# Kitware/pyLiDAR-SLAM

Measured on NVIDIA H100. Metric: icp_odometry_frames_per_sec, higher is better.
Workload: dtype f32

## Files before the change

### pylidar_slam_b200/csrc/context.cu

```cuda
#include <utility>

#include "internal.cuh"
#include "kdmap_device.cuh"

namespace pls {

long long g_kernel_launches = 0;

void DBuf::reserve(size_t bytes, cudaStream_t s, bool keep) {
    if (bytes <= cap) return;
    size_t want = bytes + bytes / 2 + 256;
    void* np = nullptr;
    PLS_CUDA(cudaStreamSynchronize(s));
    PLS_CUDA(cudaMalloc(&np, want));
    if (p) {
        if (keep) PLS_CUDA(cudaMemcpy(np, p, cap, cudaMemcpyDeviceToDevice));
        PLS_CUDA(cudaFree(p));
    }
    p = np;
    cap = want;
}

void DBuf::reserve_exact(size_t bytes, cudaStream_t s, bool keep) {
    if (bytes <= cap) return;
    void* np = nullptr;
    PLS_CUDA(cudaStreamSynchronize(s));
    PLS_CUDA(cudaMalloc(&np, bytes));
    if (p) {
        if (keep) PLS_CUDA(cudaMemcpy(np, p, cap, cudaMemcpyDeviceToDevice));
        PLS_CUDA(cudaFree(p));
    }
    p = np;
    cap = bytes;
}

void DBuf::release() {
    if (p) cudaFree(p);
    p = nullptr;
    cap = 0;
}

void HBuf::reserve(size_t bytes) {
    if (bytes <= cap) return;
    if (p) PLS_CUDA(cudaFreeHost(p));
    p = nullptr;
    cap = 0;
    PLS_CUDA(cudaHostAlloc(&p, bytes, cudaHostAllocMapped | cudaHostAllocPortable));
    cap = bytes;
}

void* HBuf::device_ptr() const {
    if (!p) return nullptr;
    void* d = nullptr;
    PLS_CUDA(cudaHostGetDevicePointer(&d, p, 0));
    return d;
}

void HBuf::release() {
    if (p) cudaFreeHost(p);
    p = nullptr;
    cap = 0;
}

void map_stream_begin(pls_context* ctx) {
    ctx->stream = ctx->stream_map;
    std::swap(ctx->sort, ctx->sort_map);
}

void map_stream_end(pls_context* ctx) {
    cudaEventRecord(ctx->ev_map_done, ctx->stream_map);
    ctx->map_pending = true;
    std::swap(ctx->sort, ctx->sort_map);
    ctx->stream = ctx->stream_main;
}

void map_stream_wait(pls_context* ctx) {
    if (ctx->map_pending) {
        cudaStreamWaitEvent(ctx->stream_main, ctx->ev_map_done, 0);
        ctx->map_pending = false;
    }
}

void sync_all(pls_context* ctx) {
    PLS_CUDA(cudaStreamSynchronize(ctx->stream_map));
    PLS_CUDA(cudaStreamSynchronize(ctx->stream_main));
    ctx->map_pending = false;
}

namespace {
struct PtrCacheEntry {
    const void* p;
    bool dev;
};
thread_local PtrCacheEntry t_ptr_cache[64] = {};
}

bool is_device_ptr(const void* p) {
    if (!p) return false;
    PtrCacheEntry& e = t_ptr_cache[(reinterpret_cast<uintptr_t>(p) >> 6) & 63u];
    if (e.p == p) return e.dev;
    const bool d = is_device_ptr_uncached(p);
    e.p = p;
    e.dev = d;
    return d;
}

bool is_device_ptr_uncached(const void* p) {
    if (!p) return false;
    cudaPointerAttributes a;
    cudaError_t e = cudaPointerGetAttributes(&a, p);
    if (e != cudaSuccess) {
        cudaGetLastError();
        return false;
    }
    return a.type == cudaMemoryTypeDevice || a.type == cudaMemoryTypeManaged;
}

const void* to_device(pls_context* ctx, const void* p, size_t bytes, DBuf& stage) {
    if (!p || bytes == 0) return p;
    if (is_device_ptr(p)) return p;
    stage.reserve(bytes, ctx->stream);
    PLS_CUDA(cudaMemcpyAsync(stage.p, p, bytes, cudaMemcpyHostToDevice, ctx->stream));
    return stage.p;
}

OutArg out_arg(pls_context* ctx, void* p, size_t bytes, DBuf& stage) {
    OutArg o;
    o.bytes = bytes;
    if (!p) return o;
    if (is_device_ptr(p)) {
        o.dev = p;
        return o;
    }
    stage.reserve(bytes, ctx->stream);
    o.host = p;
    o.dev = stage.p;
    return o;
}

void finish_out(pls_context* ctx, const OutArg& o, size_t bytes_used) {
    if (!o.host) return;
    size_t b = bytes_used == (size_t)-1 ? o.bytes : bytes_used;
    if (b) PLS_CUDA(cudaMemcpyAsync(o.host, o.dev, b, cudaMemcpyDeviceToHost, ctx->stream));
}

ProfileScope::ProfileScope(pls_context* c, int w, double bytes, bool count) : ctx(c), which(w) {
    ProfileSlot& s = ctx->prof[which];
    if (!s.enabled) return;
    if (s.used >= 4096) {
        cudaStreamSynchronize(ctx->stream_map);
        cudaStreamSynchronize(ctx->stream_main);
        profile_collect(ctx, which);
    }
    if (s.used + 2 > s.pool.size()) {
        for (int i = 0; i < 64; ++i) {
            cudaEvent_t e;
            if (cudaEventCreate(&e) != cudaSuccess) return;
            s.pool.push_back(e);
        }
    }
    e0 = s.pool[s.used++];
    e1 = s.pool[s.used++];
    if (count) {
        s.bytes += bytes;
        s.launches += 1;
    }
    cudaEventRecord(e0, ctx->stream);
}

ProfileScope::~ProfileScope() {
    if (e1) cudaEventRecord(e1, ctx->stream);
}

void profile_collect(pls_context* ctx, int which) {
    ProfileSlot& s = ctx->prof[which];
    for (size_t i = 0; i + 1 < s.used; i += 2) {
        float ms = 0.f;
        if (cudaEventElapsedTime(&ms, s.pool[i], s.pool[i + 1]) == cudaSuccess) s.ms += ms;
    }
    s.used = 0;
}

}

using namespace pls;

extern "C" {

const char* pls_version(void) { return "plslam_b200 0.1 (sm_90a)"; }

int pls_host_fingerprint(const void* host_ptr, int64_t num_bytes, uint64_t* out) {
    if (!host_ptr || !out || num_bytes < 0) return PLS_E_INVALID;
    const int64_t words = num_bytes / 8;
    uint64_t h = 0x9E3779B97F4A7C15ull ^ (uint64_t)num_bytes;
    const uint64_t* w = reinterpret_cast<const uint64_t*>(host_ptr);
    const int64_t step = words > 256 ? words / 256 : 1;
    for (int64_t i = 0; i < words; i += step) {
        uint64_t v;
        memcpy(&v, w + i, 8);
        h = (h ^ v) * 0x100000001B3ull;
        h ^= h >> 29;
    }
    if (words > 0) {
        uint64_t v;
        memcpy(&v, w + words - 1, 8);
        h = (h ^ v) * 0x100000001B3ull;
    }
    *out = h;
    return PLS_OK;
}

int pls_launch_count(int64_t* out) {
    if (!out) return PLS_E_INVALID;
    *out = (int64_t)pls::g_kernel_launches;
    return PLS_OK;
}

int pls_config_default(pls_config* c) {
    if (!c) return PLS_E_INVALID;
    memset(c, 0, sizeof(*c));
    c->height = 64;
    c->width = 2048;
    c->up_fov_deg = 3.0f;
    c->down_fov_deg = -24.0f;
    c->local_map_type = PLS_MAP_KDTREE;
    c->local_map_size = 20;
    c->num_neighbors_normals = 10;
    c->normals_kernel_size = 5;
    c->scheme = PLS_SCHEME_DEFAULT;
    c->sigma = 0.5f;
    c->gn_max_iters = 1;
    c->gn_norm_stop = 1e-3f;
    c->max_num_alignments = 100;
    c->threshold_delta_pose = 1e-4f;
    c->threshold_trans = 0.1f;
    c->threshold_rot = 0.3f;
    c->device = 0;
    c->stream = nullptr;
    return PLS_OK;
}

int pls_create(const pls_config* cfg, pls_context** out) {
    if (!cfg || !out) return PLS_E_INVALID;
    *out = nullptr;
    int ndev = 0;
    if (cudaGetDeviceCount(&ndev) != cudaSuccess || ndev <= 0) {
        cudaGetLastError();
        return PLS_E_CUDA;
    }
    if (cfg->device < 0 || cfg->device >= ndev) return PLS_E_INVALID;
    if (cfg->height <= 0 || cfg->width <= 0 || cfg->local_map_size <= 0) return PLS_E_INVALID;
    if (cfg->max_num_alignments < 1 || cfg->max_num_alignments > kMaxAlign) return PLS_E_INVALID;
    if (cfg->num_neighbors_normals < 3 || cfg->num_neighbors_normals + 1 > KD_KMAX_WIDE) return PLS_E_INVALID;
    if (cfg->normals_kernel_size < 1 || cfg->normals_kernel_size > 9 || (cfg->normals_kernel_size % 2) == 0)
        return PLS_E_INVALID;
    pls_context* ctx = new pls_context();
    ctx->cfg = *cfg;
    try {
        PLS_CUDA(cudaSetDevice(cfg->device));
        if (cfg->stream) {
            ctx->stream = (cudaStream_t)cfg->stream;
        } else {
            static const bool prio = !(getenv("PLS_STREAM_PRIORITY") && atoi(getenv("PLS_STREAM_PRIORITY")) == 0);
            int least = 0, greatest = 0;
            PLS_CUDA(cudaDeviceGetStreamPriorityRange(&least, &greatest));
            PLS_CUDA(cudaStreamCreateWithPriority(&ctx->stream, cudaStreamNonBlocking, prio ? greatest : 0));
            ctx->own_stream = true;
        }
        ctx->stream_main = ctx->stream;
        {
            static const bool prio = !(getenv("PLS_STREAM_PRIORITY") && atoi(getenv("PLS_STREAM_PRIORITY")) == 0);
            int least = 0, greatest = 0;
            PLS_CUDA(cudaDeviceGetStreamPriorityRange(&least, &greatest));
            PLS_CUDA(cudaStreamCreateWithPriority(&ctx->stream_map, cudaStreamNonBlocking, prio ? least : 0));
        }
        PLS_CUDA(cudaEventCreateWithFlags(&ctx->ev_map_done, cudaEventDisableTiming));
        ctx->pinned.reserve(kScalarOffset + 256);
        ctx->scalars.reserve(sizeof(FrameResult) + 4096, ctx->stream);
        PLS_CUDA(cudaMemsetAsync(ctx->scalars.p, 0, ctx->scalars.cap, ctx->stream));
        odometry_reset(ctx);
    } catch (const pls::Error& e) {
        fprintf(stderr, "pls_create: %s\n", e.msg.c_str());
        delete ctx;
        return e.code;
    }
    *out = ctx;
    return PLS_OK;
}

int pls_destroy(pls_context* ctx) {
    if (!ctx) return PLS_E_INVALID;
    cudaSetDevice(ctx->cfg.device);
    ctx->upd_pending = false;
    cudaStreamSynchronize(ctx->stream_map);
    cudaStreamSynchronize(ctx->stream_main);
    comm_free(ctx);
    if (ctx->p2p_pending_xchg) cudaFree(ctx->p2p_pending_xchg);
    for (auto& b : ctx->stage_in) b.release();
    for (auto& b : ctx->stage_out) b.release();
    for (auto& b : ctx->tmp) b.release();
    for (auto& b : ctx->next_buf) b.release();
    ctx->pinned.release();
    ctx->scalars.release();
    ctx->sort.keys_alt.release(); ctx->sort.vals_alt.release(); ctx->sort.hist.release();
    ctx->sort.status.release(); ctx->sort.plan.release();
    ctx->sort_map.keys_alt.release(); ctx->sort_map.vals_alt.release(); ctx->sort_map.hist.release();
    ctx->sort_map.status.release(); ctx->sort_map.plan.release();
    ctx->scan.status.release();
    ctx->sel[0].status.release(); ctx->sel[1].status.release(); ctx->input_zbuf.release();
    for (auto& b : ctx->kd.store) b.release();
    ctx->kd.morton.release(); ctx->kd.order.release(); ctx->kd.sorted.release(); ctx->kd.normals.release();
    ctx->kd.bbox.release(); ctx->kd.grid_hdr.release(); ctx->kd.cells.release(); ctx->kd.stats.release();
    ctx->kd_worklist.release(); ctx->kd_nn_state.release();
    ctx->pm.vmaps.release(); ctx->pm.nmaps.release(); ctx->pm.poses.release();
    ctx->pm.model_v.release(); ctx->pm.model_n.release(); ctx->pm.zbuf.release();
    for (auto& b : ctx->frame_vmap_buf) b.release();
    for (auto& b : ctx->frame_pts_buf) b.release();
    ctx->queries.release(); ctx->nn_prev.release();
    ctx->partials.release(); ctx->batch_buf.release(); ctx->hyp_buf.release(); ctx->gs_keys.release(); ctx->gs_vals.release(); ctx->gs_out_xyz.release();
    ctx->gs_out_idx.release();
    for (auto& s : ctx->prof)
        for (auto e : s.pool) cudaEventDestroy(e);
    if (ctx->ev_map_done) cudaEventDestroy(ctx->ev_map_done);
    if (ctx->ev_inputs) cudaEventDestroy(ctx->ev_inputs);
    if (ctx->ev_batch) cudaEventDestroy(ctx->ev_batch);
    ctx->gs_host_xyz.release(); ctx->gs_host_idx.release();
    if (ctx->stream_map) cudaStreamDestroy(ctx->stream_map);
    if (ctx->own_stream) cudaStreamDestroy(ctx->stream_main);
    delete ctx;
    return PLS_OK;
}

const char* pls_last_error(pls_context* ctx) { return ctx ? ctx->err.c_str() : "null context"; }

int pls_synchronize(pls_context* ctx) {
    PLS_API_BEGIN(ctx)
    sync_all(ctx);
    PLS_API_END(ctx)
}

int pls_wait_stream(pls_context* ctx, void* other_stream) {
    PLS_API_BEGIN(ctx)
    cudaStream_t other = (cudaStream_t)other_stream;
    if (other != ctx->stream_main) {
        if (!ctx->ev_inputs) PLS_CUDA(cudaEventCreateWithFlags(&ctx->ev_inputs, cudaEventDisableTiming));
        PLS_CUDA(cudaEventRecord(ctx->ev_inputs, other));
        PLS_CUDA(cudaStreamWaitEvent(ctx->stream_main, ctx->ev_inputs, 0));
    }
    PLS_API_END(ctx)
}

int pls_profile_enable(pls_context* ctx, int which, int enable) {
    PLS_API_BEGIN(ctx)
    PLS_REQUIRE(which >= 0 && which < kProfileSlots, "pls_profile_enable: bad slot");
    ctx->prof[which].enabled = enable != 0;
    PLS_API_END(ctx)
}

int pls_profile_read(pls_context* ctx, int which, double* ms_total, int64_t* launches, double* bytes, int reset) {
    PLS_API_BEGIN(ctx)
    PLS_REQUIRE(which >= 0 && which < kProfileSlots, "pls_profile_read: bad slot");
    sync_all(ctx);
    profile_collect(ctx, which);
    ProfileSlot& s = ctx->prof[which];
    if (ms_total) *ms_total = s.ms;
    if (launches) *launches = s.launches;
    if (bytes) *bytes = s.bytes;
    if (reset) {
        s.ms = 0;
        s.launches = 0;
        s.bytes = 0;
    }
    PLS_API_END(ctx)
}

}
```

### pylidar_slam_b200/csrc/internal.cuh

```cuda
#pragma once
#include <cuda_runtime.h>
#include <stddef.h>
#include <stdint.h>
#include <stdio.h>
#include <string.h>

#include <deque>
#include <string>
#include <vector>

#include "../../include/plslam_b200.h"

namespace pls {

constexpr int kNumSMs = 132;
constexpr int NACC = 30;
constexpr int kMaxAlign = 128;
constexpr int kProfileSlots = 16;
constexpr size_t kScalarOffset = 2048;

struct Error {
    int code;
    std::string msg;
};

extern long long g_kernel_launches;

#define PLS_CUDA(expr)                                                                            \
    do {                                                                                          \
        cudaError_t _e = (expr);                                                                  \
        if (_e != cudaSuccess) {                                                                  \
            throw pls::Error{PLS_E_CUDA, std::string(#expr) + ": " + cudaGetErrorString(_e) +     \
                                             " (" + __FILE__ + ":" + std::to_string(__LINE__) + ")"}; \
        }                                                                                         \
    } while (0)

#define PLS_CHECK_LAUNCH()            \
    do {                              \
        ++pls::g_kernel_launches;     \
        PLS_CUDA(cudaGetLastError()); \
    } while (0)

#ifdef __CUDACC__
__device__ __forceinline__ void pls_grid_dependency_wait() { asm volatile("griddepcontrol.wait;" ::: "memory"); }
#endif
template <typename... KArgs, typename... Args>
void launch_dependent(void (*kernel)(KArgs...), dim3 grid, dim3 block, cudaStream_t st, Args&&... args) {
    cudaLaunchConfig_t cfg = {};
    cfg.gridDim = grid;
    cfg.blockDim = block;
    cfg.dynamicSmemBytes = 0;
    cfg.stream = st;
    cudaLaunchAttribute attr[1];
    attr[0].id = cudaLaunchAttributeProgrammaticStreamSerialization;
    attr[0].val.programmaticStreamSerializationAllowed = 1;
    cfg.attrs = attr;
    cfg.numAttrs = 1;
    PLS_CUDA(cudaLaunchKernelEx(&cfg, kernel, static_cast<KArgs>(args)...));
    PLS_CHECK_LAUNCH();
}

#define PLS_REQUIRE(cond, text)                                   \
    do {                                                          \
        if (!(cond)) throw pls::Error{PLS_E_INVALID, (text)};     \
    } while (0)

struct DBuf {
    void* p = nullptr;
    size_t cap = 0;
    template <typename T>
    T* as() const { return reinterpret_cast<T*>(p); }
    void reserve(size_t bytes, cudaStream_t s, bool keep = false);
    void reserve_exact(size_t bytes, cudaStream_t s, bool keep = false);
    void release();
};

struct HBuf {
    void* p = nullptr;
    size_t cap = 0;
    template <typename T>
    T* as() const { return reinterpret_cast<T*>(p); }
    void reserve(size_t bytes);
    void release();
    void* device_ptr() const;
};

struct ProfileSlot {
    bool enabled = false;
    std::vector<cudaEvent_t> pool;
    size_t used = 0;
    double ms = 0.0;
    int64_t launches = 0;
    double bytes = 0.0;
};

struct SortScratch {
    DBuf keys_alt, vals_alt;
    DBuf hist;
    DBuf status;
    DBuf plan;
};

struct ScanScratch {
    DBuf status;
};

struct SelectScratch {
    DBuf status;
    uint32_t epoch = 0;
};

struct KdMap {
    DBuf store[2];
    int cur = 0;
    int64_t count = 0;
    std::deque<int64_t> frame_counts;
    DBuf morton, order;
    DBuf sorted;
    DBuf normals;
    DBuf bbox;
    bool bbox_clean = false;
    DBuf grid_hdr;
    DBuf cells;
    DBuf stats;
    size_t table_offset[16] = {};
    uint32_t table_mask[16] = {};
    uint32_t gen = 0;
    int64_t indexed = 0;
    bool valid = false;
    int64_t cap_points = 0;
    int64_t max_frame = 0;
    bool searched = false;
    bool searched_icp = false;
    bool searched_sharded = false;
    bool searched_normals = false;
    uint32_t searched_gen = 0;
    int64_t searched_n = 0;
};

struct ProjMap {
    int K = 0;
    int head = 0;
    DBuf vmaps, nmaps;
    DBuf poses;
    std::vector<float> host_poses;
    DBuf model_v, model_n;
    DBuf zbuf;
    bool valid = false;
    bool zbuf_clean = false;
    int64_t built_lo = 0, built_hi = 0;
};

struct FrameResult {
    float T[16];
    float params[6];
    float losses[kMaxAlign];
    int iters;
    int status;
    int done;
    int pad;
    double last_sums[NACC];
    long long counts[8];
    float first_pt[4];
};

struct Comm;

static_assert(sizeof(FrameResult) <= kScalarOffset, "FrameResult must fit before the scalar slots");

}

struct pls_context {
    pls_config cfg;
    cudaStream_t stream = nullptr;
    cudaStream_t stream_main = nullptr;
    cudaStream_t stream_map = nullptr;
    cudaEvent_t ev_map_done = nullptr;
    cudaEvent_t ev_inputs = nullptr;
    bool map_pending = false;
    bool own_stream = false;
    std::string err;

    pls::DBuf stage_in[4], stage_out[6];
    pls::HBuf pinned;
    pls::DBuf scalars;

    pls::SortScratch sort;
    pls::SortScratch sort_map;
    pls::ScanScratch scan;
    pls::SelectScratch sel[2];
    pls::DBuf input_zbuf;
    bool input_zbuf_clean = false;

    pls::DBuf tmp[8];
    pls::DBuf next_buf[8];

    pls::KdMap kd;
    pls::ProjMap pm;
    int frame_index = 0;
    int last_icp_iters = 0;
    bool icp_result = false;
    bool last_sharded = false;
    int sample_pointcloud = 0;
    float delta_since_update[16];
    pls::DBuf frame_vmap_buf[2];
    pls::DBuf frame_pts_buf[2];
    int frame_slot = 0;
    bool upd_pending = false, upd_insert = false;
    float upd_T[16];
    int upd_slot = 0;
    long long upd_count = 0;
    pls::DBuf queries;
    const float4* query_ptr = nullptr;
    pls::DBuf nn_prev;
    pls::DBuf kd_worklist;
    pls::DBuf kd_nn_state;
    pls::DBuf partials;
    pls::DBuf batch_buf;
    pls::DBuf hyp_buf;
    cudaEvent_t ev_batch = nullptr;
    pls::DBuf gs_keys, gs_vals, gs_out_xyz, gs_out_idx;
    uint32_t gs_seq = 0;
    pls::HBuf gs_host_xyz, gs_host_idx;
    int64_t last_query_count = 0;

    pls::Comm* comm = nullptr;
    void* p2p_pending_xchg = nullptr;
    pls::ProfileSlot prof[pls::kProfileSlots];
};

namespace pls {
void flush_map_update(pls_context* ctx);
}

#define PLS_API_BEGIN(ctx)                               \
    if (!(ctx)) return PLS_E_INVALID;                    \
    try {                                                \
        cudaSetDevice((ctx)->cfg.device);                \
        pls::flush_map_update(ctx);

#define PLS_API_BEGIN_FRAME(ctx)                         \
    if (!(ctx)) return PLS_E_INVALID;                    \
    try {                                                \
        cudaSetDevice((ctx)->cfg.device);

#define PLS_API_END(ctx)                                 \
    }                                                    \
    catch (const pls::Error& e) {                        \
        (ctx)->err = e.msg;                              \
        return e.code;                                   \
    }                                                    \
    catch (const std::exception& e) {                    \
        (ctx)->err = e.what();                           \
        return PLS_E_INVALID;                            \
    }                                                    \
    return PLS_OK;

namespace pls {

enum { SC_GS_COUNT = 0, SC_QUERY_COUNT = 1, SC_NAN_COUNT = 2, SC_INSERT_COUNT = 3, SC_PROJ_NC = 4,
       SC_SPARE0 = 5, SC_SPARE1 = 6,
       SC_GS_OVERFLOW = 7,
       SC_KD_COUNTERS = 8,
       SC_KD_LISTS = 16,
       SC_NUM = 32 };

bool is_device_ptr(const void* p);
bool is_device_ptr_uncached(const void* p);
const void* to_device(pls_context* ctx, const void* p, size_t bytes, DBuf& stage);
struct OutArg {
    void* host = nullptr;
    void* dev = nullptr;
    size_t bytes = 0;
};
OutArg out_arg(pls_context* ctx, void* p, size_t bytes, DBuf& stage);
void finish_out(pls_context* ctx, const OutArg& o, size_t bytes_used = (size_t)-1);

inline uint32_t* scalar_u32(pls_context* ctx, int i) {
    return reinterpret_cast<uint32_t*>(reinterpret_cast<char*>(ctx->scalars.p) + kScalarOffset) + i;
}
inline FrameResult* frame_result_dev(pls_context* ctx) { return reinterpret_cast<FrameResult*>(ctx->scalars.p); }
inline FrameResult* frame_result_host(pls_context* ctx) { return reinterpret_cast<FrameResult*>(ctx->pinned.p); }

void map_stream_begin(pls_context* ctx);
void map_stream_end(pls_context* ctx);
void map_stream_wait(pls_context* ctx);
void sync_all(pls_context* ctx);

struct ProfileScope {
    pls_context* ctx;
    int which;
    cudaEvent_t e0 = nullptr, e1 = nullptr;
    ProfileScope(pls_context* c, int w, double bytes, bool count = true);
    ~ProfileScope();
};
void profile_collect(pls_context* ctx, int which);
inline void profile_credit(pls_context* ctx, int which, int64_t launches, double bytes) {
    if (!ctx->prof[which].enabled) return;
    ctx->prof[which].launches += launches;
    ctx->prof[which].bytes += bytes;
}

void radix_sort_pairs(pls_context* ctx, uint64_t* keys, uint32_t* vals, int64_t n, int num_passes,
                      uint64_t** keys_out, uint32_t** vals_out, int64_t cap_n = 0);

void exclusive_scan_flags(pls_context* ctx, const uint8_t* flags, int64_t n, uint32_t* pos_out,
                          uint32_t* total_dev);

#ifdef __CUDACC__
__device__ __forceinline__ float warp_sum(float v) {
#pragma unroll
    for (int o = 16; o > 0; o >>= 1) v += __shfl_xor_sync(0xffffffffu, v, o);
    return v;
}
__device__ __forceinline__ double warp_sum(double v) {
#pragma unroll
    for (int o = 16; o > 0; o >>= 1) v += __shfl_xor_sync(0xffffffffu, v, o);
    return v;
}
__device__ __forceinline__ int float_to_ordered(float f) {
    int i = __float_as_int(f);
    return i >= 0 ? i : i ^ 0x7fffffff;
}
__device__ __forceinline__ float ordered_to_float(int i) {
    return __int_as_float(i >= 0 ? i : i ^ 0x7fffffff);
}
#endif

void launch_projection(pls_context* ctx, const float* xyz, const float* channels, int batch, int64_t n,
                       int C, int H, int W, float up, float down, float* out, unsigned long long* zbuf, float fill = 0.f);
void launch_projection_f64(pls_context* ctx, const double* xyz, int64_t n, int H, int W, float up, float down, float* out,
                           unsigned long long* zbuf);
void launch_zbuf_points(pls_context* ctx, const float* xyz, int64_t n, const uint32_t* n_dev, int H, int W, float up, float down,
                        unsigned long long* zbuf);
void launch_normal_map(pls_context* ctx, const float* vmap, int batch, int H, int W, int ksize, float* out);
struct GnParams {
    int scheme;
    double sigma;
};
void kdmap_reset(pls_context* ctx);
void kdmap_update(pls_context* ctx, const float* rel_pose_host, const float* pts_dev, int64_t n,
                  const float* vmap_dev, int H, int W, int64_t known_count);
void kdmap_update_packed(pls_context* ctx, const float* rel_pose_host, const float4* fresh_dev, int64_t num_new,
                         bool has_new);
constexpr int KD_BATCH_GRID = 6;
void kdmap_batch_begin(pls_context* lead, pls_context* const* ctxs, const int64_t* query_bounds, int num, cudaStream_t st,
                       int* grid);
void kdmap_batch_iterations(pls_context* lead, int num, cudaStream_t st, const int* grid, int first, int last);
void kdmap_batch_done(pls_context* lead, int num, cudaStream_t st, int* out);
struct KdScan {
    const float4* queries;
    const uint32_t* nq_dev;
    int64_t bound;
};
void kdmap_hypotheses_begin(pls_context* ctx, const KdScan* scans, int num, cudaStream_t st, int* grid, FrameResult** frs,
                            uint32_t** words);
void kdmap_hypothesis_adopt(pls_context* ctx, const KdScan& scan, int h, cudaStream_t st);
struct KdScanRows {
    const float* rows;
    int64_t n;
    float4* out;
    uint32_t* count;
};
void pack_valid_scans(pls_context* ctx, const std::vector<KdScanRows>& scans);
int kdmap_icp_iteration(pls_context* ctx, int64_t query_bound, const uint32_t* bound_dev, int rank, int num_ranks, int it,
                        float fuse_threshold, bool* solved);
void pack_valid_rows(pls_context* ctx, const float* pts_dev, int64_t n, float4* out, uint32_t* count_dev);
void pack_valid_rows_f64(pls_context* ctx, const double* pts_dev, int64_t n, float4* out, uint32_t* count_dev);
void pack_valid_pixels(pls_context* ctx, const float* vmap_dev, int64_t hw, float min_norm, float4* out,
                       uint32_t* count_dev);
struct GridSample {
    const void* xyz;
    bool f64;
    int64_t n;
    double voxel;
    void* out_xyz;
    long long* out_idx;
    void* host_xyz;
    long long* host_idx;
};
void grid_sample_enqueue(pls_context* ctx, const GridSample& g, bool count_to_host = true);
uint32_t grid_sample_finish(pls_context* ctx, const GridSample& g);
uint32_t grid_sample_host_count(pls_context* ctx, bool* overflowed);
void projmap_reset(pls_context* ctx);
void projmap_batch_begin(pls_context* lead, pls_context* const* ctxs, const int64_t* query_bounds, int num, cudaStream_t st,
                         int* grid);
void projmap_batch_iterations(pls_context* lead, pls_context* const* ctxs, const int64_t* query_bounds, int num, cudaStream_t st,
                              const int* grid, int first, int last);
void projmap_batch_done(pls_context* lead, int num, cudaStream_t st, int* out);
void projmap_hypotheses_begin(pls_context* ctx, int num, cudaStream_t st, FrameResult** frs, uint32_t** words);
void projmap_hypotheses_iterations(pls_context* ctx, int64_t query_bound, int num, cudaStream_t st, int first, int last);
void projmap_hypothesis_adopt(pls_context* ctx, int h, cudaStream_t st);
bool icp_shards(pls_context* ctx, int64_t work);
int comm_rank(pls_context* ctx);
int comm_size(pls_context* ctx);
void projmap_update(pls_context* ctx, const float* rel_pose_host, const float* vmap_dev);
void odometry_reset(pls_context* ctx);
void comm_allreduce_sums(pls_context* ctx, double* sums_dev);
void comm_free(pls_context* ctx);

}
```

### pylidar_slam_b200/csrc/kdmap.cu

```cuda
#include <stdlib.h>

#include <vector>

#include "gn_device.cuh"
#include "internal.cuh"
#include "icp_device.cuh"
#include "kdmap_device.cuh"
#include "pose_device.cuh"

namespace pls {

namespace {

inline int grid_for(int64_t n, int threads, int cap_blocks) {
    int64_t b = (n + threads - 1) / threads;
    return (int)(b < 1 ? 1 : (b > cap_blocks ? cap_blocks : b));
}

__global__ void kd_bbox_init_kernel(int* bbox) {
    if (threadIdx.x < 3) bbox[threadIdx.x] = 0x7fffffff;
    else if (threadIdx.x < 6) bbox[threadIdx.x] = (int)0x80000000;
}

struct Rigid {
    float R[9];
    float t[3];
};

__global__ void __launch_bounds__(256)
kd_move_append_kernel(const float4* __restrict__ src, int64_t skip, int64_t kept, Rigid X,
                      const float4* __restrict__ fresh, const uint32_t* __restrict__ num_new_dev, int64_t num_new_cap,
                      float4* __restrict__ dst, int* __restrict__ bbox) {
    const int64_t num_new = num_new_dev ? (int64_t)*num_new_dev : num_new_cap;
    const int64_t total = kept + num_new;
    float mn[3] = {FLT_MAX, FLT_MAX, FLT_MAX}, mx[3] = {-FLT_MAX, -FLT_MAX, -FLT_MAX};
    for (int64_t k = (int64_t)blockIdx.x * blockDim.x + threadIdx.x; k < total; k += (int64_t)gridDim.x * blockDim.x) {
        float4 p;
        if (k < kept) {
            float4 s = src[k + skip];
            p.x = X.R[0] * s.x + X.R[1] * s.y + X.R[2] * s.z + X.t[0];
            p.y = X.R[3] * s.x + X.R[4] * s.y + X.R[5] * s.z + X.t[1];
            p.z = X.R[6] * s.x + X.R[7] * s.y + X.R[8] * s.z + X.t[2];
            p.w = 0.f;
        } else {
            p = fresh[k - kept];
        }
        dst[k] = p;
        mn[0] = fminf(mn[0], p.x); mn[1] = fminf(mn[1], p.y); mn[2] = fminf(mn[2], p.z);
        mx[0] = fmaxf(mx[0], p.x); mx[1] = fmaxf(mx[1], p.y); mx[2] = fmaxf(mx[2], p.z);
    }
#pragma unroll
    for (int a = 0; a < 3; ++a) {
#pragma unroll
        for (int o = 16; o > 0; o >>= 1) {
            mn[a] = fminf(mn[a], __shfl_xor_sync(0xffffffffu, mn[a], o));
            mx[a] = fmaxf(mx[a], __shfl_xor_sync(0xffffffffu, mx[a], o));
        }
    }
    __shared__ float smn[8][3], smx[8][3];
    const int warp = threadIdx.x >> 5, lane = threadIdx.x & 31;
    if (lane == 0) {
#pragma unroll
        for (int a = 0; a < 3; ++a) { smn[warp][a] = mn[a]; smx[warp][a] = mx[a]; }
    }
    __syncthreads();
    if (threadIdx.x < 3) {
        const int a = threadIdx.x;
        float lo = smn[0][a], hi = smx[0][a];
        for (int w = 1; w < 8; ++w) { lo = fminf(lo, smn[w][a]); hi = fmaxf(hi, smx[w][a]); }
        if (lo != FLT_MAX) atomicMin(&bbox[a], float_to_ordered(lo));
        if (hi != -FLT_MAX) atomicMax(&bbox[3 + a], float_to_ordered(hi));
    }
}

template <typename T>
__global__ void kd_valid_rows_kernel(const T* __restrict__ pts, int64_t n, uint8_t* __restrict__ flags) {
    for (int64_t i = (int64_t)blockIdx.x * blockDim.x + threadIdx.x; i < n; i += (int64_t)gridDim.x * blockDim.x) {
        T x = pts[3 * i], y = pts[3 * i + 1], z = pts[3 * i + 2];
        flags[i] = (x == x && y == y && z == z) ? 1 : 0;
    }
}
template <typename T>
__global__ void kd_pack_rows_kernel(const T* __restrict__ pts, int64_t n, const uint8_t* __restrict__ flags,
                                    const uint32_t* __restrict__ pos, float4* __restrict__ out) {
    for (int64_t i = (int64_t)blockIdx.x * blockDim.x + threadIdx.x; i < n; i += (int64_t)gridDim.x * blockDim.x)
        if (flags[i]) out[pos[i]] = make_float4((float)pts[3 * i], (float)pts[3 * i + 1], (float)pts[3 * i + 2], 0.f);
}
constexpr int KD_PACK_THREADS = 1024, KD_PACK_ROWS = 4;
__global__ void __launch_bounds__(KD_PACK_THREADS) kd_pack_scans_kernel(const KdScanRows* __restrict__ scans) {
    __shared__ uint32_t s_warp[KD_PACK_ROWS][32];
    __shared__ uint32_t s_sub[KD_PACK_ROWS];
    const KdScanRows sc = scans[blockIdx.x];
    const int lane = threadIdx.x & 31, warp = threadIdx.x >> 5;
    const uint32_t below = (1u << lane) - 1u;
    uint32_t base = 0;
    for (int64_t t0 = 0; t0 < sc.n; t0 += (int64_t)KD_PACK_THREADS * KD_PACK_ROWS) {
        float4 v[KD_PACK_ROWS];
        bool ok[KD_PACK_ROWS];
        uint32_t rank[KD_PACK_ROWS];
#pragma unroll
        for (int j = 0; j < KD_PACK_ROWS; ++j) {
            const int64_t i = t0 + (int64_t)j * KD_PACK_THREADS + threadIdx.x;
            ok[j] = false;
            if (i < sc.n) {
                const float x = sc.rows[3 * i], y = sc.rows[3 * i + 1], z = sc.rows[3 * i + 2];
                ok[j] = x == x && y == y && z == z;
                v[j] = make_float4(x, y, z, 0.f);
            }
            const unsigned b = __ballot_sync(0xffffffffu, ok[j]);
            rank[j] = __popc(b & below);
            if (lane == 0) s_warp[j][warp] = __popc(b);
        }
        __syncthreads();
        if (warp < KD_PACK_ROWS) {
            const uint32_t c = s_warp[warp][lane];
            uint32_t inc = c;
#pragma unroll
            for (int o = 1; o < 32; o <<= 1) {
                const uint32_t u = __shfl_up_sync(0xffffffffu, inc, o);
                if (lane >= o) inc += u;
            }
            s_warp[warp][lane] = inc - c;
            if (lane == 31) s_sub[warp] = inc;
        }
        __syncthreads();
#pragma unroll
        for (int j = 0; j < KD_PACK_ROWS; ++j) {
            if (ok[j]) sc.out[base + s_warp[j][warp] + rank[j]] = v[j];
            base += s_sub[j];
        }
        __syncthreads();
    }
    if (threadIdx.x == 0) *sc.count = base;
}

template <typename T>
__global__ void kd_nonfinite_rows_kernel(const T* __restrict__ pts, int64_t n, uint32_t* __restrict__ count) {
    uint32_t bad = 0;
    for (int64_t i = (int64_t)blockIdx.x * blockDim.x + threadIdx.x; i < n; i += (int64_t)gridDim.x * blockDim.x)
        bad += !(isfinite((float)pts[3 * i]) && isfinite((float)pts[3 * i + 1]) && isfinite((float)pts[3 * i + 2]));
    bad = __reduce_add_sync(0xffffffffu, bad);
    if ((threadIdx.x & 31) == 0 && bad) atomicAdd(count, bad);
}
__global__ void kd_valid_pixels_kernel(const float* __restrict__ vmap, int64_t hw, float min_norm,
                                       uint8_t* __restrict__ flags) {
    for (int64_t i = (int64_t)blockIdx.x * blockDim.x + threadIdx.x; i < hw; i += (int64_t)gridDim.x * blockDim.x) {
        float x = vmap[i], y = vmap[hw + i], z = vmap[2 * hw + i];
        flags[i] = (sqrtf(x * x + y * y + z * z) > min_norm) ? 1 : 0;
    }
}
__global__ void kd_pack_pixels_kernel(const float* __restrict__ vmap, int64_t hw, const uint8_t* __restrict__ flags,
                                      const uint32_t* __restrict__ pos, float4* __restrict__ out) {
    for (int64_t i = (int64_t)blockIdx.x * blockDim.x + threadIdx.x; i < hw; i += (int64_t)gridDim.x * blockDim.x)
        if (flags[i]) out[pos[i]] = make_float4(vmap[i], vmap[hw + i], vmap[2 * hw + i], 0.f);
}

__global__ void kd_grid_header_kernel(int* __restrict__ bbox, KdGridHeader* __restrict__ hdr, float cell_target) {
    if (threadIdx.x != 0) return;
    const float mnx = ordered_to_float(bbox[0]), mny = ordered_to_float(bbox[1]), mnz = ordered_to_float(bbox[2]);
    const float ex = ordered_to_float(bbox[3]) - mnx, ey = ordered_to_float(bbox[4]) - mny,
                ez = ordered_to_float(bbox[5]) - mnz;
    const float ext = fmaxf(fmaxf(ex, ey), fmaxf(ez, 1e-6f));
    const int b0 = KD_MIN_B0;
    const float scale = fminf((float)(1 << b0) / cell_target, (float)KD_COORD_MAX / ext);
    hdr->mn[0] = mnx; hdr->mn[1] = mny; hdr->mn[2] = mnz;
    hdr->scale = scale;
    hdr->b0 = b0;
    hdr->cell0 = (float)(1 << b0) / scale;
    hdr->top = KD_COORD_BITS - b0;
    for (int l = 0; l < KD_MAX_LEVELS; ++l) hdr->overflow[l] = 0;
    bbox[0] = bbox[1] = bbox[2] = 0x7fffffff;
    bbox[3] = bbox[4] = bbox[5] = (int)0x80000000;
}

__global__ void kd_cell_key_kernel(const float4* __restrict__ pts, int64_t n, const KdGridHeader* __restrict__ hdr,
                                   uint64_t* __restrict__ keys, uint32_t* __restrict__ vals) {
    pls_grid_dependency_wait();
    const float mnx = hdr->mn[0], mny = hdr->mn[1], mnz = hdr->mn[2];
    const float scale = hdr->scale;
    const int b0 = hdr->b0;
    for (int64_t i = (int64_t)blockIdx.x * blockDim.x + threadIdx.x; i < n; i += (int64_t)gridDim.x * blockDim.x) {
        const float4 p = pts[i];
        const uint32_t qx = (uint32_t)fminf(fmaxf((p.x - mnx) * scale, 0.f), (float)KD_COORD_MAX);
        const uint32_t qy = (uint32_t)fminf(fmaxf((p.y - mny) * scale, 0.f), (float)KD_COORD_MAX);
        const uint32_t qz = (uint32_t)fminf(fmaxf((p.z - mnz) * scale, 0.f), (float)KD_COORD_MAX);
        keys[i] = (uint64_t)kd_cell_id(qx >> b0, qy >> b0, qz >> b0);
        vals[i] = (uint32_t)i;
    }
}

struct CellTables {
    uint4* table[KD_MAX_LEVELS];
    uint32_t mask[KD_MAX_LEVELS];
};

__device__ __forceinline__ int cell_claim(uint4* table, uint32_t mask, uint32_t id, uint32_t gen) {
    const unsigned long long want = (unsigned long long)id | ((unsigned long long)gen << 32);
    uint32_t h = kd_hash(id) & mask;
    for (int probe = 0; probe < 64; ++probe) {
        unsigned long long* word = reinterpret_cast<unsigned long long*>(&table[h]);
        unsigned long long old = *reinterpret_cast<volatile unsigned long long*>(word);
        while (true) {
            if (old == want) return (int)h;
            if ((uint32_t)(old >> 32) == gen) break;
            const unsigned long long prev = atomicCAS(word, old, want);
            if (prev == old) return (int)h;
            old = prev;
        }
        h = (h + 1) & mask;
    }
    return -1;
}

__global__ void __launch_bounds__(256)
kd_finalize_kernel(const float4* __restrict__ pts, const uint64_t* __restrict__ keys, const uint32_t* __restrict__ order,
                   int64_t n, CellTables T, KdGridHeader* hdr, uint32_t gen, float4* __restrict__ sorted) {
    pls_grid_dependency_wait();
    const int top = hdr->top;
    for (int64_t i = (int64_t)blockIdx.x * blockDim.x + threadIdx.x; i < n; i += (int64_t)gridDim.x * blockDim.x) {
        const uint32_t src = order[i];
        float4 p = pts[src];
        p.w = __uint_as_float(src);
        sorted[i] = p;
        const uint32_t k = (uint32_t)keys[i];
        int nh = top + 1, nt = top + 1;
        if (i > 0) {
            const uint32_t d = k ^ (uint32_t)keys[i - 1];
            nh = d ? min((31 - __clz((int)d)) / 3 + 1, top + 1) : 0;
        }
        if (i + 1 < n) {
            const uint32_t d = k ^ (uint32_t)keys[i + 1];
            nt = d ? min((31 - __clz((int)d)) / 3 + 1, top + 1) : 0;
        }
        const int nl = max(nh, nt);
        for (int l = 0; l < nl; ++l) {
            const int slot = cell_claim(T.table[l], T.mask[l], k >> (3 * l), gen);
            if (slot < 0) {
                hdr->overflow[l] = 1;
            } else {
                if (l < nh) T.table[l][slot].z = (uint32_t)i;
                if (l < nt) T.table[l][slot].w = (uint32_t)i;
            }
        }
    }
}

__global__ void kd_export_kernel(const float4* __restrict__ pts, int64_t n, float* __restrict__ out) {
    for (int64_t i = (int64_t)blockIdx.x * blockDim.x + threadIdx.x; i < n; i += (int64_t)gridDim.x * blockDim.x) {
        float4 p = pts[i];
        out[3 * i] = p.x; out[3 * i + 1] = p.y; out[3 * i + 2] = p.z;
    }
}

constexpr int KD_THREADS = 256;
constexpr int KD_WARPS = KD_THREADS / 32;

enum { KDC_NN_CAND = 0, KDC_KNN_CAND = 1, KDC_NORMALS = 2 };
enum { KDL_PENDING = 0, KDL_HARD_NN = 2, KDL_WORDS = 4 };

#ifdef PLS_KD_SPLIT
constexpr int KD_SPLIT_ITERS = 8;
constexpr int KD_SPLIT_BLOCKS = 8 * kNumSMs;
constexpr int KD_SPLIT_WORDS = (KD_SPLIT_ITERS + 1) * KD_SPLIT_BLOCKS * 2 * KD_SPLIT_STAMPS;
__device__ unsigned long long g_kd_split[KD_SPLIT_WORDS];
__device__ unsigned long long g_kd_split_normals_end;

__device__ __forceinline__ unsigned long long* kd_split_record(const FrameResult* fr) {
    const int slot = fr->done ? KD_SPLIT_ITERS : fr->iters;
    if ((!fr->done && slot >= KD_SPLIT_ITERS) || blockIdx.x >= KD_SPLIT_BLOCKS) return nullptr;
    return g_kd_split + ((size_t)slot * KD_SPLIT_BLOCKS + blockIdx.x) * 2 * KD_SPLIT_STAMPS;
}
#define KD_SPLIT_BEGIN()                             \
    unsigned long long* split = kd_split_record(fr); \
    __shared__ unsigned long long s_split[2];        \
    if (threadIdx.x == 0) {                          \
        PLS_SPLIT(0);                                \
        s_split[0] = s_split[1] = 0;                 \
        unsigned sm;                                 \
        asm volatile("mov.u32 %0, %%smid;" : "=r"(sm)); \
        if (split) split[11] = sm + 1;               \
    }
#define KD_SPLIT_MAX(k, dep) atomicMax(&s_split[k], split_now(dep))
#define KD_SPLIT_BLOCK_MAX()         \
    if (threadIdx.x == 0 && split) { \
        split[2] = s_split[0];       \
        split[3] = s_split[1];       \
    }
#define KD_SPLIT_ARG , unsigned long long* split, unsigned long long* s_split
#define KD_SPLIT_PASS , split, s_split
#else
#define KD_SPLIT_BEGIN()
#define KD_SPLIT_MAX(k, dep) \
    do {                     \
    } while (0)
#define KD_SPLIT_BLOCK_MAX()
#define KD_SPLIT_ARG
#define KD_SPLIT_PASS
#endif

__device__ __forceinline__ unsigned kd_logical_blocks(int64_t bound, const uint32_t* __restrict__ bound_dev) {
    if (!bound_dev) return gridDim.x;
    const int64_t n = min(bound, (int64_t)*bound_dev);
    const int64_t b = (n + KD_THREADS - 1) / KD_THREADS;
    return (unsigned)(b < 1 ? 1 : (b > 8 * kNumSMs ? 8 * kNumSMs : b));
}

__device__ __forceinline__ void block_flush_list(const int* s_list, int n, int* __restrict__ list, uint32_t* count, int* s_base) {
    if (n == 0) return;
    if (threadIdx.x == 0) *s_base = (int)atomicAdd(count, (uint32_t)n);
    __syncthreads();
    for (int i = threadIdx.x; i < n; i += blockDim.x) list[*s_base + i] = s_list[i];
}

__device__ __forceinline__ bool claim_normal(const KdIndex& ix, int pos) {
    const uint32_t claimed = kd_normal_claimed(ix.gen), valid = kd_normal_valid(ix.gen);
    uint32_t* w = reinterpret_cast<uint32_t*>(&ix.normals[pos].w);
    const uint32_t cur = __ldcg(w);
    return cur != valid && cur != claimed && atomicCAS(w, cur, claimed) == cur;
}

__device__ __forceinline__ void transform_query(const float* T, const float4& p0, float* p) {
    p[0] = p0.x * T[0] + p0.y * T[1] + p0.z * T[2] + T[3];
    p[1] = p0.x * T[4] + p0.y * T[5] + p0.z * T[6] + T[7];
    p[2] = p0.x * T[8] + p0.y * T[9] + p0.z * T[10] + T[11];
}

__device__ __forceinline__ bool match_proven(const KdIndex& ix, const float* p, int pos, const float4& state) {
    if (pos < 0) return false;
    const float4 s = state;
    const float d = sqrtf(dist2_point(p[0], p[1], p[2], __ldg(ix.sorted + pos)));
    const float eps = sqrtf(dist2_point(p[0], p[1], p[2], s));
    return (d + eps) * 1.00001f + 1e-6f < sqrtf(s.w);
}

template <int R = 1>
__device__ __forceinline__ void warp_normal_moments(const KdIndex& ix, const KdGridLocal& g, const float4& c, int k, int lane,
                                                    int* cand, unsigned long long* stage, float* cov) {
    if constexpr (R == 1) {
        int ni;
        const int found = warp_knn(ix, g, c.x, c.y, c.z, k + 1, lane, ni, cand, stage);
        warp_second_moments(ix, c, k, found, ni, lane, cov);
    } else {
        unsigned long long kept[R];
        const int found = warp_knn_wide<R>(ix, g, c.x, c.y, c.z, k + 1, lane, kept, cand, stage);
        warp_second_moments_wide<R>(ix, c, k, found, kept, lane, cov);
    }
}

__device__ __forceinline__ void store_normal(const KdIndex& ix, int pos, const float* cov, uint32_t valid) {
    float nn[3];
    smallest_eigenvector(cov, nn);
    __stcg(ix.normals + pos, make_float4(nn[0], nn[1], nn[2], __uint_as_float(valid)));
}

__device__ __forceinline__ void accumulate_match(double* acc, const KdIndex& ix, const float* p, int pos, int scheme,
                                                 float sigma KD_SPLIT_ARG) {
    const float4 qq = __ldg(ix.sorted + pos);
    const float4 nv = __ldcg(ix.normals + pos);
    float q[3] = {qq.x, qq.y, qq.z};
    float nn[3] = {nv.x, nv.y, nv.z};
    float J[6];
    const float r = p2plane_residual_jacobian_identity(p, q, nn, J);
    KD_SPLIT_MAX(0, r);
    const float w = ls_weight<float>(scheme, sigma, r, p, q);
    accumulate_normal_equations<float>(acc, J, w, r * w, r);
}

template <int THREADS>
__device__ __forceinline__ void block_partial_and_finish(double* acc, FrameResult* fr, double* __restrict__ partials,
                                                         float fuse_threshold, unsigned block, unsigned grid KD_SPLIT_ARG) {
    KD_SPLIT_MAX(1, acc[0] + acc[29]);
    __syncwarp();
    block_reduce_store<THREADS, KD_WARPS>(acc, partials + (size_t)block * NACC);
    KD_SPLIT_BLOCK_MAX()
    if (fuse_threshold >= 0.f) icp_finish_in_last_block<THREADS>(fr, partials, (int)grid, fuse_threshold PLS_SPLIT_PASS);
}

__device__ __forceinline__ void kd_nn_verify_body(const KdIndex& ix, const float4* __restrict__ queries,
                                                  const uint32_t* __restrict__ nq_dev, int64_t q_begin, int64_t q_stride,
                                                  const float* __restrict__ T, const int* __restrict__ done,
                                                  const int* __restrict__ match, const float4* __restrict__ nn_state,
                                                  int* __restrict__ hard, uint32_t* lists, int parity, unsigned block) {
    if (done && *done) return;
    __shared__ float sT[12];
    __shared__ int s_hard[KD_THREADS];
    __shared__ int s_nh, s_base;
    if (threadIdx.x < 12) sT[threadIdx.x] = T[threadIdx.x];
    if (threadIdx.x == 0) {
        s_nh = 0;
        if (block == 0)
            for (int l = 0; l < KDL_WORDS; l += 2) lists[l + (parity ^ 1)] = 0;
    }
    __syncthreads();
    const int64_t nq = (int64_t)*nq_dev;
    const int64_t qi = q_begin + ((int64_t)block * KD_THREADS + threadIdx.x) * q_stride;
    if (qi < nq) {
        float p[3];
        transform_query(sT, queries[qi], p);
        if (!match_proven(ix, p, match[qi], nn_state[qi])) s_hard[atomicAdd(&s_nh, 1)] = (int)qi;
    }
    __syncthreads();
    block_flush_list(s_hard, s_nh, hard, lists + KDL_HARD_NN + parity, &s_base);
}

__global__ void __launch_bounds__(KD_THREADS)
kd_nn_verify_kernel(KdIndex ix, const float4* __restrict__ queries, const uint32_t* __restrict__ nq_dev, int64_t q_begin,
                    int64_t q_stride, const float* __restrict__ T, const int* __restrict__ done, const int* __restrict__ match,
                    const float4* __restrict__ nn_state, int* __restrict__ hard, uint32_t* lists, int parity) {
    kd_nn_verify_body(ix, queries, nq_dev, q_begin, q_stride, T, done, match, nn_state, hard, lists, parity, blockIdx.x);
}


__device__ __forceinline__ void kd_nn_warp_body(const KdIndex& ix, const float4* __restrict__ queries,
                                                const uint32_t* __restrict__ nq_dev, int64_t q_begin, int64_t q_stride,
                                                const int* __restrict__ hard, uint32_t* lists, int parity,
                                                const float* __restrict__ T, const int* __restrict__ done,
                                                int* __restrict__ match, float4* __restrict__ nn_state, int want_normals,
                                                int* __restrict__ pending, unsigned long long* __restrict__ counters,
                                                unsigned block, unsigned grid) {
    if (done && *done) return;
    int n;
    if (hard) {
        n = (int)lists[KDL_HARD_NN + parity];
    } else {
        const int64_t nq = (int64_t)*nq_dev;
        n = nq > q_begin ? (int)((nq - q_begin + q_stride - 1) / q_stride) : 0;
        if (block == 0 && threadIdx.x == 0)
            for (int l = 0; l < KDL_WORDS; l += 2) lists[l + (parity ^ 1)] = 0;
    }
    const int lane = threadIdx.x & 31;
    const int warp_global = block * KD_WARPS + (threadIdx.x >> 5);
    const int total_warps = grid * KD_WARPS;
    if (warp_global >= n) return;
    float t[12];
#pragma unroll
    for (int a = 0; a < 12; ++a) t[a] = T[a];
    const KdGridLocal g = kd_load_grid(ix);
    uint32_t* pending_count = lists + KDL_PENDING + parity;
    int my_pos = -1, held = 0, cand = 0;
    auto flush_claims = [&]() {
        const bool mine = want_normals && my_pos >= 0 && claim_normal(ix, my_pos);
        const unsigned m = __ballot_sync(FULL, mine);
        if (m) {
            int base = 0;
            if (lane == 0) base = (int)atomicAdd(pending_count, (uint32_t)__popc(m));
            base = __shfl_sync(FULL, base, 0);
            if (mine) pending[base + __popc(m & ((1u << lane) - 1u))] = my_pos;
        }
        my_pos = -1;
        held = 0;
    };
    int s = warp_global;
    int64_t qi = hard ? (int64_t)hard[s] : q_begin + (int64_t)s * q_stride;
    float4 p0 = queries[qi];
    int hint = hard ? match[qi] : -1;
    while (true) {
        const int sn = s + total_warps;
        int64_t qn = qi;
        float4 pn = p0;
        int hn = -1;
        if (sn < n) {
            qn = hard ? (int64_t)hard[sn] : q_begin + (int64_t)sn * q_stride;
            pn = queries[qn];
            if (hard) hn = match[qn];
        }
        float p[3];
        transform_query(t, p0, p);
        float second;
        const int pos = warp_nearest(ix, g, p[0], p[1], p[2], hint, lane, &cand, &second);
        if (lane == 0) {
            match[qi] = pos;
            if (nn_state) nn_state[qi] = make_float4(p[0], p[1], p[2], second);
        }
        if (lane == held) my_pos = pos;
        if (++held == 32) flush_claims();
        if (sn >= n) break;
        s = sn;
        qi = qn;
        p0 = pn;
        hint = hn;
    }
    flush_claims();
    if (counters && lane == 0 && cand) atomicAdd(counters + KDC_NN_CAND, (unsigned long long)cand);
}

__global__ void __launch_bounds__(KD_THREADS)
kd_nn_warp_kernel(KdIndex ix, const float4* __restrict__ queries, const uint32_t* __restrict__ nq_dev, int64_t q_begin,
                  int64_t q_stride, const int* __restrict__ hard, uint32_t* lists, int parity, const float* __restrict__ T,
                  const int* __restrict__ done, int* __restrict__ match, float4* __restrict__ nn_state, int want_normals,
                  int* __restrict__ pending, unsigned long long* __restrict__ counters) {
    pls_grid_dependency_wait();
    kd_nn_warp_body(ix, queries, nq_dev, q_begin, q_stride, hard, lists, parity, T, done, match, nn_state, want_normals,
                    pending, counters, blockIdx.x, gridDim.x);
}

template <int R = 1>
__device__ __forceinline__ void kd_normals_warp_body(const KdIndex& ix, int k_normals, const int* __restrict__ worklist,
                                                     const uint32_t* __restrict__ wl_count, const int* __restrict__ done,
                                                     unsigned long long* __restrict__ counters, unsigned block, unsigned grid) {
    if (done && *done) return;
    __shared__ unsigned long long s_stage[KD_WARPS][KNN_STAGE];
    const int n = (int)*wl_count;
    const int lane = threadIdx.x & 31;
    const int warp_global = block * KD_WARPS + (threadIdx.x >> 5);
    const int total_warps = grid * KD_WARPS;
    if (warp_global >= n) return;
    unsigned long long* stage = s_stage[threadIdx.x >> 5];
    const KdGridLocal g = kd_load_grid(ix);
    const uint32_t valid = kd_normal_valid(ix.gen);
    float mycov[6];
    int mypos = -1, held = 0, cand = 0, done_here = 0;
    int e = warp_global;
    int pos = worklist[e];
    float4 c = __ldg(ix.sorted + pos);
    while (true) {
        const int en = e + total_warps;
        int posn = 0;
        float4 cn = c;
        if (en < n) {
            posn = worklist[en];
// ... 104 lines not shown
    for (int64_t round = (int64_t)block * KD_THREADS;; round += (int64_t)grid * KD_THREADS) {
        if (q_begin + round * q_stride >= nq) break;
        if (threadIdx.x == 0) s_nh = 0;
        __syncthreads();
        const int64_t qi = q_begin + (round + threadIdx.x) * q_stride;
        if (owner && qi < nq) {
            float p[3];
            transform_query(sT, queries[qi], p);
            if (!match_proven(ix, p, match[qi], nn_state[qi])) s_hard[atomicAdd(&s_nh, 1)] = threadIdx.x;
        }
        __syncthreads();
        const int nh = s_nh;
#ifdef PLS_KD_SPLIT
        if (threadIdx.x == 0 && split) split[9] += (unsigned long long)nh;
#endif
        if (warp < nh) {
            const KdGridLocal g = kd_load_grid(ix);
            for (int e = warp; e < nh; e += KD_REFINE_WARPS) {
                const int64_t q = q_begin + (round + s_hard[e]) * q_stride;
                float p[3];
                transform_query(sT, queries[q], p);
                float second;
                const int pos = warp_nearest(ix, g, p[0], p[1], p[2], match[q], lane, &cand_nn, &second);
                if (lane == 0) {
                    match[q] = pos;
                    nn_state[q] = make_float4(p[0], p[1], p[2], second);
                }
                if (pos < 0) continue;
                const uint32_t state = __shfl_sync(FULL, __ldcg(reinterpret_cast<const uint32_t*>(&ix.normals[pos].w)), 0);
                if (state == valid) continue;
                float cov[6];
                warp_normal_moments(ix, g, __ldg(ix.sorted + pos), k_normals, lane, &cand_knn, s_stage[warp], cov);
                if (lane == 0) store_normal(ix, pos, cov, valid);
                ++normals_here;
            }
        }
        __syncthreads();
    }
    if (counters && lane == 0) {
        if (cand_nn) atomicAdd(counters + KDC_NN_CAND, (unsigned long long)cand_nn);
        if (cand_knn) atomicAdd(counters + KDC_KNN_CAND, (unsigned long long)cand_knn);
        if (normals_here) atomicAdd(counters + KDC_NORMALS, (unsigned long long)normals_here);
    }
#ifdef PLS_KD_SPLIT
    if (lane == 0 && split && normals_here) atomicAdd(split + 10, (unsigned long long)normals_here);
#endif
    if (threadIdx.x == 0) PLS_SPLIT(1);
    double acc[NACC];
#pragma unroll
    for (int a = 0; a < NACC; ++a) acc[a] = 0.0;
    for (int64_t s = (int64_t)block * KD_THREADS + threadIdx.x; owner; s += (int64_t)grid * KD_THREADS) {
        const int64_t qi = q_begin + s * q_stride;
        if (qi >= nq) break;
        const int pos = match[qi];
        if (pos < 0) continue;
        float p[3];
        transform_query(sT, queries[qi], p);
        accumulate_match(acc, ix, p, pos, scheme, sigma KD_SPLIT_PASS);
    }
    block_partial_and_finish<KD_REFINE_THREADS>(acc, fr, partials, fuse_threshold, block, grid KD_SPLIT_PASS);
}

__global__ void __launch_bounds__(KD_REFINE_THREADS)
kd_icp_refine_kernel(KdIndex ix, const float4* __restrict__ queries, const uint32_t* __restrict__ nq_dev, int64_t q_begin,
                     int64_t q_stride, FrameResult* fr, int scheme, float sigma, int k_normals, int* __restrict__ match,
                     float4* __restrict__ nn_state, double* __restrict__ partials, float fuse_threshold,
                     unsigned long long* __restrict__ counters, int64_t bound, const uint32_t* __restrict__ bound_dev) {
    pls_grid_dependency_wait();
    const unsigned grid = kd_logical_blocks(bound, bound_dev);
    if (blockIdx.x >= grid) return;
    KD_SPLIT_BEGIN()
    kd_icp_refine_body(ix, queries, nq_dev, q_begin, q_stride, fr, scheme, sigma, k_normals, match, nn_state, partials,
                       fuse_threshold, counters, blockIdx.x, grid KD_SPLIT_PASS);
}

struct KdSeq {
    KdIndex ix;
    const float4* queries;
    const uint32_t* nq_dev;
    FrameResult* fr;
    int* match;
    float4* nn_state;
    int* pending;
    int* hard;
    uint32_t* lists;
    double* partials;
    unsigned long long* counters;
    int scheme;
    float sigma;
    int k_normals;
    float fuse_threshold;
    int max_iters;
    int blocks;
    int refine_blocks;
    int verify_blocks;
    int nn_blocks, kn_blocks;
};
static_assert(sizeof(KdSeq) % sizeof(int) == 0, "KdSeq is copied in 4-byte words");

__device__ __forceinline__ void load_seq(const KdSeq* __restrict__ seqs, KdSeq& s) {
    const int* src = reinterpret_cast<const int*>(seqs + blockIdx.y);
    int* dst = reinterpret_cast<int*>(&s);
    for (int i = threadIdx.x; i < (int)(sizeof(KdSeq) / sizeof(int)); i += blockDim.x) dst[i] = __ldg(src + i);
    __syncthreads();
}

#ifdef PLS_KD_SPLIT
#define KD_SPLIT_NONE()                     \
    unsigned long long* split = nullptr;    \
    __shared__ unsigned long long s_split[2];
#else
#define KD_SPLIT_NONE()
#endif

__device__ __forceinline__ bool four_launch_step(const KdSeq& s, int it) {
    return it == 0 || (s.refine_blocks == 0 && it < s.max_iters);
}

__global__ void __launch_bounds__(KD_THREADS) kd_nn_verify_batch_kernel(const KdSeq* __restrict__ seqs, int it) {
    __shared__ KdSeq s;
    load_seq(seqs, s);
    if ((int)blockIdx.x >= s.verify_blocks || !four_launch_step(s, it)) return;
    kd_nn_verify_body(s.ix, s.queries, s.nq_dev, 0, 1, s.fr->T, &s.fr->done, s.match, s.nn_state, s.hard, s.lists, it & 1,
                      blockIdx.x);
}

__global__ void __launch_bounds__(KD_THREADS) kd_nn_warp_batch_kernel(const KdSeq* __restrict__ seqs, int it) {
    __shared__ KdSeq s;
    load_seq(seqs, s);
    if ((int)blockIdx.x >= s.nn_blocks || !four_launch_step(s, it)) return;
    kd_nn_warp_body(s.ix, s.queries, s.nq_dev, 0, 1, it == 0 ? nullptr : s.hard, s.lists, it & 1, s.fr->T, &s.fr->done,
                    s.match, s.nn_state, 1, s.pending, s.counters, blockIdx.x, s.nn_blocks);
}

__global__ void __launch_bounds__(KD_THREADS) kd_normals_warp_batch_kernel(const KdSeq* __restrict__ seqs, int it) {
    __shared__ KdSeq s;
    load_seq(seqs, s);
    if ((int)blockIdx.x >= s.kn_blocks || !four_launch_step(s, it) || kd_wide_k(s.k_normals)) return;
    kd_normals_warp_body(s.ix, s.k_normals, s.pending, s.lists + KDL_PENDING + (it & 1), &s.fr->done, s.counters,
                         blockIdx.x, s.kn_blocks);
}

template <int R>
__global__ void __launch_bounds__(KD_THREADS) kd_normals_wide_batch_kernel(const KdSeq* __restrict__ seqs, int it) {
    __shared__ KdSeq s;
    load_seq(seqs, s);
    if ((int)blockIdx.x >= s.kn_blocks || !four_launch_step(s, it) || !kd_wide_k(s.k_normals)) return;
    kd_normals_warp_body<R>(s.ix, s.k_normals, s.pending, s.lists + KDL_PENDING + (it & 1), &s.fr->done, s.counters,
                            blockIdx.x, s.kn_blocks);
}

__global__ void __launch_bounds__(KD_THREADS) kd_residual_batch_kernel(const KdSeq* __restrict__ seqs, int it) {
    __shared__ KdSeq s;
    load_seq(seqs, s);
    if ((int)blockIdx.x >= s.blocks || !four_launch_step(s, it)) return;
    KD_SPLIT_NONE()
    kd_residual_body(s.ix, s.queries, s.nq_dev, 0, 1, s.fr, s.scheme, s.sigma, s.match, s.partials, s.fuse_threshold,
                     blockIdx.x, s.blocks KD_SPLIT_PASS);
}

__global__ void __launch_bounds__(KD_REFINE_THREADS) kd_icp_refine_batch_kernel(const KdSeq* __restrict__ seqs, int it) {
    __shared__ KdSeq s;
    load_seq(seqs, s);
    if ((int)blockIdx.x >= s.refine_blocks || it >= s.max_iters) return;
    KD_SPLIT_NONE()
    kd_icp_refine_body(s.ix, s.queries, s.nq_dev, 0, 1, s.fr, s.scheme, s.sigma, s.k_normals, s.match, s.nn_state,
                       s.partials, s.fuse_threshold, s.counters, blockIdx.x, s.refine_blocks KD_SPLIT_PASS);
}

__global__ void kd_batch_done_kernel(const KdSeq* __restrict__ seqs, int num, int* __restrict__ out) {
    for (int i = threadIdx.x; i < num; i += blockDim.x) out[i] = seqs[i].fr->done;
}

__global__ void kd_rows_to_float4_kernel(const float* __restrict__ rows, int64_t n, float4* __restrict__ out) {
    for (int64_t i = (int64_t)blockIdx.x * blockDim.x + threadIdx.x; i < n; i += (int64_t)gridDim.x * blockDim.x)
        out[i] = make_float4(rows[3 * i], rows[3 * i + 1], rows[3 * i + 2], 0.f);
}

__global__ void kd_search_export_kernel(KdIndex ix, const int* __restrict__ match, int64_t n, float* __restrict__ out_nb,
                                        float* __restrict__ out_nrm, long long* __restrict__ out_idx) {
    const float nan = __int_as_float(0x7fc00000);
    for (int64_t i = (int64_t)blockIdx.x * blockDim.x + threadIdx.x; i < n; i += (int64_t)gridDim.x * blockDim.x) {
        const int pos = match[i];
        float4 q = make_float4(nan, nan, nan, 0.f), nv = make_float4(nan, nan, nan, 0.f);
        long long idx = -1;
        if (pos >= 0) {
            q = __ldg(ix.sorted + pos);
            idx = (long long)__float_as_uint(q.w);
            if (out_nrm) nv = __ldcg(ix.normals + pos);
        }
        out_nb[3 * i] = q.x; out_nb[3 * i + 1] = q.y; out_nb[3 * i + 2] = q.z;
        if (out_idx) out_idx[i] = idx;
        if (out_nrm) { out_nrm[3 * i] = nv.x; out_nrm[3 * i + 1] = nv.y; out_nrm[3 * i + 2] = nv.z; }
    }
}

__global__ void __launch_bounds__(KD_THREADS)
kd_knn_export_kernel(KdIndex ix, const float* __restrict__ rows, int64_t n, int K, long long* __restrict__ out_idx,
                     float* __restrict__ out_d2, int* __restrict__ out_pos) {
    __shared__ unsigned long long s_stage[KD_WARPS][KNN_STAGE];
    const int lane = threadIdx.x & 31, warp = threadIdx.x >> 5;
    const KdGridLocal g = kd_load_grid(ix);
    const float nan = __int_as_float(0x7fc00000);
    for (int64_t q = (int64_t)blockIdx.x * KD_WARPS + warp; q < n; q += (int64_t)gridDim.x * KD_WARPS) {
        const float x = rows[3 * q], y = rows[3 * q + 1], z = rows[3 * q + 2];
        int pos;
        warp_knn(ix, g, x, y, z, K, lane, pos, nullptr, s_stage[warp]);
        if (lane < K) {
            long long idx = -1;
            float d2 = nan;
            if (pos >= 0) {
                const float4 s = __ldg(ix.sorted + pos);
                idx = (long long)__float_as_uint(s.w);
                d2 = dist2_point(x, y, z, s);
            }
            out_idx[q * K + lane] = idx;
            out_d2[q * K + lane] = d2;
            if (out_pos) out_pos[q * K + lane] = pos;
        }
    }
}

template <int R>
__global__ void __maxnreg__(128)
kd_knn_wide_export_kernel(KdIndex ix, const float* __restrict__ rows, int64_t n, int K, long long* __restrict__ out_idx,
                          float* __restrict__ out_d2, int* __restrict__ out_pos) {
    __shared__ unsigned long long s_stage[KD_WARPS][KNN_STAGE];
    const int lane = threadIdx.x & 31, warp = threadIdx.x >> 5;
    const KdGridLocal g = kd_load_grid(ix);
    const float nan = __int_as_float(0x7fc00000);
    for (int64_t q = (int64_t)blockIdx.x * KD_WARPS + warp; q < n; q += (int64_t)gridDim.x * KD_WARPS) {
        const float x = rows[3 * q], y = rows[3 * q + 1], z = rows[3 * q + 2];
        unsigned long long kept[R];
        warp_knn_wide<R>(ix, g, x, y, z, K, lane, kept, nullptr, s_stage[warp]);
#pragma unroll
        for (int r = 0; r < R; ++r) {
            const int j = r * 32 + lane;
            if (j >= K) break;
            const int pos = kept[r] != KNN_NONE ? (int)(unsigned)kept[r] : -1;
            long long idx = -1;
            float d2 = nan;
            if (pos >= 0) {
                const float4 s = __ldg(ix.sorted + pos);
                idx = (long long)__float_as_uint(s.w);
                d2 = dist2_point(x, y, z, s);
            }
            out_idx[q * K + j] = idx;
            out_d2[q * K + j] = d2;
            if (out_pos) out_pos[q * K + j] = pos;
        }
    }
}

size_t cell_table_bytes(int64_t M, uint32_t* masks, size_t* offsets) {
    size_t off = 0;
    for (int l = 0; l < KD_MAX_LEVELS; ++l) {
        uint64_t want = (uint64_t)(1.5 * (double)M) >> l;
        uint32_t sz = 64;
        while (sz < want) sz <<= 1;
        if (masks) masks[l] = sz - 1;
        if (offsets) offsets[l] = off;
        off += (size_t)sz * sizeof(uint4);
    }
    return off;
}

void kd_reserve_capacity(pls_context* ctx, int64_t need) {
    KdMap& kd = ctx->kd;
    if (need <= kd.cap_points) return;
    cudaStream_t st = ctx->stream;
    int64_t steady = (int64_t)(1.3 * (double)kd.max_frame * (double)(ctx->cfg.local_map_size + 1));
    if (steady > need + (8ll << 20)) steady = need + (8ll << 20);
    int64_t cap = need + need / 4 + 64;
    if (cap < steady) cap = steady;
    const size_t C = (size_t)cap;
    kd.store[kd.cur].reserve_exact(C * sizeof(float4), st, true);
    kd.store[kd.cur ^ 1].reserve_exact(C * sizeof(float4), st);
    kd.morton.reserve_exact(C * sizeof(uint64_t), st);
    kd.order.reserve_exact(C * sizeof(uint32_t), st);
    kd.sorted.reserve_exact(C * sizeof(float4), st);
    kd.normals.reserve_exact(C * sizeof(float4), st);
    const size_t table_bytes = cell_table_bytes(cap, nullptr, nullptr);
    kd.cells.reserve_exact(table_bytes, st);
    PLS_CUDA(cudaMemsetAsync(kd.normals.p, 0, C * sizeof(float4), st));
    PLS_CUDA(cudaMemsetAsync(kd.cells.p, 0, table_bytes, st));
    kd.cap_points = cap;
}

KdIndex make_index(pls_context* ctx) {
    KdIndex ix;
    ix.sorted = ctx->kd.sorted.as<float4>();
    ix.normals = ctx->kd.normals.as<float4>();
    ix.M = (int)ctx->kd.indexed;
    ix.gen = ctx->kd.gen;
    ix.grid = ctx->kd.grid_hdr.as<KdGridHeader>();
    for (int l = 0; l < KD_MAX_LEVELS; ++l) {
        ix.table[l] = reinterpret_cast<const uint4*>(reinterpret_cast<const char*>(ctx->kd.cells.p) + ctx->kd.table_offset[l]);
        ix.mask[l] = ctx->kd.table_mask[l];
    }
    ix.stats = ctx->kd.stats.p ? ctx->kd.stats.as<unsigned long long>() : nullptr;
    return ix;
}

void build_index(pls_context* ctx) {
    KdMap& kd = ctx->kd;
    cudaStream_t st = ctx->stream;
    const int64_t M = kd.count;
    kd.indexed = M;
    kd.valid = M > 0;
    if (M <= 0) return;
    ProfileScope ps(ctx, 3, (double)M * 32.0);
    PLS_REQUIRE(M < (1ll << 30), "kd map: too many points");
    kd_reserve_capacity(ctx, M);
    kd.gen += 1;
    if (kd.gen >= 0x7ffffff0u) {
        PLS_CUDA(cudaMemsetAsync(kd.normals.p, 0, kd.normals.cap, st));
        PLS_CUDA(cudaMemsetAsync(kd.cells.p, 0, kd.cells.cap, st));
        kd.gen = 1;
    }
    const float4* pts = kd.store[kd.cur].as<float4>();
    kd.grid_hdr.reserve(sizeof(KdGridHeader), st);
    static const float cell_target = getenv("PLS_KD_CELL") ? (float)atof(getenv("PLS_KD_CELL")) : KD_CELL_TARGET;
    kd_grid_header_kernel<<<1, 32, 0, st>>>(kd.bbox.as<int>(), kd.grid_hdr.as<KdGridHeader>(), cell_target);
    PLS_CHECK_LAUNCH();
    kd.bbox_clean = true;
    launch_dependent(kd_cell_key_kernel, grid_for(M, 256, 8 * kNumSMs), 256, st, pts, M, kd.grid_hdr.as<KdGridHeader>(),
                     kd.morton.as<uint64_t>(), kd.order.as<uint32_t>());
    uint64_t* sk;
    uint32_t* sv;
    radix_sort_pairs(ctx, kd.morton.as<uint64_t>(), kd.order.as<uint32_t>(), M, 4, &sk, &sv, kd.cap_points);
    cell_table_bytes(kd.cap_points, kd.table_mask, kd.table_offset);
    CellTables T;
    for (int l = 0; l < KD_MAX_LEVELS; ++l) {
        T.table[l] = reinterpret_cast<uint4*>(reinterpret_cast<char*>(kd.cells.p) + kd.table_offset[l]);
        T.mask[l] = kd.table_mask[l];
    }
    launch_dependent(kd_finalize_kernel, grid_for(M, 256, 8 * kNumSMs), 256, st, pts, sk, sv, M, T, kd.grid_hdr.as<KdGridHeader>(),
                     kd.gen, kd.sorted.as<float4>());
}

}

void kdmap_reset(pls_context* ctx) {
    if (getenv("PLS_KD_STATS") && !ctx->kd.stats.p) {
        ctx->kd.stats.reserve(16 * sizeof(unsigned long long), ctx->stream);
        cudaMemsetAsync(ctx->kd.stats.p, 0, 16 * sizeof(unsigned long long), ctx->stream);
    }
    ctx->kd.count = 0;
    ctx->kd.cur = 0;
    ctx->kd.frame_counts.clear();
    ctx->kd.indexed = 0;
    ctx->kd.valid = false;
    ctx->kd.bbox_clean = false;
    ctx->kd.max_frame = 0;
    ctx->kd.searched = false;
}

template <typename T>
static void pack_valid_rows_impl(pls_context* ctx, const T* pts_dev, int64_t n, float4* out, uint32_t* count_dev) {
    cudaStream_t st = ctx->stream;
    if (n <= 0) {
        PLS_CUDA(cudaMemsetAsync(count_dev, 0, sizeof(uint32_t), st));
        return;
    }
    ctx->tmp[1].reserve((size_t)n, st);
    ctx->tmp[2].reserve((size_t)n * sizeof(uint32_t), st);
    const int g = grid_for(n, 256, 8 * kNumSMs);
    kd_valid_rows_kernel<T><<<g, 256, 0, st>>>(pts_dev, n, ctx->tmp[1].as<uint8_t>());
    PLS_CHECK_LAUNCH();
    exclusive_scan_flags(ctx, ctx->tmp[1].as<uint8_t>(), n, ctx->tmp[2].as<uint32_t>(), count_dev);
    kd_pack_rows_kernel<T><<<g, 256, 0, st>>>(pts_dev, n, ctx->tmp[1].as<uint8_t>(), ctx->tmp[2].as<uint32_t>(), out);
    PLS_CHECK_LAUNCH();
}

void pack_valid_rows(pls_context* ctx, const float* pts_dev, int64_t n, float4* out, uint32_t* count_dev) {
    pack_valid_rows_impl<float>(ctx, pts_dev, n, out, count_dev);
}
void pack_valid_rows_f64(pls_context* ctx, const double* pts_dev, int64_t n, float4* out, uint32_t* count_dev) {
    pack_valid_rows_impl<double>(ctx, pts_dev, n, out, count_dev);
}

void pack_valid_scans(pls_context* ctx, const std::vector<KdScanRows>& scans) {
    cudaStream_t st = ctx->stream;
    const size_t bytes = scans.size() * sizeof(KdScanRows);
    ctx->stage_in[2].reserve(bytes, st);
    PLS_CUDA(cudaMemcpyAsync(ctx->stage_in[2].p, scans.data(), bytes, cudaMemcpyHostToDevice, st));
    kd_pack_scans_kernel<<<(unsigned)scans.size(), KD_PACK_THREADS, 0, st>>>(ctx->stage_in[2].as<KdScanRows>());
    PLS_CHECK_LAUNCH();
}

void pack_valid_pixels(pls_context* ctx, const float* vmap_dev, int64_t hw, float min_norm, float4* out,
                       uint32_t* count_dev) {
    cudaStream_t st = ctx->stream;
    ctx->tmp[1].reserve((size_t)hw, st);
    ctx->tmp[2].reserve((size_t)hw * sizeof(uint32_t), st);
    const int g = grid_for(hw, 256, 8 * kNumSMs);
    kd_valid_pixels_kernel<<<g, 256, 0, st>>>(vmap_dev, hw, min_norm, ctx->tmp[1].as<uint8_t>());
    PLS_CHECK_LAUNCH();
    exclusive_scan_flags(ctx, ctx->tmp[1].as<uint8_t>(), hw, ctx->tmp[2].as<uint32_t>(), count_dev);
    kd_pack_pixels_kernel<<<g, 256, 0, st>>>(vmap_dev, hw, ctx->tmp[1].as<uint8_t>(), ctx->tmp[2].as<uint32_t>(), out);
    PLS_CHECK_LAUNCH();
}

void kdmap_update_packed(pls_context* ctx, const float* rel_pose_host, const float4* fresh_dev, int64_t num_new,
                         bool has_new) {
    KdMap& kd = ctx->kd;
    cudaStream_t st = ctx->stream;
    Rigid X;
    int64_t skip = 0;
    const bool first = kd.frame_counts.empty() && kd.count == 0;
    if (first) {
        for (int i = 0; i < 9; ++i) X.R[i] = (i % 4 == 0) ? 1.f : 0.f;
        X.t[0] = X.t[1] = X.t[2] = 0.f;
        kd.frame_counts.push_back(num_new);
    } else {
        float inv[16];
        rigid_inverse(rel_pose_host, inv);
        X.R[0] = inv[0]; X.R[1] = inv[1]; X.R[2] = inv[2];
        X.R[3] = inv[4]; X.R[4] = inv[5]; X.R[5] = inv[6];
        X.R[6] = inv[8]; X.R[7] = inv[9]; X.R[8] = inv[10];
        X.t[0] = inv[3]; X.t[1] = inv[7]; X.t[2] = inv[11];
        if (has_new) {
            kd.frame_counts.push_back(num_new);
            if ((int)kd.frame_counts.size() > ctx->cfg.local_map_size) {
                skip = kd.frame_counts.front();
                kd.frame_counts.pop_front();
            }
        }
    }
    if (!has_new) num_new = 0;
    const int64_t kept = kd.count - skip;
    const int64_t total = kept + num_new;
    if (num_new > kd.max_frame) kd.max_frame = num_new;
    kd_reserve_capacity(ctx, total > 0 ? total : 1);
    const int dst = kd.cur ^ 1;
    kd.bbox.reserve(8 * sizeof(int), st);
    if (!kd.bbox_clean) {
        kd_bbox_init_kernel<<<1, 32, 0, st>>>(kd.bbox.as<int>());
        PLS_CHECK_LAUNCH();
    }
    kd.bbox_clean = false;
    if (total > 0) {
        kd_move_append_kernel<<<grid_for(total, 256, 8 * kNumSMs), 256, 0, st>>>(
            kd.store[kd.cur].as<float4>(), skip, kept, X, fresh_dev, nullptr, num_new, kd.store[dst].as<float4>(),
            kd.bbox.as<int>());
        PLS_CHECK_LAUNCH();
    }
    kd.cur = dst;
    kd.count = total;
    build_index(ctx);
}

void kdmap_update(pls_context* ctx, const float* rel_pose_host, const float* pts_dev, int64_t n,
                  const float* vmap_dev, int H, int W, int64_t known_count) {
    cudaStream_t st = ctx->stream;
    const bool has_new = (pts_dev != nullptr) || (vmap_dev != nullptr);
    const int64_t cap_new = pts_dev ? n : (vmap_dev ? (int64_t)H * W : 0);
    int64_t num_new = 0;
    if (has_new && cap_new > 0) {
        ctx->tmp[4].reserve((size_t)cap_new * sizeof(float4), st);
        uint32_t* cnt = scalar_u32(ctx, SC_INSERT_COUNT);
        if (pts_dev) {
            pack_valid_rows(ctx, pts_dev, cap_new, ctx->tmp[4].as<float4>(), cnt);
        } else {
            pack_valid_pixels(ctx, vmap_dev, cap_new, 0.01f, ctx->tmp[4].as<float4>(), cnt);
        }
        if (known_count >= 0) {
            num_new = known_count;
        } else {
            uint32_t c = 0;
            PLS_CUDA(cudaMemcpyAsync(&c, cnt, sizeof(uint32_t), cudaMemcpyDeviceToHost, st));
            PLS_CUDA(cudaStreamSynchronize(st));
            num_new = c;
        }
    }
    kdmap_update_packed(ctx, rel_pose_host, ctx->tmp[4].as<float4>(), num_new, has_new);
}

static int resident_blocks(const void* kernel) {
    int per_sm = 0;
    if (cudaOccupancyMaxActiveBlocksPerMultiprocessor(&per_sm, kernel, KD_THREADS, 0) != cudaSuccess || per_sm < 1) {
        cudaGetLastError();
        per_sm = 2;
    }
    return per_sm * kNumSMs;
}

static unsigned long long* kd_counters(pls_context* ctx) {
    return reinterpret_cast<unsigned long long*>(scalar_u32(ctx, SC_KD_COUNTERS));
}

static void record_search(KdMap& kd, bool icp, bool sharded, bool normals, int64_t n) {
    kd.searched = true;
    kd.searched_icp = icp;
    kd.searched_sharded = sharded;
    kd.searched_normals = normals;
    kd.searched_gen = kd.gen;
    kd.searched_n = n;
}

struct KdPlan {
    int64_t mine;
    size_t slots;
    int blocks;
    int wblocks;
};

static KdPlan plan_kd_iteration(pls_context* ctx, int64_t query_bound, int num_ranks) {
    cudaStream_t st = ctx->stream;
    KdPlan p;
    p.mine = (query_bound + num_ranks - 1) / num_ranks;
    p.slots = (size_t)p.mine + 64;
    p.blocks = grid_for(p.mine, KD_THREADS, 8 * kNumSMs);
    p.wblocks = (int)((p.mine + KD_WARPS - 1) / KD_WARPS);
    ctx->nn_prev.reserve((size_t)query_bound * sizeof(int), st);
    ctx->partials.reserve((size_t)p.blocks * NACC * sizeof(double), st);
    ctx->kd_worklist.reserve(2 * p.slots * sizeof(int), st);
    ctx->kd_nn_state.reserve(p.slots * (size_t)num_ranks * sizeof(float4), st);
    return p;
}

template <int R>
static void launch_normals_wide(pls_context* ctx, int wblocks, const KdIndex& ix, const int* pending, const uint32_t* count,
                                const int* done, unsigned long long* counters) {
    static const int resident = resident_blocks((const void*)kd_normals_wide_kernel<R>);
    launch_dependent(kd_normals_wide_kernel<R>, wblocks < resident ? wblocks : resident, KD_THREADS, ctx->stream, ix,
                     ctx->cfg.num_neighbors_normals, pending, count, done, counters);
}

static void launch_search(pls_context* ctx, const KdPlan& plan, const KdIndex& ix, const float4* queries, const uint32_t* nq_dev,
                          int rank, int num_ranks, const float* T, const int* done, int* match, bool first, bool normals,
                          int parity) {
    cudaStream_t st = ctx->stream;
    int* pending = ctx->kd_worklist.as<int>();
    int* hard_nn = pending + plan.slots;
    float4* nn_state = ctx->kd_nn_state.as<float4>();
    uint32_t* lists = scalar_u32(ctx, SC_KD_LISTS);
    unsigned long long* counters = kd_counters(ctx);
    const int tblocks = (int)((plan.mine + KD_THREADS - 1) / KD_THREADS);
    static const int resident_nn = resident_blocks((const void*)kd_nn_warp_kernel);
    static const int resident_kn = resident_blocks((const void*)kd_normals_warp_kernel);
    const int wblocks = plan.wblocks;
    if (!first) {
        ProfileScope p6(ctx, 6, 0.0);
        kd_nn_verify_kernel<<<tblocks, KD_THREADS, 0, st>>>(ix, queries, nq_dev, (int64_t)rank, (int64_t)num_ranks, T, done, match,
                                                            nn_state, hard_nn, lists, parity);
        PLS_CHECK_LAUNCH();
    }
    {
        ProfileScope p7(ctx, 7, 0.0);
        launch_dependent(kd_nn_warp_kernel, wblocks < resident_nn ? wblocks : resident_nn, KD_THREADS, st, ix, queries, nq_dev,
                         (int64_t)rank, (int64_t)num_ranks, first ? nullptr : hard_nn, lists, parity, T, done, match, nn_state,
                         normals ? 1 : 0, pending, counters);
    }
    if (!normals) return;
    ProfileScope p9(ctx, 9, 0.0);
    const int k = ctx->cfg.num_neighbors_normals;
    if (!kd_wide_k(k)) {
        launch_dependent(kd_normals_warp_kernel, wblocks < resident_kn ? wblocks : resident_kn, KD_THREADS, st, ix, k, pending,
                         lists + KDL_PENDING + parity, done, counters);
        return;
    }
    switch (kd_wide_regs(k + 1)) {
        case 2: launch_normals_wide<2>(ctx, wblocks, ix, pending, lists + KDL_PENDING + parity, done, counters); break;
        case 4: launch_normals_wide<4>(ctx, wblocks, ix, pending, lists + KDL_PENDING + parity, done, counters); break;
        default: launch_normals_wide<8>(ctx, wblocks, ix, pending, lists + KDL_PENDING + parity, done, counters); break;
    }
}

constexpr int64_t KD_COLD_MAP_POINTS = 2000000;

static bool kd_later_four_launch(int64_t indexed, int k) { return indexed >= KD_COLD_MAP_POINTS || kd_wide_k(k); }

int kdmap_icp_iteration(pls_context* ctx, int64_t query_bound, const uint32_t* bound_dev, int rank, int num_ranks, int it,
                        float fuse_threshold, bool* solved) {
    PLS_REQUIRE(ctx->kd.valid, "kd map: search before any update");
    PLS_REQUIRE(!bound_dev || num_ranks == 1, "kd ICP: a device-side query bound needs an unsharded frame");
    cudaStream_t st = ctx->stream;
    FrameResult* fr = frame_result_dev(ctx);
    const uint32_t* nq_dev = reinterpret_cast<const uint32_t*>(&fr->counts[1]);
    ProfileScope ps(ctx, 0, 0.0, false);
    const KdIndex ix = make_index(ctx);
    const KdPlan plan = plan_kd_iteration(ctx, query_bound, num_ranks);
    const int blocks = plan.blocks;
    record_search(ctx->kd, true, num_ranks > 1, true, 0);
    if (it == 0 || kd_later_four_launch(ctx->kd.indexed, ctx->cfg.num_neighbors_normals)) {
        launch_search(ctx, plan, ix, ctx->query_ptr, nq_dev, rank, num_ranks, fr->T, &fr->done, ctx->nn_prev.as<int>(), it == 0,
                      true, it & 1);
        ProfileScope p10(ctx, 10, 0.0);
        launch_dependent(kd_residual_kernel, blocks, KD_THREADS, st, ix, ctx->query_ptr, nq_dev, (int64_t)rank, (int64_t)num_ranks,
                         fr, ctx->cfg.scheme, ctx->cfg.sigma, ctx->nn_prev.as<int>(), ctx->partials.as<double>(), fuse_threshold,
                         plan.mine, bound_dev);
    } else {
        ProfileScope p11(ctx, 11, 0.0);
        launch_dependent(kd_icp_refine_kernel, blocks, KD_REFINE_THREADS, st, ix, ctx->query_ptr, nq_dev, (int64_t)rank,
                         (int64_t)num_ranks, fr, ctx->cfg.scheme, ctx->cfg.sigma, ctx->cfg.num_neighbors_normals,
                         ctx->nn_prev.as<int>(), ctx->kd_nn_state.as<float4>(), ctx->partials.as<double>(), fuse_threshold,
                         kd_counters(ctx), plan.mine, bound_dev);
    }
    *solved = fuse_threshold >= 0.f;
    return blocks;
}

static KdSeq make_seq(pls_context* ctx, const KdPlan& plan, const float4* queries, FrameResult* fr, const uint32_t* nq_dev,
                      int* match, float4* nn_state, int* worklist, uint32_t* words, double* partials, int share_nn,
                      int share_kn) {
    KdSeq s;
    s.ix = make_index(ctx);
    s.queries = queries;
    s.nq_dev = nq_dev;
    s.fr = fr;
    s.match = match;
    s.nn_state = nn_state;
    s.pending = worklist;
    s.hard = worklist + plan.slots;
    s.lists = words + (SC_KD_LISTS - SC_KD_COUNTERS);
    s.partials = partials;
    s.counters = reinterpret_cast<unsigned long long*>(words);
    s.scheme = ctx->cfg.scheme;
    s.sigma = ctx->cfg.sigma;
    s.k_normals = ctx->cfg.num_neighbors_normals;
    s.fuse_threshold = ctx->cfg.threshold_delta_pose;
    s.max_iters = ctx->cfg.max_num_alignments;
    s.blocks = plan.blocks;
    s.refine_blocks = kd_later_four_launch(ctx->kd.indexed, ctx->cfg.num_neighbors_normals) ? 0 : plan.blocks;
    s.verify_blocks = (int)((plan.mine + KD_THREADS - 1) / KD_THREADS);
    s.nn_blocks = plan.wblocks < share_nn ? plan.wblocks : share_nn;
    s.kn_blocks = plan.wblocks < share_kn ? plan.wblocks : share_kn;
    return s;
}

static void upload_seqs(pls_context* lead, const std::vector<KdSeq>& seqs, cudaStream_t st, int* grid) {
    grid[0] = grid[1] = grid[2] = 1;
    grid[3] = grid[4] = grid[5] = 0;
    for (const KdSeq& s : seqs) {
        grid[0] = grid[0] > s.blocks ? grid[0] : s.blocks;
        grid[1] = grid[1] > s.nn_blocks ? grid[1] : s.nn_blocks;
        grid[2] = grid[2] > s.kn_blocks ? grid[2] : s.kn_blocks;
        if (s.refine_blocks == 0) grid[3] = grid[3] > s.verify_blocks ? grid[3] : s.verify_blocks;
        else grid[4] = 1;
        if (kd_wide_k(s.k_normals)) {
            const int r = kd_wide_regs(s.k_normals + 1);
            grid[5] = grid[5] > r ? grid[5] : r;
        }
    }
    const size_t bytes = seqs.size() * sizeof(KdSeq);
    lead->batch_buf.reserve(bytes + PLS_MAX_SEQUENCES * sizeof(int), st);
    PLS_CUDA(cudaMemcpyAsync(lead->batch_buf.p, seqs.data(), bytes, cudaMemcpyHostToDevice, st));
}

void kdmap_batch_begin(pls_context* lead, pls_context* const* ctxs, const int64_t* query_bounds, int num, cudaStream_t st,
                       int* grid) {
    static const int resident_nn = resident_blocks((const void*)kd_nn_warp_batch_kernel);
    static const int resident_kn = resident_blocks((const void*)kd_normals_warp_batch_kernel);
    const int share_nn = (resident_nn + num - 1) / num, share_kn = (resident_kn + num - 1) / num;
    std::vector<KdSeq> seqs;
    for (int i = 0; i < num; ++i) {
        pls_context* ctx = ctxs[i];
        PLS_REQUIRE(ctx->kd.valid, "kd map: search before any update");
        const KdPlan plan = plan_kd_iteration(ctx, query_bounds[i], 1);
        ctx->last_sharded = false;
        record_search(ctx->kd, true, false, true, 0);
        FrameResult* fr = frame_result_dev(ctx);
        seqs.push_back(make_seq(ctx, plan, ctx->query_ptr, fr, reinterpret_cast<const uint32_t*>(&fr->counts[1]), ctx->nn_prev.as<int>(),
                                ctx->kd_nn_state.as<float4>(), ctx->kd_worklist.as<int>(), scalar_u32(ctx, SC_KD_COUNTERS),
                                ctx->partials.as<double>(), share_nn, share_kn));
    }
    upload_seqs(lead, seqs, st, grid);
}

void kdmap_batch_iterations(pls_context* lead, int num, cudaStream_t st, const int* grid, int first, int last) {
    const KdSeq* seqs = lead->batch_buf.as<KdSeq>();
    for (int it = first; it < last; ++it) {
        if (it > 0 && grid[4]) {
            kd_icp_refine_batch_kernel<<<dim3(grid[0], num), KD_REFINE_THREADS, 0, st>>>(seqs, it);
            PLS_CHECK_LAUNCH();
        }
        if (it > 0 && !grid[3]) continue;
        if (it > 0) {
            kd_nn_verify_batch_kernel<<<dim3(grid[3], num), KD_THREADS, 0, st>>>(seqs, it);
            PLS_CHECK_LAUNCH();
        }
        kd_nn_warp_batch_kernel<<<dim3(grid[1], num), KD_THREADS, 0, st>>>(seqs, it);
        PLS_CHECK_LAUNCH();
        kd_normals_warp_batch_kernel<<<dim3(grid[2], num), KD_THREADS, 0, st>>>(seqs, it);
        PLS_CHECK_LAUNCH();
        if (grid[5]) {
            const dim3 g(grid[2], num);
            if (grid[5] == 2) kd_normals_wide_batch_kernel<2><<<g, KD_THREADS, 0, st>>>(seqs, it);
            else if (grid[5] == 4) kd_normals_wide_batch_kernel<4><<<g, KD_THREADS, 0, st>>>(seqs, it);
            else kd_normals_wide_batch_kernel<8><<<g, KD_THREADS, 0, st>>>(seqs, it);
            PLS_CHECK_LAUNCH();
        }
        kd_residual_batch_kernel<<<dim3(grid[0], num), KD_THREADS, 0, st>>>(seqs, it);
        PLS_CHECK_LAUNCH();
    }
}

void kdmap_hypotheses_begin(pls_context* ctx, const KdScan* scans, int num, cudaStream_t st, int* grid, FrameResult** frs,
                            uint32_t** words) {
    PLS_REQUIRE(ctx->kd.valid, "kd map: search before any update");
    static const int resident_nn = resident_blocks((const void*)kd_nn_warp_batch_kernel);
    static const int resident_kn = resident_blocks((const void*)kd_normals_warp_batch_kernel);
    ctx->last_sharded = false;
    record_search(ctx->kd, true, false, true, 0);
    auto up = [](size_t b) { return (b + 255) & ~(size_t)255; };
    const size_t fr_bytes = up((size_t)num * sizeof(FrameResult)), word_bytes = up((size_t)num * 16 * sizeof(uint32_t));
    std::vector<KdPlan> plans;
    std::vector<size_t> offs;
    size_t total = fr_bytes + word_bytes;
    for (int h = 0; h < num; ++h) {
        plans.push_back(plan_kd_iteration(ctx, scans[h].bound, 1));
        const KdPlan& p = plans.back();
        offs.push_back(total);
        total += up((size_t)scans[h].bound * sizeof(int)) + up(p.slots * sizeof(float4)) + up(2 * p.slots * sizeof(int)) +
                 up((size_t)p.blocks * NACC * sizeof(double));
    }
    ctx->hyp_buf.reserve(total, st);
    char* base = ctx->hyp_buf.as<char>();
    *frs = reinterpret_cast<FrameResult*>(base);
    *words = reinterpret_cast<uint32_t*>(base + fr_bytes);
    const int share_nn = (resident_nn + num - 1) / num, share_kn = (resident_kn + num - 1) / num;
    std::vector<KdSeq> seqs;
    for (int h = 0; h < num; ++h) {
        const KdPlan& p = plans[(size_t)h];
        char* match = base + offs[(size_t)h];
        char* state = match + up((size_t)scans[h].bound * sizeof(int));
        char* list = state + up(p.slots * sizeof(float4));
        char* part = list + up(2 * p.slots * sizeof(int));
        seqs.push_back(make_seq(ctx, p, scans[h].queries, *frs + h, scans[h].nq_dev, reinterpret_cast<int*>(match),
                                reinterpret_cast<float4*>(state), reinterpret_cast<int*>(list), *words + 16 * h,
                                reinterpret_cast<double*>(part), share_nn, share_kn));
    }
    upload_seqs(ctx, seqs, st, grid);
}

void kdmap_hypothesis_adopt(pls_context* ctx, const KdScan& scan, int h, cudaStream_t st) {
    KdSeq s;
    PLS_CUDA(cudaMemcpyAsync(&s, ctx->batch_buf.as<KdSeq>() + h, sizeof(KdSeq), cudaMemcpyDeviceToHost, st));
    PLS_CUDA(cudaStreamSynchronize(st));
    PLS_CUDA(cudaMemcpyAsync(ctx->nn_prev.p, s.match, (size_t)scan.bound * sizeof(int), cudaMemcpyDeviceToDevice, st));
    PLS_CUDA(cudaMemcpyAsync(ctx->kd_nn_state.p, s.nn_state, (size_t)scan.bound * sizeof(float4), cudaMemcpyDeviceToDevice,
                             st));
    FrameResult* fr = frame_result_dev(ctx);
    PLS_CUDA(cudaMemcpyAsync(fr, s.fr, offsetof(FrameResult, counts), cudaMemcpyDeviceToDevice, st));
    uint32_t* nq = reinterpret_cast<uint32_t*>(&fr->counts[1]);
    if (scan.nq_dev != nq) PLS_CUDA(cudaMemcpyAsync(nq, scan.nq_dev, sizeof(uint32_t), cudaMemcpyDeviceToDevice, st));
    ctx->query_ptr = scan.queries;
}

void kdmap_batch_done(pls_context* lead, int num, cudaStream_t st, int* out) {
    int* dev = reinterpret_cast<int*>(lead->batch_buf.as<char>() + (size_t)num * sizeof(KdSeq));
    kd_batch_done_kernel<<<1, 64, 0, st>>>(lead->batch_buf.as<KdSeq>(), num, dev);
    PLS_CHECK_LAUNCH();
    PLS_CUDA(cudaMemcpyAsync(out, dev, (size_t)num * sizeof(int), cudaMemcpyDeviceToHost, st));
    PLS_CUDA(cudaStreamSynchronize(st));
}

}

using namespace pls;

extern "C" {

int pls_kdmap_update_points(pls_context* ctx, const float* rel_pose, const float* points, int64_t n) {
    PLS_API_BEGIN(ctx)
    map_stream_wait(ctx);
    PLS_REQUIRE(rel_pose, "pls_kdmap_update_points: rel_pose required");
    PLS_REQUIRE(ctx->cfg.local_map_type == PLS_MAP_KDTREE, "context holds a projective map");
    float rel[16];
    if (is_device_ptr(rel_pose)) PLS_CUDA(cudaMemcpy(rel, rel_pose, sizeof(rel), cudaMemcpyDeviceToHost));
    else memcpy(rel, rel_pose, sizeof(rel));
    const float* d = (points && n > 0) ? (const float*)to_device(ctx, points, (size_t)n * 3 * sizeof(float), ctx->stage_in[0]) : nullptr;
    kdmap_update(ctx, rel, d, d ? n : 0, nullptr, 0, 0, -1);
    PLS_CUDA(cudaStreamSynchronize(ctx->stream));
    PLS_API_END(ctx)
}

int pls_kdmap_set_points(pls_context* ctx, const void* xyz, int is_f64, int64_t n) {
    PLS_API_BEGIN(ctx)
    PLS_REQUIRE(ctx->cfg.local_map_type == PLS_MAP_KDTREE, "context holds a projective map");
    PLS_REQUIRE(n >= 0 && (xyz || n == 0), "pls_kdmap_set_points: points must be [n,3] with n >= 0");
    PLS_REQUIRE(n < (1ll << 30), "kd map: too many points");
    sync_all(ctx);
    cudaStream_t st = ctx->stream;
    const size_t elem = is_f64 ? sizeof(double) : sizeof(float);
    const void* d = n > 0 ? to_device(ctx, xyz, (size_t)n * 3 * elem, ctx->stage_in[0]) : nullptr;
    if (n > 0) {
        uint32_t* bad = scalar_u32(ctx, SC_SPARE0);
        PLS_CUDA(cudaMemsetAsync(bad, 0, sizeof(uint32_t), st));
        const int g = grid_for(n, 256, 8 * kNumSMs);
        if (is_f64) kd_nonfinite_rows_kernel<double><<<g, 256, 0, st>>>((const double*)d, n, bad);
        else kd_nonfinite_rows_kernel<float><<<g, 256, 0, st>>>((const float*)d, n, bad);
        PLS_CHECK_LAUNCH();
        uint32_t nbad = 0;
        PLS_CUDA(cudaMemcpyAsync(&nbad, bad, sizeof(nbad), cudaMemcpyDeviceToHost, st));
        PLS_CUDA(cudaStreamSynchronize(st));
        PLS_REQUIRE(nbad == 0, "pls_kdmap_set_points: the cloud has rows with a NaN or infinite coordinate, which the "
                               "kd map cannot search");
    }
    kdmap_reset(ctx);
    if (n > 0) {
        ctx->tmp[4].reserve((size_t)n * sizeof(float4), st);
        if (is_f64) pack_valid_rows_f64(ctx, (const double*)d, n, ctx->tmp[4].as<float4>(), scalar_u32(ctx, SC_INSERT_COUNT));
        else pack_valid_rows(ctx, (const float*)d, n, ctx->tmp[4].as<float4>(), scalar_u32(ctx, SC_INSERT_COUNT));
    }
    kdmap_update_packed(ctx, nullptr, ctx->tmp[4].as<float4>(), n, true);
    ctx->kd.frame_counts.clear();
    ctx->kd.max_frame = 0;
    PLS_CUDA(cudaStreamSynchronize(st));
    PLS_API_END(ctx)
}

int pls_kdmap_frames(pls_context* ctx, int64_t* out_counts, int* out_num) {
    PLS_API_BEGIN(ctx)
    PLS_REQUIRE(out_num, "pls_kdmap_frames: null output");
    const std::deque<int64_t>& fc = ctx->kd.frame_counts;
    *out_num = (int)fc.size();
    if (out_counts)
        for (size_t i = 0; i < fc.size(); ++i) out_counts[i] = fc[i];
    PLS_API_END(ctx)
}

int pls_kdmap_update_vertex_map(pls_context* ctx, const float* rel_pose, const float* vertex_map, int height, int width) {
    PLS_API_BEGIN(ctx)
    map_stream_wait(ctx);
    PLS_REQUIRE(rel_pose && vertex_map && height > 0 && width > 0, "pls_kdmap_update_vertex_map: bad arguments");
    PLS_REQUIRE(ctx->cfg.local_map_type == PLS_MAP_KDTREE, "context holds a projective map");
    float rel[16];
    if (is_device_ptr(rel_pose)) PLS_CUDA(cudaMemcpy(rel, rel_pose, sizeof(rel), cudaMemcpyDeviceToHost));
    else memcpy(rel, rel_pose, sizeof(rel));
    const float* d = (const float*)to_device(ctx, vertex_map, (size_t)3 * height * width * sizeof(float), ctx->stage_in[0]);
    kdmap_update(ctx, rel, nullptr, 0, d, height, width, -1);
    PLS_CUDA(cudaStreamSynchronize(ctx->stream));
    PLS_API_END(ctx)
}

int pls_kdmap_stats(pls_context* ctx, unsigned long long* out16) {
    PLS_API_BEGIN(ctx)
    PLS_REQUIRE(out16, "pls_kdmap_stats: null output");
    memset(out16, 0, 16 * sizeof(unsigned long long));
    if (ctx->kd.stats.p) {
        PLS_CUDA(cudaMemcpyAsync(out16, ctx->kd.stats.p, 16 * sizeof(unsigned long long), cudaMemcpyDeviceToHost, ctx->stream));
        PLS_CUDA(cudaStreamSynchronize(ctx->stream));
    }
    PLS_API_END(ctx)
}

int pls_kdmap_size(pls_context* ctx, int64_t* num_points) {
    PLS_API_BEGIN(ctx)
    PLS_REQUIRE(num_points, "pls_kdmap_size: null output");
    *num_points = ctx->kd.count;
    PLS_API_END(ctx)
}

int pls_kdmap_points(pls_context* ctx, float* out) {
    PLS_API_BEGIN(ctx)
    map_stream_wait(ctx);
    PLS_REQUIRE(out, "pls_kdmap_points: null output");
    const int64_t M = ctx->kd.count;
    if (M > 0) {
        OutArg o = out_arg(ctx, out, (size_t)M * 3 * sizeof(float), ctx->stage_out[0]);
        kd_export_kernel<<<grid_for(M, 256, 8 * kNumSMs), 256, 0, ctx->stream>>>(ctx->kd.store[ctx->kd.cur].as<float4>(), M,
                                                                                 (float*)o.dev);
        PLS_CHECK_LAUNCH();
        finish_out(ctx, o);
        PLS_CUDA(cudaStreamSynchronize(ctx->stream));
    }
    PLS_API_END(ctx)
}

int pls_kdmap_nn_search(pls_context* ctx, const float* queries, int64_t n, float* out_neighbors, float* out_normals,
                        int64_t* out_idx) {
    PLS_API_BEGIN(ctx)
    map_stream_wait(ctx);
    PLS_REQUIRE(queries && out_neighbors && n > 0, "pls_kdmap_nn_search: bad arguments");
    if (!ctx->kd.valid) throw pls::Error{PLS_E_STATE, "pls_kdmap_nn_search: the map is empty"};
    const float* d = (const float*)to_device(ctx, queries, (size_t)n * 3 * sizeof(float), ctx->stage_in[0]);
    OutArg onb = out_arg(ctx, out_neighbors, (size_t)n * 3 * sizeof(float), ctx->stage_out[0]);
    OutArg onr = out_arg(ctx, out_normals, (size_t)n * 3 * sizeof(float), ctx->stage_out[1]);
    OutArg oix = out_arg(ctx, out_idx, (size_t)n * sizeof(int64_t), ctx->stage_out[2]);
    cudaStream_t st = ctx->stream;
    ctx->queries.reserve((size_t)n * sizeof(float4), st);
    ctx->tmp[6].reserve(16 * sizeof(float) + 16, st);
    static const float eye12[12] = {1, 0, 0, 0, 0, 1, 0, 0, 0, 0, 1, 0};
    PLS_CUDA(cudaMemcpyAsync(ctx->tmp[6].p, eye12, sizeof(eye12), cudaMemcpyHostToDevice, st));
    uint32_t* nq = scalar_u32(ctx, SC_QUERY_COUNT);
    const uint32_t nq_host[3] = {(uint32_t)n, 0u, 0u};
    PLS_CUDA(cudaMemcpyAsync(nq, nq_host, sizeof(uint32_t), cudaMemcpyHostToDevice, st));
    PLS_CUDA(cudaMemsetAsync(scalar_u32(ctx, SC_KD_LISTS), 0, 8 * sizeof(uint32_t), st));
    kd_rows_to_float4_kernel<<<grid_for(n, 256, 8 * kNumSMs), 256, 0, st>>>(d, n, ctx->queries.as<float4>());
    PLS_CHECK_LAUNCH();
    const KdIndex ix = make_index(ctx);
    const KdPlan plan = plan_kd_iteration(ctx, n, 1);
    launch_search(ctx, plan, ix, ctx->queries.as<float4>(), nq, 0, 1, ctx->tmp[6].as<float>(), nullptr, ctx->nn_prev.as<int>(),
                  true, out_normals != nullptr, 0);
    record_search(ctx->kd, false, false, out_normals != nullptr, n);
    kd_search_export_kernel<<<grid_for(n, 256, 8 * kNumSMs), 256, 0, st>>>(ix, ctx->nn_prev.as<int>(), n, (float*)onb.dev,
                                                                            (float*)onr.dev, (long long*)oix.dev);
    PLS_CHECK_LAUNCH();
    finish_out(ctx, onb);
    finish_out(ctx, onr);
    finish_out(ctx, oix);
    PLS_CUDA(cudaStreamSynchronize(ctx->stream));
    PLS_API_END(ctx)
}

int pls_kdmap_knn(pls_context* ctx, const float* queries, int64_t n, int k, int64_t* out_idx, float* out_d2,
                  int32_t* out_pos) {
    PLS_API_BEGIN(ctx)
    map_stream_wait(ctx);
    PLS_REQUIRE(queries && out_idx && out_d2 && n > 0, "pls_kdmap_knn: bad arguments");
    PLS_REQUIRE(k >= 0 && k + 1 <= KD_KMAX_WIDE, "pls_kdmap_knn: k must be in [0, 255]");
    if (!ctx->kd.valid) throw pls::Error{PLS_E_STATE, "pls_kdmap_knn: the map is empty"};
    const int K = k + 1;
    const size_t entries = (size_t)n * K;
    const float* d = (const float*)to_device(ctx, queries, (size_t)n * 3 * sizeof(float), ctx->stage_in[0]);
    OutArg oix = out_arg(ctx, out_idx, entries * sizeof(int64_t), ctx->stage_out[0]);
    OutArg od2 = out_arg(ctx, out_d2, entries * sizeof(float), ctx->stage_out[1]);
    OutArg ops = out_arg(ctx, out_pos, entries * sizeof(int32_t), ctx->stage_out[2]);
    const int blocks = grid_for(n, KD_THREADS / 32, 8 * kNumSMs);
    const KdIndex ix = make_index(ctx);
    long long* pi = (long long*)oix.dev;
    float* pd = (float*)od2.dev;
    int* pp = (int*)ops.dev;
    cudaStream_t st = ctx->stream;
    if (K <= KD_KMAX) kd_knn_export_kernel<<<blocks, KD_THREADS, 0, st>>>(ix, d, n, K, pi, pd, pp);
    else if (kd_wide_regs(K) == 2) kd_knn_wide_export_kernel<2><<<blocks, KD_THREADS, 0, st>>>(ix, d, n, K, pi, pd, pp);
    else if (kd_wide_regs(K) == 4) kd_knn_wide_export_kernel<4><<<blocks, KD_THREADS, 0, st>>>(ix, d, n, K, pi, pd, pp);
    else kd_knn_wide_export_kernel<8><<<blocks, KD_THREADS, 0, st>>>(ix, d, n, K, pi, pd, pp);
    PLS_CHECK_LAUNCH();
    finish_out(ctx, oix);
    finish_out(ctx, od2);
    finish_out(ctx, ops);
    PLS_CUDA(cudaStreamSynchronize(ctx->stream));
    PLS_API_END(ctx)
}

int pls_kdmap_last_correspondences(pls_context* ctx, int64_t n, int64_t* out_idx, float* out_neighbors, float* out_normals,
                                   float* out_search_state, double* out_sums) {
    PLS_API_BEGIN_FRAME(ctx)
    const KdMap& kd = ctx->kd;
    if (!kd.searched) throw pls::Error{PLS_E_STATE, "pls_kdmap_last_correspondences: no kd search has run"};
    if (!kd.valid || kd.searched_gen != kd.gen)
        throw pls::Error{PLS_E_STATE, "pls_kdmap_last_correspondences: the map was rebuilt since the last search"};
    if (kd.searched_sharded)
        throw pls::Error{PLS_E_STATE, "pls_kdmap_last_correspondences: the last ICP split its queries over the ranks"};
    cudaStream_t st = ctx->stream;
    int64_t count = kd.searched_n;
    if (kd.searched_icp) {
        long long c = 0;
        PLS_CUDA(cudaMemcpyAsync(&c, &frame_result_dev(ctx)->counts[1], sizeof(c), cudaMemcpyDeviceToHost, st));
        PLS_CUDA(cudaStreamSynchronize(st));
        count = (int64_t)c;
    }
    PLS_REQUIRE(n == count, "pls_kdmap_last_correspondences: n must be the query count of the last search");
    if (n > 0 && (out_idx || out_neighbors || out_normals)) {
        OutArg onb = out_arg(ctx, out_neighbors, (size_t)n * 3 * sizeof(float), ctx->stage_out[0]);
        OutArg onr = out_arg(ctx, out_normals, (size_t)n * 3 * sizeof(float), ctx->stage_out[1]);
        OutArg oix = out_arg(ctx, out_idx, (size_t)n * sizeof(int64_t), ctx->stage_out[2]);
        float* nb = (float*)onb.dev;
        if (!nb) {
            ctx->stage_out[3].reserve((size_t)n * 3 * sizeof(float), st);
            nb = ctx->stage_out[3].as<float>();
        }
        kd_search_export_kernel<<<grid_for(n, 256, 8 * kNumSMs), 256, 0, st>>>(
            make_index(ctx), ctx->nn_prev.as<int>(), n, nb, kd.searched_normals ? (float*)onr.dev : nullptr,
            (long long*)oix.dev);
        PLS_CHECK_LAUNCH();
        if (onr.dev && !kd.searched_normals)
            PLS_CUDA(cudaMemsetAsync(onr.dev, 0xff, onr.bytes, st));
        finish_out(ctx, onb);
        finish_out(ctx, onr);
        finish_out(ctx, oix);
    }
    if (n > 0 && out_search_state)
        PLS_CUDA(cudaMemcpyAsync(out_search_state, ctx->kd_nn_state.p, (size_t)n * sizeof(float4), cudaMemcpyDefault, st));
    if (out_sums) {
        if (kd.searched_icp) {
            PLS_CUDA(cudaMemcpyAsync(out_sums, frame_result_dev(ctx)->last_sums, NACC * sizeof(double), cudaMemcpyDefault, st));
        } else {
            PLS_CUDA(cudaStreamSynchronize(st));
            if (is_device_ptr(out_sums)) PLS_CUDA(cudaMemsetAsync(out_sums, 0xff, NACC * sizeof(double), st));
            else memset(out_sums, 0xff, NACC * sizeof(double));
        }
    }
    PLS_CUDA(cudaStreamSynchronize(st));
    PLS_API_END(ctx)
}

#ifdef PLS_KD_SPLIT
PLS_API int pls_debug_kd_split(pls_context* ctx, unsigned long long* out, int64_t words) {
    PLS_API_BEGIN(ctx)
    PLS_REQUIRE(out && words == (int64_t)KD_SPLIT_WORDS + 1, "pls_debug_kd_split: bad arguments");
    sync_all(ctx);
    PLS_CUDA(cudaMemcpyFromSymbol(out, g_kd_split, KD_SPLIT_WORDS * sizeof(unsigned long long)));
    PLS_CUDA(cudaMemcpyFromSymbol(out + KD_SPLIT_WORDS, g_kd_split_normals_end, sizeof(unsigned long long)));
    static const unsigned long long zero = 0;
    void* p = nullptr;
    PLS_CUDA(cudaGetSymbolAddress(&p, g_kd_split));
    PLS_CUDA(cudaMemset(p, 0, KD_SPLIT_WORDS * sizeof(unsigned long long)));
    PLS_CUDA(cudaMemcpyToSymbol(g_kd_split_normals_end, &zero, sizeof(zero)));
    PLS_API_END(ctx)
}
#endif

}
```

### pylidar_slam_b200/csrc/odometry.cu

```cuda
#include <stdlib.h>

#include <chrono>
#include <utility>
#include <vector>

#include "internal.cuh"
#include "icp_device.cuh"
#include "pose_device.cuh"
#include "projection_device.cuh"
#include "select_device.cuh"

namespace pls {

int projmap_icp_iteration(pls_context* ctx, int64_t query_bound, int rank, int num_ranks);
int comm_rank(pls_context* ctx);
int comm_size(pls_context* ctx);
bool comm_is_p2p(pls_context* ctx);
void* comm_p2p_peers(pls_context* ctx);
unsigned long long* comm_p2p_seq(pls_context* ctx);
double* comm_allreduce_buffer(pls_context* ctx);

namespace {

int64_t g_shard_min_override = -1;
int64_t shard_min_default() {
    static const int64_t v = getenv("PLS_SHARD_MIN") ? atoll(getenv("PLS_SHARD_MIN")) : 24576;
    return v;
}

struct Pose16 {
    float m[16];
};

__device__ __forceinline__ void frame_begin_body(FrameResult* fr, const float* T0_dev , const Pose16& T0,
                                                 uint32_t* worklist_counts , int queries_are_rows) {
    int t = threadIdx.x;
    if (t < 16) worklist_counts[t] = 0;
    if (t < 16) fr->T[t] = T0_dev ? T0_dev[t] : T0.m[t];
    uint32_t* cw = reinterpret_cast<uint32_t*>(fr->counts);
    static_assert(sizeof(fr->counts) == 16 * sizeof(uint32_t), "counts: 8 words of 64 bits");
    if (t < 16 && t != 2 && t != 4) cw[t] = 0u;
    if (t == 2 && queries_are_rows) cw[2] = cw[4];
    if (t < 6) fr->params[t] = 0.f;
    if (t < kMaxAlign) fr->losses[t] = __int_as_float(0x7fc00000);
    if (t == 0) {
        fr->iters = 0;
        fr->status = 0;
        fr->done = 0;
        fr->pad = 0;
    }
    if (t < NACC) fr->last_sums[t] = 0.0;
}

__global__ void frame_begin_kernel(FrameResult* fr, const float* T0_dev , Pose16 T0, int max_iters,
                                   uint32_t* worklist_counts , int queries_are_rows) {
    frame_begin_body(fr, T0_dev, T0, worklist_counts, queries_are_rows);
}

__global__ void hypotheses_begin_kernel(FrameResult* frs, const float* __restrict__ T0s, uint32_t* words) {
    frame_begin_body(frs + blockIdx.x, T0s + 16 * blockIdx.x, Pose16{}, words + 16 * blockIdx.x, 0);
}


__global__ void __launch_bounds__(256) reduce_partials_kernel(const FrameResult* fr, const double* __restrict__ partials,
                                                              int num_blocks, double* __restrict__ out) {
    if (fr->done) return;
    __shared__ double sums[NACC];
    sum_partials_256(partials, num_blocks, sums);
    __syncthreads();
    if (threadIdx.x < NACC) out[threadIdx.x] = sums[threadIdx.x];
}

__global__ void __launch_bounds__(256) icp_step_kernel(FrameResult* fr, const double* __restrict__ partials,
                                                       int num_blocks, const double* __restrict__ reduced, float threshold_delta) {
    icp_step_body(fr, partials, num_blocks, reduced, threshold_delta);
}

struct P2PSlot {
    double sums[NACC];
    unsigned long long seq;
    unsigned long long pad;
};
static_assert(sizeof(P2PSlot) == 256, "P2PSlot must match comm.cu's kP2PSlotBytes");
__global__ void __launch_bounds__(256)
icp_step_p2p_kernel(FrameResult* fr, const double* __restrict__ partials, int num_blocks, float threshold_delta,
                    P2PSlot* const* __restrict__ peers, int world, int rank, unsigned long long* seq_counter) {
    if (fr->done) return;
    __shared__ double sums[NACC];
    __shared__ int timed_out;
    __shared__ unsigned long long s_seq;
    if (threadIdx.x == 0) {
        timed_out = 0;
        s_seq = ++(*seq_counter);
    }
    sum_partials_256(partials, num_blocks, sums);
    __syncthreads();
    const unsigned long long seq = s_seq;
    const int parity = (int)(seq & 1ull);
    if (threadIdx.x < NACC)
        for (int r = 0; r < world; ++r) peers[r][parity * world + rank].sums[threadIdx.x] = sums[threadIdx.x];
    __threadfence_system();
    __syncthreads();
    if (threadIdx.x < world) {
        volatile unsigned long long* flag = &peers[threadIdx.x][parity * world + rank].seq;
        *flag = seq;
    }
    if (threadIdx.x < world) {
        volatile unsigned long long* mine = &peers[rank][parity * world + threadIdx.x].seq;
        const long long t0 = clock64();
        while (*mine < seq) {
            if (clock64() - t0 > 6000000000ll) {
                timed_out = 1;
                break;
            }
        }
    }
    __threadfence_system();
    __syncthreads();
    if (timed_out) {
        if (threadIdx.x == 0) {
            fr->status = PLS_E_COMM;
            fr->done = 1;
        }
        return;
    }
    if (threadIdx.x < NACC) {
        double s = 0.0;
        for (int r = 0; r < world; ++r) s += __ldcv(&peers[rank][parity * world + r].sums[threadIdx.x]);
        sums[threadIdx.x] = s;
        fr->last_sums[threadIdx.x] = s;
    }
    __syncthreads();
    if (threadIdx.x != 0) return;
    icp_solve_and_update(fr, sums, threshold_delta);
}

__global__ void scrub_vertex_map_kernel(const float* __restrict__ in, int64_t hw, float* __restrict__ out) {
    for (int64_t i = (int64_t)blockIdx.x * blockDim.x + threadIdx.x; i < hw; i += (int64_t)gridDim.x * blockDim.x) {
        float x = in[i], y = in[hw + i], z = in[2 * hw + i];
        bool bad = !(x == x) || !(y == y) || !(z == z);
        out[i] = bad ? 0.f : x;
        out[hw + i] = bad ? 0.f : y;
        out[2 * hw + i] = bad ? 0.f : z;
    }
}

__global__ void first_point_kernel(const float4* __restrict__ packed, const uint32_t* __restrict__ count,
                                   float4* __restrict__ out, uint32_t* __restrict__ out_count, FrameResult* fr) {
    if (threadIdx.x == 0) {
        uint32_t c = *count;
        if (c > 0) {
            out[0] = packed[0];
            fr->first_pt[0] = packed[0].x; fr->first_pt[1] = packed[0].y; fr->first_pt[2] = packed[0].z;
        }
        *out_count = c > 0 ? 1u : 0u;
    }
}

struct FrameInputSelect {
    const float* pts;
    ProjConst pc;
    unsigned long long* zbuf;
    float4* frame_pts;
    float4* queries;
    struct State {
        float x, y, z;
        int pix;
    };
    __device__ __forceinline__ uint32_t flags(int64_t i, State& s) const {
        s.x = pts[3 * i];
        s.y = pts[3 * i + 1];
        s.z = pts[3 * i + 2];
        s.pix = -1;
        const bool valid = s.x == s.x && s.y == s.y && s.z == s.z;
        if (!valid) return 0u;
        uint32_t f = 1u;
        if (zbuf) {
            int pix;
            float r;
            if (project_to_pixel(s.x, s.y, s.z, pc, pix, r) &&
                zbuf[pix] == (((unsigned long long)__float_as_uint(r) << 32) | (unsigned long long)(uint32_t)i)) {
                s.pix = pix;
                f |= 2u;
            }
        }
        return f;
    }
    __device__ __forceinline__ void emit(int64_t, int which, uint32_t pos, const State& s) const {
        if (which == 0) {
            frame_pts[pos] = make_float4(s.x, s.y, s.z, 0.f);
        } else {
            queries[pos] = make_float4(s.x, s.y, s.z, 0.f);
            zbuf[s.pix] = ~0ull;
        }
    }
};

}

bool icp_shards(pls_context* ctx, int64_t work) {
    const int size = comm_size(ctx);
    int64_t shard_min = g_shard_min_override >= 0 ? g_shard_min_override : shard_min_default();
    if (g_shard_min_override < 0 && ctx->cfg.local_map_type == PLS_MAP_KDTREE && ctx->kd.indexed >= 2000000) shard_min /= 3;
    return size > 1 && work / size >= shard_min;
}

namespace {

inline int grid_for(int64_t n, int threads = 256) {
    int64_t b = (n + threads - 1) / threads;
    int64_t cap = 8 * kNumSMs;
    return (int)(b < 1 ? 1 : (b > cap ? cap : b));
}

uint32_t* count_slot(pls_context* ctx, int i) { return reinterpret_cast<uint32_t*>(&frame_result_dev(ctx)->counts[i]); }

int enqueue_icp_iterations(pls_context* ctx, int64_t query_bound, const uint32_t* bound_dev, int first, int last) {
    cudaStream_t st = ctx->stream;
    FrameResult* fr = frame_result_dev(ctx);
    int rank = comm_rank(ctx), size = comm_size(ctx);
    if (size > 1) {
        PLS_REQUIRE(!bound_dev, "ICP: a device-side query bound cannot decide the sharding");
        const int64_t work = ctx->cfg.local_map_type == PLS_MAP_KDTREE ? query_bound : (int64_t)ctx->cfg.height * ctx->cfg.width;
        if (!icp_shards(ctx, work)) {
            rank = 0;
            size = 1;
        }
    }
    ctx->last_sharded = size > 1;
    int last_blocks = 0;
    for (int it = first; it < last; ++it) {
        int blocks;
        bool solved = false;
        if (ctx->cfg.local_map_type == PLS_MAP_KDTREE)
            blocks = kdmap_icp_iteration(ctx, query_bound, bound_dev, rank, size, it,
                                         size == 1 ? ctx->cfg.threshold_delta_pose : -1.f, &solved);
        else
            blocks = projmap_icp_iteration(ctx, query_bound, rank, size);
        last_blocks = blocks;
        if (solved) continue;
        if (size > 1 && comm_is_p2p(ctx)) {
            icp_step_p2p_kernel<<<1, 256, 0, st>>>(fr, ctx->partials.as<double>(), blocks, ctx->cfg.threshold_delta_pose,
                                                   (P2PSlot* const*)comm_p2p_peers(ctx), size, rank, comm_p2p_seq(ctx));
            PLS_CHECK_LAUNCH();
            continue;
        }
        const double* reduced = nullptr;
        if (size > 1) {
            double* buf = comm_allreduce_buffer(ctx);
            reduce_partials_kernel<<<1, 256, 0, st>>>(fr, ctx->partials.as<double>(), blocks, buf);
            PLS_CHECK_LAUNCH();
            comm_allreduce_sums(ctx, buf);
            reduced = buf;
            blocks = 0;
        }
        icp_step_kernel<<<1, 256, 0, st>>>(fr, ctx->partials.as<double>(), blocks, reduced, ctx->cfg.threshold_delta_pose);
        PLS_CHECK_LAUNCH();
    }
    return last_blocks;
}

struct HostTrace {
    bool on = getenv("PLS_HOST_TRACE") != nullptr;
    double acc[4] = {0, 0, 0, 0};
    int frames = 0, extra_rounds = 0;
    std::chrono::steady_clock::time_point t;
    void start() { if (on) t = std::chrono::steady_clock::now(); }
    void lap(int k) {
        if (!on) return;
        const auto now = std::chrono::steady_clock::now();
        acc[k] += std::chrono::duration<double, std::micro>(now - t).count();
        t = now;
    }
    void end_frame() {
        if (!on || ++frames < 64) return;
        fprintf(stderr, "[plslam_b200 host trace] per frame: enqueue input+ICP %.1f us, wait for the pose %.1f us, "
                        "map-update enqueue %.1f us, rest %.1f us; %d of %d frames needed a second round of ICP launches\n",
                acc[0] / frames, acc[1] / frames, acc[2] / frames, acc[3] / frames, extra_rounds, frames);
        frames = 0;
        extra_rounds = 0;
        acc[0] = acc[1] = acc[2] = acc[3] = 0;
    }
};
HostTrace g_trace;

struct BatchTrace {
    const char* path = nullptr;
    cudaEvent_t ev[3] = {nullptr, nullptr, nullptr};
    std::chrono::steady_clock::time_point t_call, t_epi;
    int sequences = 0, icp_sequences = 0, extra_rounds = 0;
    void begin(cudaStream_t st) {
        path = getenv("PLS_BATCH_TRACE");
        if (!path) return;
        t_call = std::chrono::steady_clock::now();
        for (auto& e : ev) PLS_CUDA(cudaEventCreate(&e));
        PLS_CUDA(cudaEventRecord(ev[0], st));
    }
    void inputs_done(cudaStream_t st, int num, int icp) {
        sequences = num;
        icp_sequences = icp;
        if (path) PLS_CUDA(cudaEventRecord(ev[1], st));
    }
    void icp_done(cudaStream_t st) {
        if (path) PLS_CUDA(cudaEventRecord(ev[2], st));
    }
    void epilogue_begin() {
        if (path) t_epi = std::chrono::steady_clock::now();
    }
    void end() {
        if (!path) return;
        const auto now = std::chrono::steady_clock::now();
        float input_ms = 0.f, icp_ms = 0.f;
        PLS_CUDA(cudaEventSynchronize(ev[1]));
        PLS_CUDA(cudaEventElapsedTime(&input_ms, ev[0], ev[1]));
        if (icp_sequences > 0) PLS_CUDA(cudaEventElapsedTime(&icp_ms, ev[1], ev[2]));
        FILE* f = fopen(path, "a");
        if (!f) return;
        fprintf(f, "{\"sequences\": %d, \"icp_sequences\": %d, \"input_ms\": %.6f, \"icp_ms\": %.6f, \"epilogue_ms\": %.6f, "
                   "\"call_ms\": %.6f, \"extra_rounds\": %d}\n",
                sequences, icp_sequences, input_ms, icp_ms,
                std::chrono::duration<double, std::milli>(now - t_epi).count(),
                std::chrono::duration<double, std::milli>(now - t_call).count(), extra_rounds);
        fclose(f);
    }
    ~BatchTrace() {
        for (auto e : ev)
            if (e) cudaEventDestroy(e);
    }
};

void frame_begin(pls_context* ctx, const float* T0_host, const float* T0_dev, bool queries_are_rows) {
    Pose16 T0;
    for (int i = 0; i < 16; ++i) T0.m[i] = T0_host ? T0_host[i] : ((i % 5 == 0) ? 1.f : 0.f);
    frame_begin_kernel<<<1, kMaxAlign, 0, ctx->stream>>>(frame_result_dev(ctx), T0_dev, T0, ctx->cfg.max_num_alignments,
                                                         scalar_u32(ctx, SC_KD_COUNTERS), queries_are_rows ? 1 : 0);
    PLS_CHECK_LAUNCH();
}

template <typename Enqueue, typename ReadDone>
int icp_rounds(pls_context* const* ctxs, int num, Enqueue enqueue, ReadDone read_done) {
    int upfront = 0, max_it = 0;
    for (int j = 0; j < num; ++j) {
        const int last = ctxs[j]->last_icp_iters, m = ctxs[j]->cfg.max_num_alignments;
        const int u = last > 0 && last + 1 < m ? last + 1 : m;
        upfront = u > upfront ? u : upfront;
        max_it = m > max_it ? m : max_it;
    }
    enqueue(0, upfront);
    int enq = upfront, extra = 0;
    int done[PLS_MAX_SEQUENCES];
    while (enq < max_it) {
        read_done(done);
        bool more = false;
        for (int j = 0; j < num; ++j) more = more || (!done[j] && enq < ctxs[j]->cfg.max_num_alignments);
        if (!more) break;
        const int k = (max_it - enq) < 4 ? (max_it - enq) : 4;
        enqueue(enq, enq + k);
        enq += k;
        extra += 1;
    }
    return extra;
}

int run_icp(pls_context* ctx, int64_t query_bound, const uint32_t* bound_dev) {
    cudaStream_t st = ctx->stream;
    FrameResult* fr = frame_result_dev(ctx);
    if (query_bound < 1) query_bound = 1;
    ctx->pm.zbuf_clean = false;
    int blocks = 0;
    auto enqueue = [&](int first, int last) {
        blocks = enqueue_icp_iterations(ctx, query_bound, bound_dev, first, last);
        if (first == 0) g_trace.lap(0);
    };
    auto read_done = [&](int* done) {
        int flags[3];
        PLS_CUDA(cudaMemcpyAsync(flags, &fr->iters, sizeof(flags), cudaMemcpyDeviceToHost, st));
        PLS_CUDA(cudaStreamSynchronize(st));
        done[0] = flags[2];
    };
    g_trace.extra_rounds += icp_rounds(&ctx, 1, enqueue, read_done);
    return blocks;
}

void enqueue_result_copy(pls_context* ctx, cudaStream_t st) {
    PLS_CUDA(cudaMemcpyAsync(ctx->pinned.p, ctx->scalars.p, kScalarOffset + SC_NUM * sizeof(uint32_t), cudaMemcpyDeviceToHost,
                             st));
}

void fetch_result(pls_context* ctx) {
    enqueue_result_copy(ctx, ctx->stream);
    PLS_CUDA(cudaStreamSynchronize(ctx->stream));
}

void credit_icp_profile(pls_context* ctx, const FrameResult* h, int blocks) {
    if (ctx->cfg.local_map_type == PLS_MAP_KDTREE) {
        const unsigned long long* kc = reinterpret_cast<const unsigned long long*>(
            reinterpret_cast<const char*>(h) + kScalarOffset + SC_KD_COUNTERS * sizeof(uint32_t));
        const double iters = (double)h->iters, nq = (double)h->counts[1] / (ctx->last_sharded ? (double)comm_size(ctx) : 1.0);
        const double bytes = iters * nq * (12.0 + 27.0 * 8.0 + 4.0) + 16.0 * (double)kc[0]
                             + 32.0 * (double)kc[2] + 16.0 * (double)kc[1]
                             + iters * (nq * 36.0 + (double)blocks * NACC * 8.0);
        profile_credit(ctx, 0, h->iters, bytes);
    } else {
        const double share = ctx->last_sharded ? 1.0 / (double)comm_size(ctx) : 1.0;
        const double hw = (double)ctx->cfg.height * ctx->cfg.width * share;
        profile_credit(ctx, 1, h->iters, (double)h->iters * (hw * 12.0 * (ctx->pm.K + 1) + h->last_sums[29] * share * 12.0 +
                                                              (double)blocks * NACC * 8.0));
    }
}

void raise_status(pls_context* ctx, int status) {
    if (status == PLS_E_COMM) throw pls::Error{PLS_E_COMM, "peer-to-peer all-reduce timed out waiting for a peer rank"};
    if (status == PLS_E_SINGULAR) throw pls::Error{PLS_E_SINGULAR, "Invalid Jacobian in Gauss Newton minimization"};
}

bool keyframe_decision(pls_context* ctx, const float* T) {
    float nd[16], prm[6];
    mat4_mul(ctx->delta_since_update, T, nd);
    from_pose(nd, prm);
    const float tn = sqrtf(prm[0] * prm[0] + prm[1] * prm[1] + prm[2] * prm[2]);
    const float rn = sqrtf(prm[3] * prm[3] + prm[4] * prm[4] + prm[5] * prm[5]);
    const bool insert = tn > ctx->cfg.threshold_trans || rn * 180.0f / 3.14159265358979323846f > ctx->cfg.threshold_rot;
    if (insert) {
        for (int i = 0; i < 16; ++i) ctx->delta_since_update[i] = (i % 5 == 0) ? 1.f : 0.f;
    } else {
        memcpy(ctx->delta_since_update, nd, sizeof(nd));
    }
    return insert;
}

}

void flush_map_update(pls_context* ctx) {
    if (!ctx->upd_pending) return;
    ctx->upd_pending = false;
    const bool kd = ctx->cfg.local_map_type == PLS_MAP_KDTREE;
    DBuf& frame_vmap = ctx->frame_vmap_buf[ctx->upd_slot];
    DBuf& frame_pts = ctx->frame_pts_buf[ctx->upd_slot];
    map_stream_begin(ctx);
    try {
        if (kd) {
            if (ctx->upd_insert) kdmap_update_packed(ctx, ctx->upd_T, frame_pts.as<float4>(), (int64_t)ctx->upd_count, true);
            else kdmap_update_packed(ctx, ctx->upd_T, nullptr, 0, false);
        } else {
            projmap_update(ctx, ctx->upd_T, ctx->upd_insert ? frame_vmap.as<float>() : nullptr);
        }
    } catch (...) {
        map_stream_end(ctx);
        throw;
    }
    map_stream_end(ctx);
}

namespace {

struct FrameIn {
    int64_t pts_bound = 0;
    int64_t query_bound = 0;
    const uint32_t* n_dev = nullptr;
};

struct FrameOut {
    float* pose;
    float* params;
    int* has_pose;
    double* info;
    int64_t samples;
    void put_samples() const {
        if (info && samples >= 0) info[4] = (double)samples;
    }
};

const char* frame_refusal(const pls_context* ctx, int layout, int64_t n, double voxel) {
    if (ctx->cfg.gn_max_iters != 1) return "fused ICP path supports gauss_newton_config.max_iters == 1";
    if (layout < 0) return nullptr;
    if (layout < PLS_INPUT_NDARRAY || layout > PLS_INPUT_TENSOR_F64) return "process_frame: unknown layout";
    if (voxel > 0.0 && layout != PLS_INPUT_NDARRAY && layout != PLS_INPUT_TENSOR) return "grid-sampled input is a point layout";
    if (layout != PLS_INPUT_VERTEX_MAP && n <= 0) return "process_frame: empty point cloud";
    return nullptr;
}

const void* stage_frame_input(pls_context* ctx, const void* data, int* layout, int64_t n) {
    const int hint = *layout & (PLS_PTR_DEVICE | PLS_PTR_HOST);
    *layout &= ~(PLS_PTR_DEVICE | PLS_PTR_HOST);
    const bool is64 = *layout == PLS_INPUT_NDARRAY_F64 || *layout == PLS_INPUT_TENSOR_F64;
    const size_t bytes = *layout == PLS_INPUT_VERTEX_MAP ? (size_t)3 * ctx->cfg.height * ctx->cfg.width * sizeof(float)
                                                         : (size_t)n * 3 * (is64 ? sizeof(double) : sizeof(float));
    if (hint == PLS_PTR_DEVICE) return data;
    if (hint != PLS_PTR_HOST) return to_device(ctx, data, bytes, ctx->stage_in[0]);
    ctx->stage_in[0].reserve(bytes, ctx->stream);
    PLS_CUDA(cudaMemcpyAsync(ctx->stage_in[0].p, data, bytes, cudaMemcpyHostToDevice, ctx->stream));
    return ctx->stage_in[0].p;
}

GridSample frame_grid_sample(pls_context* ctx, const void* raw, int64_t n, double voxel) {
    ctx->gs_out_xyz.reserve((size_t)n * 3 * sizeof(float), ctx->stream);
    return GridSample{raw, false, n, voxel, ctx->gs_out_xyz.p, nullptr, nullptr, nullptr};
}

bool frame_input(pls_context* ctx, const void* data_void, int layout, int64_t n, const uint32_t* n_dev,
                 const float* init_pose, FrameIn& in, const FrameOut& out) {
    cudaStream_t st = ctx->stream;
    const bool is64 = layout == PLS_INPUT_NDARRAY_F64 || layout == PLS_INPUT_TENSOR_F64;
    if (layout == PLS_INPUT_NDARRAY_F64) layout = PLS_INPUT_NDARRAY;
    if (layout == PLS_INPUT_TENSOR_F64) layout = PLS_INPUT_TENSOR;
    const float* data_dev = is64 ? nullptr : (const float*)data_void;
    const double* data64 = is64 ? (const double*)data_void : nullptr;
    const int H = ctx->cfg.height, W = ctx->cfg.width;
    const int64_t hw = (int64_t)H * W;
    const bool kd = ctx->cfg.local_map_type == PLS_MAP_KDTREE;
    FrameResult* fr = frame_result_dev(ctx);
    if (layout == PLS_INPUT_NDARRAY) ctx->sample_pointcloud = 1;
    const bool first = ctx->frame_index == 0;
    ctx->frame_slot ^= 1;
    DBuf& frame_vmap = ctx->frame_vmap_buf[ctx->frame_slot];
    DBuf& frame_pts = ctx->frame_pts_buf[ctx->frame_slot];

    frame_vmap.reserve((size_t)3 * hw * sizeof(float), st);
    int64_t pts_bound = 0;
    bool fused_input = false;
    if (layout == PLS_INPUT_VERTEX_MAP) {
        scrub_vertex_map_kernel<<<grid_for(hw), 256, 0, st>>>(data_dev, hw, frame_vmap.as<float>());
        PLS_CHECK_LAUNCH();
        ctx->tmp[5].reserve((size_t)hw * sizeof(float4), st);
        pack_valid_pixels(ctx, frame_vmap.as<float>(), hw, 0.f, ctx->tmp[5].as<float4>(), count_slot(ctx, 1));
        frame_pts.reserve(sizeof(float4) * 4, st);
        first_point_kernel<<<1, 32, 0, st>>>(ctx->tmp[5].as<float4>(), count_slot(ctx, 1), frame_pts.as<float4>(),
                                              count_slot(ctx, 2), fr);
        PLS_CHECK_LAUNCH();
        pts_bound = 1;
    } else {
        PLS_REQUIRE(n > 0, "process_frame: empty point cloud");
        frame_pts.reserve((size_t)n * sizeof(float4), st);
        pts_bound = n;
        fused_input = !is64 && kd && !first && n <= SEL_MAX_N && n < (1ll << 32);
        PLS_REQUIRE(fused_input || !n_dev, "process_frame: a device-side row count needs the fused kd input stage");
        if (fused_input) {
            const bool pixel_queries = !ctx->sample_pointcloud;
            FrameInputSelect op;
            op.pts = data_dev;
            op.pc = make_proj_const(H, W, ctx->cfg.up_fov_deg, ctx->cfg.down_fov_deg);
            op.zbuf = nullptr;
            op.frame_pts = frame_pts.as<float4>();
            op.queries = nullptr;
            if (pixel_queries) {
                if (ctx->input_zbuf.cap < (size_t)hw * sizeof(unsigned long long)) ctx->input_zbuf_clean = false;
                ctx->input_zbuf.reserve((size_t)hw * sizeof(unsigned long long), st);
                if (!ctx->input_zbuf_clean)
                    PLS_CUDA(cudaMemsetAsync(ctx->input_zbuf.p, 0xff, (size_t)hw * sizeof(unsigned long long), st));
                ctx->input_zbuf_clean = false;
                ctx->queries.reserve((size_t)(n < hw ? n : hw) * sizeof(float4), st);
                launch_zbuf_points(ctx, data_dev, n, n_dev, H, W, ctx->cfg.up_fov_deg, ctx->cfg.down_fov_deg,
                                   ctx->input_zbuf.as<unsigned long long>());
                op.zbuf = ctx->input_zbuf.as<unsigned long long>();
                op.queries = ctx->queries.as<float4>();
            }
            select_launch(ctx, op, n, n_dev, count_slot(ctx, 2), pixel_queries ? count_slot(ctx, 1) : nullptr);
            if (pixel_queries) ctx->input_zbuf_clean = true;
        } else if (is64) {
            pack_valid_rows_f64(ctx, data64, n, frame_pts.as<float4>(), count_slot(ctx, 2));
        } else {
            pack_valid_rows(ctx, data_dev, n, frame_pts.as<float4>(), count_slot(ctx, 2));
        }
        if (!fused_input && (first || !ctx->sample_pointcloud || !kd)) {
            ctx->tmp[3].reserve((size_t)hw * sizeof(unsigned long long), st);
            if (is64)
                launch_projection_f64(ctx, data64, n, H, W, ctx->cfg.up_fov_deg, ctx->cfg.down_fov_deg, frame_vmap.as<float>(),
                                      ctx->tmp[3].as<unsigned long long>());
            else
                launch_projection(ctx, data_dev, nullptr, 1, n, 3, H, W, ctx->cfg.up_fov_deg, ctx->cfg.down_fov_deg,
                                  frame_vmap.as<float>(), ctx->tmp[3].as<unsigned long long>());
        }
    }
    in.pts_bound = pts_bound;
    in.n_dev = n_dev;

    float eye[16];
    for (int i = 0; i < 16; ++i) eye[i] = (i % 5 == 0) ? 1.f : 0.f;

    if (first) {
        flush_map_update(ctx);
        map_stream_wait(ctx);
        if (kd) kdmap_update(ctx, eye, nullptr, 0, frame_vmap.as<float>(), H, W, -1);
        else projmap_update(ctx, eye, frame_vmap.as<float>());
        ctx->frame_index = 1;
        if (out.has_pose) *out.has_pose = 0;
        if (out.pose) memcpy(out.pose, eye, sizeof(eye));
        if (out.params) memset(out.params, 0, 6 * sizeof(float));
        fetch_result(ctx);
        if (out.info) {
            FrameResult* h = frame_result_host(ctx);
            for (int i = 0; i < 12; ++i) out.info[i] = 0.0;
            out.info[3] = (double)ctx->kd.count;
            out.info[5] = (double)(pts_bound - (int64_t)h->counts[2]);
        }
        out.put_samples();
        return false;
    }

    int64_t query_bound;
    const bool queries_are_rows = ctx->sample_pointcloud && layout != PLS_INPUT_VERTEX_MAP;
    if (queries_are_rows) {
        ctx->query_ptr = frame_pts.as<float4>();
        query_bound = n;
    } else if (layout == PLS_INPUT_VERTEX_MAP) {
        ctx->query_ptr = ctx->tmp[5].as<float4>();
        query_bound = hw;
    } else if (fused_input) {
        ctx->query_ptr = ctx->queries.as<float4>();
        query_bound = n < hw ? n : hw;
    } else {
        ctx->queries.reserve((size_t)hw * sizeof(float4), st);
        pack_valid_pixels(ctx, frame_vmap.as<float>(), hw, 0.f, ctx->queries.as<float4>(), count_slot(ctx, 1));
        ctx->query_ptr = ctx->queries.as<float4>();
        query_bound = n < hw ? n : hw;
    }
    in.query_bound = query_bound;

    flush_map_update(ctx);
    map_stream_wait(ctx);
    frame_begin(ctx, init_pose, nullptr, queries_are_rows);
    return true;
}

void frame_epilogue(pls_context* ctx, const FrameIn& in, const FrameOut& out, bool trace) {
    FrameResult* h = frame_result_host(ctx);
    ctx->last_icp_iters = h->iters;
    raise_status(ctx, h->status);

    const bool insert = keyframe_decision(ctx, h->T);
    ctx->upd_pending = true;
    ctx->upd_insert = insert;
    memcpy(ctx->upd_T, h->T, sizeof(ctx->upd_T));
    ctx->upd_slot = ctx->frame_slot;
    ctx->upd_count = (long long)h->counts[2];
    if (trace) g_trace.lap(2);
    ctx->frame_index += 1;
    if (out.pose) memcpy(out.pose, h->T, 16 * sizeof(float));
    if (out.params) memcpy(out.params, h->params, 6 * sizeof(float));
    if (out.has_pose) *out.has_pose = 1;
    if (out.info) {
        out.info[0] = (double)h->iters;
        out.info[1] = h->iters > 0 ? (double)h->losses[h->iters - 1] : 0.0;
        out.info[2] = (double)h->counts[1];
        out.info[3] = (double)ctx->kd.count;
        out.info[4] = (double)h->counts[0];
        out.info[5] = (double)(in.pts_bound - (int64_t)h->counts[2]);
        out.info[6] = (double)h->status;
        out.info[7] = insert ? 1.0 : 0.0;
        out.info[8] = h->first_pt[0]; out.info[9] = h->first_pt[1]; out.info[10] = h->first_pt[2];
        out.info[11] = ctx->last_sharded ? 1.0 : 0.0;
    }
    out.put_samples();
}

bool process_frame_device(pls_context* ctx, const void* data_void, int layout, int64_t n, const uint32_t* n_dev,
                          const float* init_pose, FrameOut out) {
    g_trace.start();
    FrameIn in;
    if (!frame_input(ctx, data_void, layout, n, n_dev, init_pose, in, out)) return true;
    int icp_blocks = run_icp(ctx, in.query_bound, in.n_dev);
    fetch_result(ctx);
    g_trace.lap(1);
    if (in.n_dev) {
        bool overflowed = false;
        const int64_t rows = grid_sample_host_count(ctx, &overflowed);
        if (overflowed) return false;
        in.pts_bound = rows;
        out.samples = rows;
        const int64_t q = rows < in.query_bound ? rows : in.query_bound;
        icp_blocks = grid_for(q < 1 ? 1 : q);
    }
    ctx->icp_result = true;
    credit_icp_profile(ctx, frame_result_host(ctx), icp_blocks);
    frame_epilogue(ctx, in, out, true);
    g_trace.lap(3);
    g_trace.end_frame();
    return true;
}

struct FrameEntryState {
    int frame_slot, frame_index, last_icp_iters;
    bool input_zbuf_clean;
    explicit FrameEntryState(const pls_context* ctx)
        : frame_slot(ctx->frame_slot), frame_index(ctx->frame_index), last_icp_iters(ctx->last_icp_iters),
          input_zbuf_clean(ctx->input_zbuf_clean) {}
    void restore(pls_context* ctx) const {
        ctx->frame_slot = frame_slot;
        ctx->frame_index = frame_index;
        ctx->last_icp_iters = last_icp_iters;
        ctx->input_zbuf_clean = input_zbuf_clean;
    }
};

}

void odometry_reset(pls_context* ctx) {
    kdmap_reset(ctx);
    projmap_reset(ctx);
    ctx->frame_index = 0;
    ctx->last_icp_iters = 0;
    for (int i = 0; i < 16; ++i) ctx->delta_since_update[i] = (i % 5 == 0) ? 1.f : 0.f;
}

static void register_batch(pls_context* ctx, const KdScan* scans, int64_t n, const float* T0_dev, int B, float* out_T,
                           float* out_params, float* out_losses, int* out_iters, int* out_status) {
    const bool kd = ctx->cfg.local_map_type == PLS_MAP_KDTREE;
    cudaStream_t st = ctx->stream;
    const int M = ctx->cfg.max_num_alignments;
    std::vector<FrameResult> h((size_t)PLS_MAX_SEQUENCES);
    std::vector<float> T((size_t)B * 16), params((size_t)B * 6), losses((size_t)B * M);
    std::vector<int> iters((size_t)B), status((size_t)B);
    int first_error = PLS_OK, last = 0;
    for (int c0 = 0; c0 < B; c0 += PLS_MAX_SEQUENCES) {
        const int num = B - c0 < PLS_MAX_SEQUENCES ? B - c0 : PLS_MAX_SEQUENCES;
        int grid[KD_BATCH_GRID];
        FrameResult* frs = nullptr;
        uint32_t* words = nullptr;
        if (kd) kdmap_hypotheses_begin(ctx, scans + c0, num, st, grid, &frs, &words);
        else projmap_hypotheses_begin(ctx, num, st, &frs, &words);
        hypotheses_begin_kernel<<<num, kMaxAlign, 0, st>>>(frs, T0_dev + 16 * (size_t)c0, words);
        PLS_CHECK_LAUNCH();
        std::vector<pls_context*> same((size_t)num, ctx);
        if (kd)
            icp_rounds(same.data(), num, [&](int a, int b) { kdmap_batch_iterations(ctx, num, st, grid, a, b); },
                       [&](int* done) { kdmap_batch_done(ctx, num, st, done); });
        else
            icp_rounds(same.data(), num, [&](int a, int b) { projmap_hypotheses_iterations(ctx, n, num, st, a, b); },
                       [&](int* done) { projmap_batch_done(ctx, num, st, done); });
        PLS_CUDA(cudaMemcpyAsync(h.data(), frs, (size_t)num * sizeof(FrameResult), cudaMemcpyDeviceToHost, st));
        PLS_CUDA(cudaStreamSynchronize(st));
        for (int j = 0; j < num; ++j) {
            const FrameResult& r = h[(size_t)j];
            const size_t b = (size_t)(c0 + j);
            memcpy(&T[16 * b], r.T, 16 * sizeof(float));
            memcpy(&params[6 * b], r.params, 6 * sizeof(float));
            memcpy(&losses[(size_t)M * b], r.losses, (size_t)M * sizeof(float));
            iters[b] = r.iters;
            status[b] = r.status;
            if (first_error == PLS_OK && (r.status == PLS_E_SINGULAR || r.status == PLS_E_COMM)) first_error = r.status;
        }
        last = num - 1;
    }
    if (kd) kdmap_hypothesis_adopt(ctx, scans[B - 1], last, st);
    else projmap_hypothesis_adopt(ctx, last, st);
    fetch_result(ctx);
    ctx->icp_result = true;
    auto put = [&](void* dst, const void* src, size_t bytes) {
        if (!dst) return;
        if (is_device_ptr(dst)) PLS_CUDA(cudaMemcpy(dst, src, bytes, cudaMemcpyHostToDevice));
        else memcpy(dst, src, bytes);
    };
    put(out_T, T.data(), T.size() * sizeof(float));
    put(out_params, params.data(), params.size() * sizeof(float));
    put(out_losses, losses.data(), losses.size() * sizeof(float));
    put(out_iters, iters.data(), iters.size() * sizeof(int));
    put(out_status, status.data(), status.size() * sizeof(int));
    if (!out_status) raise_status(ctx, first_error);
}

}

using namespace pls;

extern "C" {

int pls_map_init(pls_context* ctx) {
    PLS_API_BEGIN(ctx)
    sync_all(ctx);
    kdmap_reset(ctx);
    projmap_reset(ctx);
    PLS_API_END(ctx)
}

int pls_set_shard_min(int64_t work_items_per_rank) {
    g_shard_min_override = work_items_per_rank;
    return PLS_OK;
}

int pls_last_sharded(pls_context* ctx, int* out) {
    PLS_API_BEGIN(ctx)
    PLS_REQUIRE(out, "pls_last_sharded: null output");
    *out = ctx->last_sharded ? 1 : 0;
    PLS_API_END(ctx)
}

int pls_odometry_init(pls_context* ctx) {
    PLS_API_BEGIN(ctx)
    sync_all(ctx);
    odometry_reset(ctx);
    PLS_API_END(ctx)
}

int pls_register_frame(pls_context* ctx, const float* points, int64_t n, const float* T0, float* out_T,
                       float* out_params, float* out_losses, int* out_iters) {
    PLS_API_BEGIN(ctx)
    PLS_REQUIRE(points && n > 0, "pls_register_frame: points must be [n,3] with n > 0");
    PLS_REQUIRE(ctx->cfg.gn_max_iters == 1, "fused ICP path supports gauss_newton_config.max_iters == 1");
    cudaStream_t st = ctx->stream;
    map_stream_wait(ctx);
    const float* d = (const float*)to_device(ctx, points, (size_t)n * 3 * sizeof(float), ctx->stage_in[0]);
    FrameResult* fr = frame_result_dev(ctx);
    PLS_CUDA(cudaMemsetAsync(fr->counts, 0, sizeof(fr->counts), st));
    ctx->queries.reserve((size_t)n * sizeof(float4), st);
    pack_valid_rows(ctx, d, n, ctx->queries.as<float4>(), count_slot(ctx, 1));
    ctx->query_ptr = ctx->queries.as<float4>();
    const float* T0_dev = nullptr;
    if (T0) {
        ctx->tmp[6].reserve(16 * sizeof(float), st);
        PLS_CUDA(cudaMemcpyAsync(ctx->tmp[6].p, T0, 16 * sizeof(float),
                                 is_device_ptr(T0) ? cudaMemcpyDeviceToDevice : cudaMemcpyHostToDevice, st));
        T0_dev = ctx->tmp[6].as<float>();
    }
    frame_begin(ctx, nullptr, T0_dev, false);
    const int icp_blocks = run_icp(ctx, n, nullptr);
    fetch_result(ctx);
    ctx->icp_result = true;
    FrameResult* h = frame_result_host(ctx);
    credit_icp_profile(ctx, h, icp_blocks);
    auto put = [&](void* dst, const void* src, size_t bytes) {
        if (!dst) return;
        if (is_device_ptr(dst)) PLS_CUDA(cudaMemcpy(dst, src, bytes, cudaMemcpyHostToDevice));
        else memcpy(dst, src, bytes);
    };
    put(out_T, h->T, 16 * sizeof(float));
    put(out_params, h->params, 6 * sizeof(float));
    put(out_losses, h->losses, (size_t)ctx->cfg.max_num_alignments * sizeof(float));
    if (out_iters) *out_iters = h->iters;
    raise_status(ctx, h->status);
    PLS_API_END(ctx)
}

int pls_register_hypotheses(pls_context* ctx, const float* points, int64_t n, const float* T0s, int B, float* out_T,
                            float* out_params, float* out_losses, int* out_iters, int* out_status) {
    PLS_API_BEGIN(ctx)
    PLS_REQUIRE(points && n > 0, "pls_register_hypotheses: points must be [n,3] with n > 0");
    PLS_REQUIRE(T0s && B > 0, "pls_register_hypotheses: T0s must be [B,16] with B > 0");
    PLS_REQUIRE(ctx->cfg.gn_max_iters == 1, "fused ICP path supports gauss_newton_config.max_iters == 1");
    const bool kd = ctx->cfg.local_map_type == PLS_MAP_KDTREE;
    PLS_REQUIRE(!ctx->comm, "pls_register_hypotheses: a context with a multi-GPU communicator is not supported");
    if (kd) PLS_REQUIRE(ctx->kd.valid, "kd map: search before any update");
    else PLS_REQUIRE(ctx->pm.valid, "projective map: search before any update");
    cudaStream_t st = ctx->stream;
    map_stream_wait(ctx);
    const float* d = (const float*)to_device(ctx, points, (size_t)n * 3 * sizeof(float), ctx->stage_in[0]);
    const float* T0_dev = (const float*)to_device(ctx, T0s, (size_t)B * 16 * sizeof(float), ctx->stage_in[1]);
    FrameResult* fr = frame_result_dev(ctx);
    PLS_CUDA(cudaMemsetAsync(fr->counts, 0, sizeof(fr->counts), st));
    ctx->queries.reserve((size_t)n * sizeof(float4), st);
    pack_valid_rows(ctx, d, n, ctx->queries.as<float4>(), count_slot(ctx, 1));
    ctx->query_ptr = ctx->queries.as<float4>();
    const std::vector<KdScan> scans(kd ? (size_t)B : 0, KdScan{ctx->query_ptr, count_slot(ctx, 1), n});
    register_batch(ctx, scans.data(), n, T0_dev, B, out_T, out_params, out_losses, out_iters, out_status);
    PLS_API_END(ctx)
}

int pls_register_scans(pls_context* ctx, const float* const* scans, const int64_t* n, int S, const int* scan_of,
                       const float* T0s, int B, float* out_T, float* out_params, float* out_losses, int* out_iters,
                       int* out_status) {
    PLS_API_BEGIN(ctx)
    PLS_REQUIRE(ctx->cfg.local_map_type == PLS_MAP_KDTREE, "pls_register_scans: needs a kd-tree local map");
    PLS_REQUIRE(ctx->cfg.gn_max_iters == 1, "fused ICP path supports gauss_newton_config.max_iters == 1");
    PLS_REQUIRE(!ctx->comm, "pls_register_scans: a context with a multi-GPU communicator is not supported");
    PLS_REQUIRE(ctx->kd.valid, "kd map: search before any update");
    PLS_REQUIRE(scans && n && S > 0, "pls_register_scans: scans and n must hold S > 0 scans");
    PLS_REQUIRE(T0s && B > 0, "pls_register_scans: T0s must be [B,16] with B > 0");
    PLS_REQUIRE(scan_of || B == S, "pls_register_scans: without scan_of, B must equal S");
    for (int s = 0; s < S; ++s) PLS_REQUIRE(scans[s] && n[s] > 0, "pls_register_scans: every scan must be [n,3] with n > 0");
    for (int b = 0; scan_of && b < B; ++b)
        PLS_REQUIRE(scan_of[b] >= 0 && scan_of[b] < S, "pls_register_scans: scan_of entries must lie in [0, S)");
    cudaStream_t st = ctx->stream;
    map_stream_wait(ctx);
    size_t host_rows = 0;
    for (int s = 0; s < S; ++s)
        if (!is_device_ptr(scans[s])) host_rows += (size_t)n[s];
    if (host_rows) ctx->stage_in[0].reserve(host_rows * 3 * sizeof(float), st);
    size_t rows = 0;
    for (int s = 0; s < S; ++s) rows += (size_t)n[s];
    ctx->queries.reserve(rows * sizeof(float4) + (size_t)S * sizeof(uint32_t), st);
    float4* q = ctx->queries.as<float4>();
    uint32_t* counts = reinterpret_cast<uint32_t*>(q + rows);
    std::vector<KdScanRows> pack((size_t)S);
    std::vector<KdScan> packed((size_t)S);
    float* staged = ctx->stage_in[0].as<float>();
    for (int s = 0; s < S; ++s) {
        const float* d = scans[s];
        if (!is_device_ptr(d)) {
            PLS_CUDA(cudaMemcpyAsync(staged, d, (size_t)n[s] * 3 * sizeof(float), cudaMemcpyHostToDevice, st));
            d = staged;
            staged += (size_t)n[s] * 3;
        }
        pack[(size_t)s] = KdScanRows{d, n[s], q, counts + s};
        packed[(size_t)s] = KdScan{q, counts + s, n[s]};
        q += n[s];
    }
    const float* T0_dev = (const float*)to_device(ctx, T0s, (size_t)B * 16 * sizeof(float), ctx->stage_in[1]);
    FrameResult* fr = frame_result_dev(ctx);
    PLS_CUDA(cudaMemsetAsync(fr->counts, 0, sizeof(fr->counts), st));
    pack_valid_scans(ctx, pack);
    std::vector<KdScan> regs((size_t)B);
    for (int b = 0; b < B; ++b) regs[(size_t)b] = packed[(size_t)(scan_of ? scan_of[b] : b)];
    register_batch(ctx, regs.data(), 0, T0_dev, B, out_T, out_params, out_losses, out_iters, out_status);
    PLS_API_END(ctx)
}

int pls_process_frame(pls_context* ctx, const void* data, int layout, int64_t n, const float* init_pose,
                      float* out_pose, float* out_params, int* out_has_pose, double* out_info) {
    PLS_API_BEGIN(ctx)
    PLS_REQUIRE(data, "pls_process_frame: null data");
    if (const char* why = frame_refusal(ctx, layout & ~(PLS_PTR_DEVICE | PLS_PTR_HOST), n, 0.0))
        throw pls::Error{PLS_E_INVALID, why};
    const void* d = stage_frame_input(ctx, data, &layout, n);
    process_frame_device(ctx, d, layout, n, nullptr, init_pose, FrameOut{out_pose, out_params, out_has_pose, out_info, -1});
    PLS_API_END(ctx)
}

int pls_process_frame_grid_sample(pls_context* ctx, const float* raw_points, int64_t n, double voxel, int layout,
                                  const float* init_pose, float* out_pose, float* out_params, int* out_has_pose,
                                  double* out_info) {
    PLS_API_BEGIN(ctx)
    PLS_REQUIRE(raw_points && n > 0 && voxel > 0.0, "pls_process_frame_grid_sample: bad arguments");
    if (const char* why = frame_refusal(ctx, layout, n, voxel)) throw pls::Error{PLS_E_INVALID, why};
    const void* d = to_device(ctx, raw_points, (size_t)n * 3 * sizeof(float), ctx->stage_in[0]);
    const GridSample g = frame_grid_sample(ctx, d, n, voxel);
    const FrameOut out{out_pose, out_params, out_has_pose, out_info, -1};
    const bool deferred = ctx->frame_index > 0 && ctx->cfg.local_map_type == PLS_MAP_KDTREE && comm_size(ctx) == 1 &&
                          n <= SEL_MAX_N;
    if (deferred) {
        const FrameEntryState entry(ctx);
        grid_sample_enqueue(ctx, g, false);
        if (process_frame_device(ctx, ctx->gs_out_xyz.p, layout, n, scalar_u32(ctx, SC_GS_COUNT), init_pose, out)) return PLS_OK;
        entry.restore(ctx);
    } else {
        grid_sample_enqueue(ctx, g);
        PLS_CUDA(cudaStreamSynchronize(ctx->stream));
    }
    const int64_t S = grid_sample_finish(ctx, g);
    FrameOut sized = out;
    sized.samples = S;
    process_frame_device(ctx, ctx->gs_out_xyz.p, layout, S, nullptr, init_pose, sized);
    PLS_API_END(ctx)
}

int pls_last_icp_sums(pls_context* ctx, double* out_sums, int* out_iters) {
    PLS_API_BEGIN_FRAME(ctx)
    PLS_REQUIRE(out_sums, "pls_last_icp_sums: null output");
    if (!ctx->icp_result) throw pls::Error{PLS_E_STATE, "pls_last_icp_sums: no ICP frame has run on this context"};
    const FrameResult* h = frame_result_host(ctx);
    memcpy(out_sums, h->last_sums, NACC * sizeof(double));
    if (out_iters) *out_iters = h->iters;
    PLS_API_END(ctx)
}

int pls_process_frames(pls_context* const* ctxs, int num, const void* const* data, const int* layouts, const int64_t* n,
                       double voxel, const float* const* init_poses, float* out_poses, float* out_params, int* out_has_pose,
                       double* out_info, int* out_status) {
    const char* why = nullptr;
    if (!ctxs || num < 0 || num > PLS_MAX_SEQUENCES) why = "pls_process_frames: need 0 <= num <= PLS_MAX_SEQUENCES contexts";
    else if (num > 0 && (!data || !layouts || !n)) why = "pls_process_frames: data, layouts and n are required";
    for (int i = 0; !why && i < num; ++i) {
        const pls_context* c = ctxs[i];
        if (!c) { why = "pls_process_frames: null context"; break; }
        if (c->cfg.local_map_type != ctxs[0]->cfg.local_map_type)
            why = "pls_process_frames: batched sequences share one local map type: all kd-tree or all projective";
        else if (c->comm) why = "pls_process_frames: a context with a multi-GPU communicator cannot be batched";
        else if (c->cfg.device != ctxs[0]->cfg.device) why = "pls_process_frames: every context must be on one device";
        for (int j = 0; !why && j < i; ++j)
            if (ctxs[j] == c) why = "pls_process_frames: a context is listed twice";
        if (!why) why = frame_refusal(c, data[i] ? layouts[i] & ~(PLS_PTR_DEVICE | PLS_PTR_HOST) : -1, n[i], voxel);
    }
    if (why) {
        for (int i = 0; ctxs && i < num; ++i)
            if (ctxs[i]) ctxs[i]->err = why;
        return PLS_E_INVALID;
    }
    std::vector<int> active;
    for (int i = 0; i < num; ++i)
        if (data[i]) active.push_back(i);
    for (int i = 0; i < num; ++i)
        if (out_status) out_status[i] = PLS_OK;
    if (active.empty()) return PLS_OK;

    struct ProfileOff {
        std::vector<std::pair<pls_context*, int>> off;
        ~ProfileOff() {
            for (auto& o : off) o.first->prof[o.second].enabled = true;
        }
    } prof_off;
    for (int i : active)
        for (int w = 0; w < kProfileSlots; ++w)
            if (ctxs[i]->prof[w].enabled) {
                ctxs[i]->prof[w].enabled = false;
                prof_off.off.push_back({ctxs[i], w});
            }

    pls_context* lead = ctxs[active[0]];
    int cur = active[0];
    std::vector<int> status((size_t)num, PLS_OK);
    std::vector<char> finished((size_t)num, 0);
    for (int i = 0; i < num; ++i) finished[i] = data[i] == nullptr;
    BatchTrace trace;
    try {
        PLS_CUDA(cudaSetDevice(lead->cfg.device));
        const cudaStream_t st = lead->stream;
        trace.begin(st);
        auto order_before_lead = [&](pls_context* ctx) {
            if (ctx == lead) return;
            if (!ctx->ev_batch) PLS_CUDA(cudaEventCreateWithFlags(&ctx->ev_batch, cudaEventDisableTiming));
            PLS_CUDA(cudaEventRecord(ctx->ev_batch, ctx->stream));
            PLS_CUDA(cudaStreamWaitEvent(st, ctx->ev_batch, 0));
        };
        std::vector<const void*> dev((size_t)num, nullptr);
        std::vector<int64_t> rows(n, n + num);
        std::vector<int> lay(layouts, layouts + num);
        std::vector<GridSample> gs((size_t)num);
        for (int i : active) {
            cur = i;
            pls_context* ctx = ctxs[i];
            flush_map_update(ctx);
            dev[i] = stage_frame_input(ctx, data[i], &lay[i], n[i]);
            if (voxel > 0.0) {
                gs[i] = frame_grid_sample(ctx, dev[i], n[i], voxel);
                grid_sample_enqueue(ctx, gs[i]);
                order_before_lead(ctx);
            }
        }
        if (voxel > 0.0) {
            PLS_CUDA(cudaStreamSynchronize(st));
            for (int i : active) {
                cur = i;
                rows[i] = grid_sample_finish(ctxs[i], gs[i]);
                dev[i] = ctxs[i]->gs_out_xyz.p;
            }
        }
        std::vector<FrameIn> in((size_t)num);
        std::vector<pls_context*> icp;
        std::vector<int> icp_seq;
        std::vector<int64_t> bounds;
        auto outputs = [&](int i) {
            return FrameOut{out_poses ? out_poses + 16 * i : nullptr, out_params ? out_params + 6 * i : nullptr,
                            out_has_pose ? out_has_pose + i : nullptr, out_info ? out_info + 12 * i : nullptr,
                            voxel > 0.0 ? rows[i] : -1};
        };
        for (int i : active) {
            cur = i;
            pls_context* ctx = ctxs[i];
            bool runs_icp = false;
            try {
                runs_icp = frame_input(ctx, dev[i], lay[i], rows[i], nullptr, init_poses ? init_poses[i] : nullptr, in[i],
                                       outputs(i));
            } catch (const pls::Error& e) {
                if (e.code != PLS_E_INVALID) throw;
                ctx->err = e.msg;
                status[i] = e.code;
                finished[i] = 1;
                continue;
            }
            if (!runs_icp) {
                finished[i] = 1;
                continue;
            }
            ctx->pm.zbuf_clean = false;
            icp.push_back(ctx);
            icp_seq.push_back(i);
            bounds.push_back(in[i].query_bound < 1 ? 1 : in[i].query_bound);
            order_before_lead(ctx);
        }
        const int m = (int)icp.size();
        trace.inputs_done(st, (int)active.size(), m);
        if (m > 0) {
            cur = icp_seq[0];
            int grid[KD_BATCH_GRID];
            const bool kd = lead->cfg.local_map_type == PLS_MAP_KDTREE;
            if (kd) kdmap_batch_begin(lead, icp.data(), bounds.data(), m, st, grid);
            else projmap_batch_begin(lead, icp.data(), bounds.data(), m, st, grid);
            auto enqueue = [&](int first, int last) {
                if (kd) kdmap_batch_iterations(lead, m, st, grid, first, last);
                else projmap_batch_iterations(lead, icp.data(), bounds.data(), m, st, grid, first, last);
            };
            auto read_done = [&](int* done) {
                if (kd) kdmap_batch_done(lead, m, st, done);
                else projmap_batch_done(lead, m, st, done);
            };
            trace.extra_rounds += icp_rounds(icp.data(), m, enqueue, read_done);
            for (pls_context* ctx : icp) enqueue_result_copy(ctx, st);
            trace.icp_done(st);
            PLS_CUDA(cudaStreamSynchronize(st));
            for (pls_context* ctx : icp) ctx->icp_result = true;
        }
        trace.epilogue_begin();
        for (int j = 0; j < m; ++j) {
            const int i = icp_seq[j];
            cur = i;
            try {
                frame_epilogue(icp[j], in[i], outputs(i), false);
            } catch (const pls::Error& e) {
                if (e.code != PLS_E_SINGULAR) throw;
                icp[j]->err = e.msg;
                status[i] = e.code;
            }
            finished[i] = 1;
        }
        trace.end();
    } catch (...) {
        int code = PLS_E_INVALID;
        std::string msg;
        try {
            throw;
        } catch (const pls::Error& e) {
            code = e.code;
            msg = e.msg;
        } catch (const std::exception& e) {
            msg = e.what();
        }
        for (int i = 0; i < num; ++i) {
            if (!finished[i]) {
                status[i] = code;
                ctxs[i]->err = msg;
            }
            if (out_status) out_status[i] = status[i];
        }
        return code;
    }
    int first_error = PLS_OK;
    for (int i = 0; i < num; ++i) {
        if (out_status) out_status[i] = status[i];
        if (first_error == PLS_OK) first_error = status[i];
    }
    return first_error;
}

}
```

### pylidar_slam_b200/csrc/primitives.cu

```cuda
#include "internal.cuh"

namespace pls {

namespace {

constexpr int SORT_THREADS = 256;
constexpr int SORT_WARPS = SORT_THREADS / 32;
constexpr int SORT_ITEMS = 8;
constexpr int SORT_TILE = SORT_THREADS * SORT_ITEMS;
constexpr int LOOKBACK = 8;
constexpr int RADIX = 256;
constexpr uint32_t FLAG_AGG = 1u << 30;
constexpr uint32_t FLAG_PREFIX = 2u << 30;
constexpr uint32_t VALUE_MASK = (1u << 30) - 1u;

__device__ __forceinline__ uint32_t ld_volatile_u32(const uint32_t* p) {
    uint32_t v;
    asm volatile("ld.volatile.global.u32 %0, [%1];" : "=r"(v) : "l"(p));
    return v;
}
__device__ __forceinline__ void st_volatile_u32(uint32_t* p, uint32_t v) {
    asm volatile("st.volatile.global.u32 [%0], %1;" ::"l"(p), "r"(v) : "memory");
}

__global__ void __launch_bounds__(256) sort_hist_kernel(const uint64_t* __restrict__ keys, int64_t n,
                                                        int num_passes, uint32_t* __restrict__ hist,
                                                        uint32_t* __restrict__ done_counter, uint32_t* __restrict__ status,
                                                        int64_t status_words) {
    __shared__ uint32_t sh[8 * RADIX];
    __shared__ int s_last;
    pls_grid_dependency_wait();
    for (int64_t i = (int64_t)blockIdx.x * blockDim.x + threadIdx.x; i < status_words; i += (int64_t)gridDim.x * blockDim.x)
        status[i] = 0u;
    for (int i = threadIdx.x; i < num_passes * RADIX; i += blockDim.x) sh[i] = 0;
    __syncthreads();
    for (int64_t i = (int64_t)blockIdx.x * blockDim.x + threadIdx.x; i < n; i += (int64_t)gridDim.x * blockDim.x) {
        const uint64_t k = keys[i];
        for (int p = 0; p < num_passes; ++p) atomicAdd(&sh[p * RADIX + (int)((k >> (8 * p)) & 255u)], 1u);
    }
    __syncthreads();
    for (int i = threadIdx.x; i < num_passes * RADIX; i += blockDim.x)
        if (sh[i]) atomicAdd(&hist[i], sh[i]);
    __threadfence();
    __syncthreads();
    if (threadIdx.x == 0) s_last = atomicAdd(done_counter, 1u) == gridDim.x - 1;
    __syncthreads();
    if (!s_last) return;
    __threadfence();
    const int t = threadIdx.x;
    for (int p = 0; p < num_passes; ++p) {
        uint32_t* h = hist + p * RADIX;
        const uint32_t v = __ldcg(h + t);
        __syncthreads();
        sh[t] = v;
        __syncthreads();
        for (int o = 1; o < RADIX; o <<= 1) {
            const uint32_t a = (t >= o) ? sh[t - o] : 0u;
            __syncthreads();
            sh[t] += a;
            __syncthreads();
        }
        h[t] = sh[t] - v;
    }
}

__global__ void __launch_bounds__(SORT_THREADS)
sort_pass_kernel(const uint64_t* __restrict__ kin, const uint32_t* __restrict__ vin, uint64_t* __restrict__ kout,
                 uint32_t* __restrict__ vout, int64_t n, int shift, const uint32_t* __restrict__ base,
                 uint32_t* status, uint32_t* tile_counter) {
    __shared__ uint32_t warp_hist[SORT_WARPS][RADIX];
    __shared__ uint32_t tile_offset[RADIX];
    __shared__ uint32_t s_tile;
    __shared__ uint32_t tile_start[RADIX];
    __shared__ uint32_t scan_warp[SORT_WARPS];
    __shared__ uint64_t s_keys[SORT_TILE];
    __shared__ uint32_t s_vals[SORT_TILE];
    const int tid = threadIdx.x, warp = tid >> 5, lane = tid & 31;
    pls_grid_dependency_wait();
    if (tid == 0) s_tile = atomicAdd(tile_counter, 1u);
    for (int i = tid; i < SORT_WARPS * RADIX; i += SORT_THREADS) (&warp_hist[0][0])[i] = 0;
    __syncthreads();
    const uint32_t tile = s_tile;
    const int64_t seg = (int64_t)tile * SORT_TILE + (int64_t)warp * (32 * SORT_ITEMS);
    const uint32_t lt_mask = (1u << lane) - 1u;

    uint64_t key[SORT_ITEMS];
    uint32_t val[SORT_ITEMS];
    uint32_t rank[SORT_ITEMS];
#pragma unroll
    for (int i = 0; i < SORT_ITEMS; ++i) {
        int64_t idx = seg + i * 32 + lane;
        bool valid = idx < n;
        key[i] = valid ? kin[idx] : 0ull;
        val[i] = valid ? vin[idx] : 0u;
    }
#pragma unroll
    for (int i = 0; i < SORT_ITEMS; ++i) {
        int64_t idx = seg + i * 32 + lane;
        bool valid = idx < n;
        uint32_t d = valid ? (uint32_t)((key[i] >> shift) & 255u) : 0xffffu;
        uint32_t peers = __match_any_sync(0xffffffffu, d);
        uint32_t pre = valid ? warp_hist[warp][d] : 0u;
        __syncwarp();
        if (valid && lane == (__ffs(peers) - 1)) warp_hist[warp][d] = pre + __popc(peers);
        __syncwarp();
        rank[i] = pre + __popc(peers & lt_mask);
    }
    __syncthreads();
    {
        const int d = tid;
        uint32_t sum = 0;
#pragma unroll
        for (int w = 0; w < SORT_WARPS; ++w) {
            uint32_t c = warp_hist[w][d];
            warp_hist[w][d] = sum;
            sum += c;
        }
        uint32_t excl = 0;
        uint32_t* st = status + (size_t)tile * RADIX + d;
        if (tile == 0) {
            st_volatile_u32(st, FLAG_PREFIX | sum);
        } else {
            st_volatile_u32(st, FLAG_AGG | sum);
            int64_t t = (int64_t)tile - 1;
            bool done = false;
            while (!done) {
                uint32_t s[LOOKBACK];
#pragma unroll
                for (int k = 0; k < LOOKBACK; ++k)
                    s[k] = (t - k >= 0) ? ld_volatile_u32(status + (size_t)(t - k) * RADIX + d) : FLAG_PREFIX;
#pragma unroll
                for (int k = 0; k < LOOKBACK; ++k) {
                    if (done || (s[k] >> 30) == 0u) break;
                    excl += s[k] & VALUE_MASK;
                    --t;
                    if (s[k] & FLAG_PREFIX) done = true;
                }
            }
            st_volatile_u32(st, FLAG_PREFIX | (excl + sum));
        }
        tile_offset[d] = base[d] + excl;
        uint32_t inc = sum;
#pragma unroll
        for (int o = 1; o < 32; o <<= 1) {
            const uint32_t v = __shfl_up_sync(0xffffffffu, inc, o);
            if (lane >= o) inc += v;
        }
        if (lane == 31) scan_warp[warp] = inc;
        __syncthreads();
        uint32_t before = 0;
#pragma unroll
        for (int w = 0; w < SORT_WARPS; ++w) before += (w < warp) ? scan_warp[w] : 0u;
        tile_start[d] = before + inc - sum;
    }
    __syncthreads();
#pragma unroll
    for (int i = 0; i < SORT_ITEMS; ++i) {
        int64_t idx = seg + i * 32 + lane;
        if (idx < n) {
            uint32_t d = (uint32_t)((key[i] >> shift) & 255u);
            uint32_t slot = tile_start[d] + warp_hist[warp][d] + rank[i];
            s_keys[slot] = key[i];
            s_vals[slot] = val[i];
        }
    }
    __syncthreads();
    const int64_t tile_base = (int64_t)tile * SORT_TILE;
    const int tile_n = (int)((n - tile_base) < (int64_t)SORT_TILE ? (n - tile_base) : (int64_t)SORT_TILE);
#pragma unroll
    for (int i = 0; i < SORT_ITEMS; ++i) {
        const int j = i * SORT_THREADS + tid;
        if (j < tile_n) {
            const uint64_t k = s_keys[j];
            const uint32_t d = (uint32_t)((k >> shift) & 255u);
            const uint32_t pos = tile_offset[d] + ((uint32_t)j - tile_start[d]);
            kout[pos] = k;
            vout[pos] = s_vals[j];
        }
    }
}

constexpr int SCAN_THREADS = 256;
constexpr int SCAN_ITEMS = 8;
constexpr int SCAN_TILE = SCAN_THREADS * SCAN_ITEMS;

__global__ void __launch_bounds__(SCAN_THREADS)
scan_flags_kernel(const uint8_t* __restrict__ flags, int64_t n, uint32_t* __restrict__ pos_out,
                  uint32_t* status, uint32_t* tile_counter, uint32_t* total_out) {
    __shared__ uint32_t warp_sums[SCAN_THREADS / 32];
    __shared__ uint32_t s_tile, s_excl;
    const int tid = threadIdx.x, warp = tid >> 5, lane = tid & 31;
    if (tid == 0) s_tile = atomicAdd(tile_counter, 1u);
    __syncthreads();
    const uint32_t tile = s_tile;
    const int64_t base = (int64_t)tile * SCAN_TILE + (int64_t)tid * SCAN_ITEMS;
    uint32_t f[SCAN_ITEMS];
    uint32_t local = 0;
#pragma unroll
    for (int i = 0; i < SCAN_ITEMS; ++i) {
        int64_t idx = base + i;
        f[i] = (idx < n && flags[idx]) ? 1u : 0u;
        local += f[i];
    }
    uint32_t inc = local;
#pragma unroll
    for (int o = 1; o < 32; o <<= 1) {
        uint32_t v = __shfl_up_sync(0xffffffffu, inc, o);
        if (lane >= o) inc += v;
    }
    if (lane == 31) warp_sums[warp] = inc;
    __syncthreads();
    if (warp == 0) {
        uint32_t w = (lane < SCAN_THREADS / 32) ? warp_sums[lane] : 0u;
        uint32_t winc = w;
#pragma unroll
        for (int o = 1; o < 32; o <<= 1) {
            uint32_t v = __shfl_up_sync(0xffffffffu, winc, o);
            if (lane >= o) winc += v;
        }
        if (lane < SCAN_THREADS / 32) warp_sums[lane] = winc - w;
        uint32_t tile_sum = __shfl_sync(0xffffffffu, winc, SCAN_THREADS / 32 - 1);
        if (lane == 0) {
            uint32_t excl = 0;
            if (tile == 0) {
                st_volatile_u32(status + tile, FLAG_PREFIX | tile_sum);
            } else {
                st_volatile_u32(status + tile, FLAG_AGG | tile_sum);
                int64_t t = (int64_t)tile - 1;
                bool done = false;
                while (!done) {
                    uint32_t s[LOOKBACK];
#pragma unroll
                    for (int k = 0; k < LOOKBACK; ++k) s[k] = (t - k >= 0) ? ld_volatile_u32(status + (t - k)) : FLAG_PREFIX;
#pragma unroll
                    for (int k = 0; k < LOOKBACK; ++k) {
                        if (done || (s[k] >> 30) == 0u) break;
                        excl += s[k] & VALUE_MASK;
                        --t;
                        if (s[k] & FLAG_PREFIX) done = true;
                    }
                }
                st_volatile_u32(status + tile, FLAG_PREFIX | (excl + tile_sum));
            }
            s_excl = excl;
            if ((int64_t)(tile + 1) * SCAN_TILE >= n) *total_out = excl + tile_sum;
        }
    }
    __syncthreads();
    uint32_t run = s_excl + warp_sums[warp] + (inc - local);
#pragma unroll
    for (int i = 0; i < SCAN_ITEMS; ++i) {
        int64_t idx = base + i;
        if (idx < n) pos_out[idx] = run;
        run += f[i];
    }
}

}

void radix_sort_pairs(pls_context* ctx, uint64_t* keys, uint32_t* vals, int64_t n, int num_passes,
                      uint64_t** keys_out, uint32_t** vals_out, int64_t cap_n) {
    PLS_REQUIRE(num_passes >= 1 && num_passes <= 8, "radix_sort_pairs: 1..8 passes");
    PLS_REQUIRE(n < (1ll << 30), "radix_sort_pairs: n must be < 2^30");
    SortScratch& s = ctx->sort;
    cudaStream_t st = ctx->stream;
    if (n <= 0) {
        *keys_out = keys;
        *vals_out = vals;
        return;
    }
    const int64_t tiles = (n + SORT_TILE - 1) / SORT_TILE;
    if (cap_n < n) cap_n = n;
    const int64_t cap_tiles = (cap_n + SORT_TILE - 1) / SORT_TILE;
    s.keys_alt.reserve(cap_n * sizeof(uint64_t), st);
    s.vals_alt.reserve(cap_n * sizeof(uint32_t), st);
    const size_t hist_bytes = (8 * RADIX + 1) * sizeof(uint32_t);
    const size_t status_words = (size_t)num_passes * tiles * RADIX + 8;
    s.hist.reserve(hist_bytes, st);
    s.status.reserve(((size_t)num_passes * cap_tiles * RADIX + 8) * sizeof(uint32_t), st);
    PLS_CUDA(cudaMemsetAsync(s.hist.p, 0, hist_bytes, st));
    int hist_blocks = (int)((n + 256 * 4 - 1) / (256 * 4));
    if (hist_blocks > kNumSMs) hist_blocks = kNumSMs;
    launch_dependent(sort_hist_kernel, hist_blocks, 256, st, keys, n, num_passes, s.hist.as<uint32_t>(),
                     s.hist.as<uint32_t>() + 8 * RADIX, s.status.as<uint32_t>(), (int64_t)status_words);
    uint64_t* kin = keys;
    uint32_t* vin = vals;
    uint64_t* kout = s.keys_alt.as<uint64_t>();
    uint32_t* vout = s.vals_alt.as<uint32_t>();
    uint32_t* counters = s.status.as<uint32_t>() + (size_t)num_passes * tiles * RADIX;
    for (int p = 0; p < num_passes; ++p) {
        launch_dependent(sort_pass_kernel, (unsigned)tiles, SORT_THREADS, st, kin, vin, kout, vout, n, 8 * p,
                         s.hist.as<uint32_t>() + p * RADIX, s.status.as<uint32_t>() + (size_t)p * tiles * RADIX, counters + p);
        uint64_t* tk = kin; kin = kout; kout = tk;
        uint32_t* tv = vin; vin = vout; vout = tv;
    }
    *keys_out = kin;
    *vals_out = vin;
}

void exclusive_scan_flags(pls_context* ctx, const uint8_t* flags, int64_t n, uint32_t* pos_out,
                          uint32_t* total_dev) {
    cudaStream_t st = ctx->stream;
    if (n <= 0) {
        PLS_CUDA(cudaMemsetAsync(total_dev, 0, sizeof(uint32_t), st));
        return;
    }
    PLS_REQUIRE(n < (1ll << 30), "exclusive_scan_flags: n must be < 2^30");
    const int64_t tiles = (n + SCAN_TILE - 1) / SCAN_TILE;
    ctx->scan.status.reserve((tiles + 4) * sizeof(uint32_t), st);
    PLS_CUDA(cudaMemsetAsync(ctx->scan.status.p, 0, (tiles + 4) * sizeof(uint32_t), st));
    uint32_t* status = ctx->scan.status.as<uint32_t>();
    scan_flags_kernel<<<(unsigned)tiles, SCAN_THREADS, 0, st>>>(flags, n, pos_out, status, status + tiles, total_dev);
    PLS_CHECK_LAUNCH();
}

}
```

Baseline: 2006.

## Decide kd-map update on device and overlap map rebuild with ICP result fetch

Adds a single-thread kernel that computes on the GPU whether to insert the frame into the kd map, from the ICP result and the accumulated delta pose. The map move and rebuild are then enqueued on the map stream, sized to a worst-case bound with device-read counts, before the host reads back the ICP result. This removes the host round trip between ICP completion and the map rebuild. In exchange the sort and index kernels are launched over an upper bound and exit early, a second sorted buffer keeps correspondence export valid, and host-side map state must be restored and reconciled after the fact, which adds complexity and risk.

```diff
diff --git a/pylidar_slam_b200/csrc/context.cu b/pylidar_slam_b200/csrc/context.cu
--- a/pylidar_slam_b200/csrc/context.cu
+++ b/pylidar_slam_b200/csrc/context.cu
@@ -309,7 +309,7 @@
     ctx->scan.status.release();
     ctx->sel[0].status.release(); ctx->sel[1].status.release(); ctx->input_zbuf.release();
     for (auto& b : ctx->kd.store) b.release();
-    ctx->kd.morton.release(); ctx->kd.order.release(); ctx->kd.sorted.release(); ctx->kd.normals.release();
+    ctx->kd.morton.release(); ctx->kd.order.release(); ctx->kd.sorted.release(); ctx->kd.sorted_prev.release(); ctx->kd.normals.release();
     ctx->kd.bbox.release(); ctx->kd.grid_hdr.release(); ctx->kd.cells.release(); ctx->kd.stats.release();
     ctx->kd_worklist.release(); ctx->kd_nn_state.release();
     ctx->pm.vmaps.release(); ctx->pm.nmaps.release(); ctx->pm.poses.release();
@@ -324,6 +324,7 @@
     if (ctx->ev_map_done) cudaEventDestroy(ctx->ev_map_done);
     if (ctx->ev_inputs) cudaEventDestroy(ctx->ev_inputs);
     if (ctx->ev_batch) cudaEventDestroy(ctx->ev_batch);
+    if (ctx->ev_icp_done) cudaEventDestroy(ctx->ev_icp_done);
     ctx->gs_host_xyz.release(); ctx->gs_host_idx.release();
     if (ctx->stream_map) cudaStreamDestroy(ctx->stream_map);
     if (ctx->own_stream) cudaStreamDestroy(ctx->stream_main);
diff --git a/pylidar_slam_b200/csrc/internal.cuh b/pylidar_slam_b200/csrc/internal.cuh
--- a/pylidar_slam_b200/csrc/internal.cuh
+++ b/pylidar_slam_b200/csrc/internal.cuh
@@ -117,6 +117,8 @@
     std::deque<int64_t> frame_counts;
     DBuf morton, order;
     DBuf sorted;
+    DBuf sorted_prev;
+    uint32_t prev_gen = 0;
     DBuf normals;
     DBuf bbox;
     bool bbox_clean = false;
@@ -167,6 +169,20 @@
 struct Comm;
 
 static_assert(sizeof(FrameResult) <= kScalarOffset, "FrameResult must fit before the scalar slots");
+
+struct KdUpdateWords {
+    float X[12];
+    float delta[16];
+    uint32_t gate;
+    uint32_t insert;
+    uint32_t skip;
+    uint32_t kept;
+    uint32_t num_new;
+    uint32_t total;
+    uint32_t pad[2];
+};
+constexpr size_t kUpdateOffset = kScalarOffset - 256;
+static_assert(sizeof(FrameResult) <= kUpdateOffset && sizeof(KdUpdateWords) <= 256, "KdUpdateWords after FrameResult");
 
 }
 
@@ -219,6 +235,7 @@
     pls::DBuf batch_buf;
     pls::DBuf hyp_buf;
     cudaEvent_t ev_batch = nullptr;
+    cudaEvent_t ev_icp_done = nullptr;
     pls::DBuf gs_keys, gs_vals, gs_out_xyz, gs_out_idx;
     uint32_t gs_seq = 0;
     pls::HBuf gs_host_xyz, gs_host_idx;
@@ -281,6 +298,12 @@
 }
 inline FrameResult* frame_result_dev(pls_context* ctx) { return reinterpret_cast<FrameResult*>(ctx->scalars.p); }
 inline FrameResult* frame_result_host(pls_context* ctx) { return reinterpret_cast<FrameResult*>(ctx->pinned.p); }
+inline KdUpdateWords* kd_update_words_dev(pls_context* ctx) {
+    return reinterpret_cast<KdUpdateWords*>(reinterpret_cast<char*>(ctx->scalars.p) + kUpdateOffset);
+}
+inline const KdUpdateWords* kd_update_words_host(pls_context* ctx) {
+    return reinterpret_cast<const KdUpdateWords*>(reinterpret_cast<const char*>(ctx->pinned.p) + kUpdateOffset);
+}
 
 void map_stream_begin(pls_context* ctx);
 void map_stream_end(pls_context* ctx);
@@ -302,7 +325,7 @@
 }
 
 void radix_sort_pairs(pls_context* ctx, uint64_t* keys, uint32_t* vals, int64_t n, int num_passes,
-                      uint64_t** keys_out, uint32_t** vals_out, int64_t cap_n = 0);
+                      uint64_t** keys_out, uint32_t** vals_out, int64_t cap_n = 0, const uint32_t* n_dev = nullptr);
 
 void exclusive_scan_flags(pls_context* ctx, const uint8_t* flags, int64_t n, uint32_t* pos_out,
                           uint32_t* total_dev);
@@ -341,6 +364,9 @@
 void kdmap_reset(pls_context* ctx);
 void kdmap_update(pls_context* ctx, const float* rel_pose_host, const float* pts_dev, int64_t n,
                   const float* vmap_dev, int H, int W, int64_t known_count);
+int64_t kdmap_device_update_bound(const pls_context* ctx, int64_t new_bound);
+void kdmap_update_on_device(pls_context* ctx, const float4* fresh_dev, int64_t bound, const KdUpdateWords* upd);
+void kdmap_settle_device_update(pls_context* ctx, const KdUpdateWords& w, int local_map_size);
 void kdmap_update_packed(pls_context* ctx, const float* rel_pose_host, const float4* fresh_dev, int64_t num_new,
                          bool has_new);
 constexpr int KD_BATCH_GRID = 6;
diff --git a/pylidar_slam_b200/csrc/kdmap.cu b/pylidar_slam_b200/csrc/kdmap.cu
--- a/pylidar_slam_b200/csrc/kdmap.cu
+++ b/pylidar_slam_b200/csrc/kdmap.cu
@@ -30,8 +30,17 @@
 __global__ void __launch_bounds__(256)
 kd_move_append_kernel(const float4* __restrict__ src, int64_t skip, int64_t kept, Rigid X,
                       const float4* __restrict__ fresh, const uint32_t* __restrict__ num_new_dev, int64_t num_new_cap,
-                      float4* __restrict__ dst, int* __restrict__ bbox) {
-    const int64_t num_new = num_new_dev ? (int64_t)*num_new_dev : num_new_cap;
+                      float4* __restrict__ dst, int* __restrict__ bbox, const KdUpdateWords* __restrict__ upd) {
+    int64_t num_new = num_new_dev ? (int64_t)*num_new_dev : num_new_cap;
+    if (upd) {
+        skip = upd->skip;
+        kept = upd->kept;
+        num_new = upd->num_new;
+#pragma unroll
+        for (int i = 0; i < 9; ++i) X.R[i] = upd->X[i];
+#pragma unroll
+        for (int i = 0; i < 3; ++i) X.t[i] = upd->X[9 + i];
+    }
     const int64_t total = kept + num_new;
     float mn[3] = {FLT_MAX, FLT_MAX, FLT_MAX}, mx[3] = {-FLT_MAX, -FLT_MAX, -FLT_MAX};
     for (int64_t k = (int64_t)blockIdx.x * blockDim.x + threadIdx.x; k < total; k += (int64_t)gridDim.x * blockDim.x) {
@@ -155,8 +164,9 @@
         if (flags[i]) out[pos[i]] = make_float4(vmap[i], vmap[hw + i], vmap[2 * hw + i], 0.f);
 }
 
-__global__ void kd_grid_header_kernel(int* __restrict__ bbox, KdGridHeader* __restrict__ hdr, float cell_target) {
-    if (threadIdx.x != 0) return;
+__global__ void kd_grid_header_kernel(int* __restrict__ bbox, KdGridHeader* __restrict__ hdr, float cell_target,
+                                      const uint32_t* __restrict__ gate) {
+    if (threadIdx.x != 0 || (gate && !*gate)) return;
     const float mnx = ordered_to_float(bbox[0]), mny = ordered_to_float(bbox[1]), mnz = ordered_to_float(bbox[2]);
     const float ex = ordered_to_float(bbox[3]) - mnx, ey = ordered_to_float(bbox[4]) - mny,
                 ez = ordered_to_float(bbox[5]) - mnz;
@@ -174,8 +184,9 @@
 }
 
 __global__ void kd_cell_key_kernel(const float4* __restrict__ pts, int64_t n, const KdGridHeader* __restrict__ hdr,
-                                   uint64_t* __restrict__ keys, uint32_t* __restrict__ vals) {
+                                   uint64_t* __restrict__ keys, uint32_t* __restrict__ vals, const uint32_t* __restrict__ n_dev) {
     pls_grid_dependency_wait();
+    if (n_dev) n = *n_dev;
     const float mnx = hdr->mn[0], mny = hdr->mn[1], mnz = hdr->mn[2];
     const float scale = hdr->scale;
     const int b0 = hdr->b0;
@@ -214,8 +225,10 @@
 
 __global__ void __launch_bounds__(256)
 kd_finalize_kernel(const float4* __restrict__ pts, const uint64_t* __restrict__ keys, const uint32_t* __restrict__ order,
-                   int64_t n, CellTables T, KdGridHeader* hdr, uint32_t gen, float4* __restrict__ sorted) {
+                   int64_t n, CellTables T, KdGridHeader* hdr, uint32_t gen, float4* __restrict__ sorted,
+                   const uint32_t* __restrict__ n_dev) {
     pls_grid_dependency_wait();
+    if (n_dev) n = *n_dev;
     const int top = hdr->top;
     for (int64_t i = (int64_t)blockIdx.x * blockDim.x + threadIdx.x; i < n; i += (int64_t)gridDim.x * blockDim.x) {
         const uint32_t src = order[i];
@@ -926,14 +939,15 @@
     return ix;
 }
 
-void build_index(pls_context* ctx) {
+void build_index(pls_context* ctx, const KdUpdateWords* upd) {
     KdMap& kd = ctx->kd;
     cudaStream_t st = ctx->stream;
     const int64_t M = kd.count;
     kd.indexed = M;
     kd.valid = M > 0;
     if (M <= 0) return;
-    ProfileScope ps(ctx, 3, (double)M * 32.0);
+    ProfileScope ps(ctx, 3, (double)M * 32.0, upd == nullptr);
+    const uint32_t* n_dev = upd ? &upd->total : nullptr;
     PLS_REQUIRE(M < (1ll << 30), "kd map: too many points");
     kd_reserve_capacity(ctx, M);
     kd.gen += 1;
@@ -945,14 +959,15 @@
     const float4* pts = kd.store[kd.cur].as<float4>();
     kd.grid_hdr.reserve(sizeof(KdGridHeader), st);
     static const float cell_target = getenv("PLS_KD_CELL") ? (float)atof(getenv("PLS_KD_CELL")) : KD_CELL_TARGET;
-    kd_grid_header_kernel<<<1, 32, 0, st>>>(kd.bbox.as<int>(), kd.grid_hdr.as<KdGridHeader>(), cell_target);
+    kd_grid_header_kernel<<<1, 32, 0, st>>>(kd.bbox.as<int>(), kd.grid_hdr.as<KdGridHeader>(), cell_target,
+                                            upd ? &upd->gate : nullptr);
     PLS_CHECK_LAUNCH();
     kd.bbox_clean = true;
     launch_dependent(kd_cell_key_kernel, grid_for(M, 256, 8 * kNumSMs), 256, st, pts, M, kd.grid_hdr.as<KdGridHeader>(),
-                     kd.morton.as<uint64_t>(), kd.order.as<uint32_t>());
+                     kd.morton.as<uint64_t>(), kd.order.as<uint32_t>(), n_dev);
     uint64_t* sk;
     uint32_t* sv;
-    radix_sort_pairs(ctx, kd.morton.as<uint64_t>(), kd.order.as<uint32_t>(), M, 4, &sk, &sv, kd.cap_points);
+    radix_sort_pairs(ctx, kd.morton.as<uint64_t>(), kd.order.as<uint32_t>(), M, 4, &sk, &sv, kd.cap_points, n_dev);
     cell_table_bytes(kd.cap_points, kd.table_mask, kd.table_offset);
     CellTables T;
     for (int l = 0; l < KD_MAX_LEVELS; ++l) {
@@ -960,7 +975,7 @@
         T.mask[l] = kd.table_mask[l];
     }
     launch_dependent(kd_finalize_kernel, grid_for(M, 256, 8 * kNumSMs), 256, st, pts, sk, sv, M, T, kd.grid_hdr.as<KdGridHeader>(),
-                     kd.gen, kd.sorted.as<float4>());
+                     kd.gen, kd.sorted.as<float4>(), n_dev);
 }
 
 }
@@ -1026,10 +1041,37 @@
     PLS_CHECK_LAUNCH();
 }
 
+namespace {
+
+void move_and_rebuild(pls_context* ctx, int64_t skip, int64_t kept, const Rigid& X, const float4* fresh_dev,
+                      int64_t num_new, int64_t total, const KdUpdateWords* upd) {
+    KdMap& kd = ctx->kd;
+    cudaStream_t st = ctx->stream;
+    kd_reserve_capacity(ctx, total > 0 ? total : 1);
+    const int dst = kd.cur ^ 1;
+    kd.bbox.reserve(8 * sizeof(int), st);
+    if (!kd.bbox_clean) {
+        kd_bbox_init_kernel<<<1, 32, 0, st>>>(kd.bbox.as<int>());
+        PLS_CHECK_LAUNCH();
+    }
+    kd.bbox_clean = false;
+    if (total > 0) {
+        kd_move_append_kernel<<<grid_for(total, 256, 8 * kNumSMs), 256, 0, st>>>(
+            kd.store[kd.cur].as<float4>(), skip, kept, X, fresh_dev, nullptr, num_new, kd.store[dst].as<float4>(),
+            kd.bbox.as<int>(), upd);
+        PLS_CHECK_LAUNCH();
+    }
+    kd.cur = dst;
+    kd.count = total;
+    kd.prev_gen = upd ? kd.gen : 0;
+    build_index(ctx, upd);
+}
+
+}
+
 void kdmap_update_packed(pls_context* ctx, const float* rel_pose_host, const float4* fresh_dev, int64_t num_new,
                          bool has_new) {
     KdMap& kd = ctx->kd;
-    cudaStream_t st = ctx->stream;
     Rigid X;
     int64_t skip = 0;
     const bool first = kd.frame_counts.empty() && kd.count == 0;
@@ -1056,23 +1098,38 @@
     const int64_t kept = kd.count - skip;
     const int64_t total = kept + num_new;
     if (num_new > kd.max_frame) kd.max_frame = num_new;
-    kd_reserve_capacity(ctx, total > 0 ? total : 1);
-    const int dst = kd.cur ^ 1;
-    kd.bbox.reserve(8 * sizeof(int), st);
-    if (!kd.bbox_clean) {
-        kd_bbox_init_kernel<<<1, 32, 0, st>>>(kd.bbox.as<int>());
-        PLS_CHECK_LAUNCH();
-    }
-    kd.bbox_clean = false;
-    if (total > 0) {
-        kd_move_append_kernel<<<grid_for(total, 256, 8 * kNumSMs), 256, 0, st>>>(
-            kd.store[kd.cur].as<float4>(), skip, kept, X, fresh_dev, nullptr, num_new, kd.store[dst].as<float4>(),
-            kd.bbox.as<int>());
-        PLS_CHECK_LAUNCH();
-    }
-    kd.cur = dst;
-    kd.count = total;
-    build_index(ctx);
+    move_and_rebuild(ctx, skip, kept, X, fresh_dev, num_new, total, nullptr);
+}
+
+int64_t kdmap_device_update_bound(const pls_context* ctx, int64_t new_bound) {
+    const KdMap& kd = ctx->kd;
+    if (kd.frame_counts.empty() || kd.gen + 1 >= 0x7ffffff0u) return 0;
+    int64_t bound = kd.count + new_bound;
+    if (bound > kd.cap_points) bound = kd.cap_points;
+    if (bound > (1ll << 30) - 1) bound = (1ll << 30) - 1;
+    return bound;
+}
+
+void kdmap_update_on_device(pls_context* ctx, const float4* fresh_dev, int64_t bound, const KdUpdateWords* upd) {
+    KdMap& kd = ctx->kd;
+    PLS_REQUIRE(bound > 0 && bound >= kd.count && bound <= kd.cap_points,
+                "kd map: a device-decided update needs a bound within the planned capacity");
+    std::swap(kd.sorted, kd.sorted_prev);
+    kd.sorted.reserve_exact((size_t)kd.cap_points * sizeof(float4), ctx->stream);
+    move_and_rebuild(ctx, 0, bound, Rigid{}, fresh_dev, bound - kd.count, bound, upd);
+}
+
+void kdmap_settle_device_update(pls_context* ctx, const KdUpdateWords& w, int local_map_size) {
+    KdMap& kd = ctx->kd;
+    if (w.insert) {
+        kd.frame_counts.push_back((int64_t)w.num_new);
+        if ((int)kd.frame_counts.size() > local_map_size) kd.frame_counts.pop_front();
+        if ((int64_t)w.num_new > kd.max_frame) kd.max_frame = (int64_t)w.num_new;
+    }
+    kd.count = (int64_t)w.total;
+    kd.indexed = kd.count;
+    kd.valid = kd.count > 0;
+    if (kd.count > 0) profile_credit(ctx, 3, 1, (double)kd.count * 32.0);
 }
 
 void kdmap_update(pls_context* ctx, const float* rel_pose_host, const float* pts_dev, int64_t n,
@@ -1566,7 +1623,9 @@
     PLS_API_BEGIN_FRAME(ctx)
     const KdMap& kd = ctx->kd;
     if (!kd.searched) throw pls::Error{PLS_E_STATE, "pls_kdmap_last_correspondences: no kd search has run"};
-    if (!kd.valid || kd.searched_gen != kd.gen)
+    const bool current = kd.valid && kd.searched_gen == kd.gen;
+    const bool replaced = kd.prev_gen != 0 && kd.searched_gen == kd.prev_gen;
+    if (!current && !replaced)
         throw pls::Error{PLS_E_STATE, "pls_kdmap_last_correspondences: the map was rebuilt since the last search"};
     if (kd.searched_sharded)
         throw pls::Error{PLS_E_STATE, "pls_kdmap_last_correspondences: the last ICP split its queries over the ranks"};
@@ -1588,8 +1647,10 @@
             ctx->stage_out[3].reserve((size_t)n * 3 * sizeof(float), st);
             nb = ctx->stage_out[3].as<float>();
         }
+        KdIndex ix = make_index(ctx);
+        if (!current) ix.sorted = kd.sorted_prev.as<float4>();
         kd_search_export_kernel<<<grid_for(n, 256, 8 * kNumSMs), 256, 0, st>>>(
-            make_index(ctx), ctx->nn_prev.as<int>(), n, nb, kd.searched_normals ? (float*)onr.dev : nullptr,
+            ix, ctx->nn_prev.as<int>(), n, nb, kd.searched_normals ? (float*)onr.dev : nullptr,
             (long long*)oix.dev);
         PLS_CHECK_LAUNCH();
         if (onr.dev && !kd.searched_normals)
diff --git a/pylidar_slam_b200/csrc/odometry.cu b/pylidar_slam_b200/csrc/odometry.cu
--- a/pylidar_slam_b200/csrc/odometry.cu
+++ b/pylidar_slam_b200/csrc/odometry.cu
@@ -1,6 +1,8 @@
 #include <stdlib.h>
 
 #include <chrono>
+#include <functional>
+#include <optional>
 #include <utility>
 #include <vector>
 
@@ -260,12 +262,80 @@
     return last_blocks;
 }
 
+__device__ __forceinline__ void mat4_mul_rn(const float* A, const float* B, float* C) {
+    for (int i = 0; i < 4; ++i)
+        for (int j = 0; j < 4; ++j) {
+            float s = 0.f;
+            for (int k = 0; k < 4; ++k) s = __fadd_rn(s, __fmul_rn(A[i * 4 + k], B[k * 4 + j]));
+            C[i * 4 + j] = s;
+        }
+}
+
+__device__ __forceinline__ float norm3_rn(float a, float b, float c) {
+    return __fsqrt_rn(__fadd_rn(__fadd_rn(__fmul_rn(a, a), __fmul_rn(b, b)), __fmul_rn(c, c)));
+}
+
+__global__ void kd_update_decision_kernel(const FrameResult* __restrict__ fr, KdUpdateWords* __restrict__ w, Pose16 delta,
+                                          float threshold_trans, float threshold_rot, int max_num_alignments,
+                                          uint32_t map_count, uint32_t evict_count, uint32_t total_limit,
+                                          const uint32_t* __restrict__ gs_overflow, uint32_t gs_seq) {
+    const bool failed = fr->status == PLS_E_SINGULAR || fr->status == PLS_E_COMM;
+    const bool ready = (fr->done || fr->iters >= max_num_alignments) && !failed && !(gs_overflow && *gs_overflow == gs_seq);
+    float T[16];
+    for (int i = 0; i < 16; ++i) T[i] = fr->T[i];
+    float nd[16];
+    mat4_mul_rn(delta.m, T, nd);
+    float sy = __fsqrt_rn(__fadd_rn(__fmul_rn(nd[0], nd[0]), __fmul_rn(nd[4], nd[4])));
+    float e[3];
+    if (!(sy < 1e-6f)) {
+        e[0] = atan2f(nd[9], nd[10]);
+        e[1] = atan2f(-nd[8], sy);
+        e[2] = atan2f(nd[4], nd[0]);
+    } else {
+        e[0] = atan2f(-nd[6], nd[5]);
+        e[1] = atan2f(-nd[8], sy);
+        e[2] = 0.f;
+    }
+    const float tn = norm3_rn(nd[3], nd[7], nd[11]);
+    const float rn = norm3_rn(e[0], e[1], e[2]);
+    bool insert = ready && (tn > threshold_trans ||
+                            __fdiv_rn(__fmul_rn(rn, 180.0f), 3.14159265358979323846f) > threshold_rot);
+    const bool gate = ready && map_count - (insert ? evict_count : 0u) + (insert ? (uint32_t)fr->counts[2] : 0u) <= total_limit;
+    insert = insert && gate;
+    const double R[9] = {T[0], T[1], T[2], T[4], T[5], T[6], T[8], T[9], T[10]};
+    const double t[3] = {T[3], T[7], T[11]};
+    for (int i = 0; i < 3; ++i) {
+        for (int j = 0; j < 3; ++j) w->X[3 * i + j] = (float)R[j * 3 + i];
+        w->X[9 + i] = __double2float_rn(
+            -__dadd_rn(__dadd_rn(__dmul_rn(R[i], t[0]), __dmul_rn(R[3 + i], t[1])), __dmul_rn(R[6 + i], t[2])));
+    }
+    for (int i = 0; i < 16; ++i) w->delta[i] = !gate ? delta.m[i] : (insert ? ((i % 5 == 0) ? 1.f : 0.f) : nd[i]);
+    const uint32_t num_new = insert ? (uint32_t)fr->counts[2] : 0u;
+    const uint32_t skip = insert ? evict_count : 0u;
+    w->gate = gate ? 1u : 0u;
+    w->insert = insert ? 1u : 0u;
+    w->skip = gate ? skip : 0u;
+    w->kept = gate ? map_count - skip : 0u;
+    w->num_new = num_new;
+    w->total = gate ? map_count - skip + num_new : 0u;
+}
+
 struct HostTrace {
     bool on = getenv("PLS_HOST_TRACE") != nullptr;
-    double acc[4] = {0, 0, 0, 0};
+    bool in_call = false;
+    double acc[6] = {0, 0, 0, 0, 0, 0};
     int frames = 0, extra_rounds = 0;
     std::chrono::steady_clock::time_point t;
     void start() { if (on) t = std::chrono::steady_clock::now(); }
+    void begin_call() {
+        start();
+        in_call = on;
+    }
+    void frame_start() {
+        if (in_call) lap(5);
+        else start();
+        in_call = false;
+    }
     void lap(int k) {
         if (!on) return;
         const auto now = std::chrono::steady_clock::now();
@@ -274,12 +344,14 @@
     }
     void end_frame() {
         if (!on || ++frames < 64) return;
-        fprintf(stderr, "[plslam_b200 host trace] per frame: enqueue input+ICP %.1f us, wait for the pose %.1f us, "
-                        "map-update enqueue %.1f us, rest %.1f us; %d of %d frames needed a second round of ICP launches\n",
-                acc[0] / frames, acc[1] / frames, acc[2] / frames, acc[3] / frames, extra_rounds, frames);
+        fprintf(stderr, "[plslam_b200 host trace] per frame: call prologue: map-update flush %.1f us, grid-sample "
+                        "enqueue %.1f us; enqueue input+ICP %.1f us, wait for the pose %.1f us, map update %.1f us, "
+                        "rest %.1f us; %d of %d frames needed a second round of ICP launches\n",
+                acc[4] / frames, acc[5] / frames, acc[0] / frames, acc[1] / frames, acc[2] / frames, acc[3] / frames,
+                extra_rounds, frames);
         frames = 0;
         extra_rounds = 0;
-        acc[0] = acc[1] = acc[2] = acc[3] = 0;
+        for (double& a : acc) a = 0;
     }
 };
 HostTrace g_trace;
@@ -362,34 +434,46 @@
     return extra;
 }
 
-int run_icp(pls_context* ctx, int64_t query_bound, const uint32_t* bound_dev) {
-    cudaStream_t st = ctx->stream;
-    FrameResult* fr = frame_result_dev(ctx);
+void enqueue_result_copy(pls_context* ctx, cudaStream_t st) {
+    PLS_CUDA(cudaMemcpyAsync(ctx->pinned.p, ctx->scalars.p, kScalarOffset + SC_NUM * sizeof(uint32_t), cudaMemcpyDeviceToHost,
+                             st));
+}
+
+void fetch_result(pls_context* ctx) {
+    enqueue_result_copy(ctx, ctx->stream);
+    PLS_CUDA(cudaStreamSynchronize(ctx->stream));
+}
+
+int run_icp(pls_context* ctx, int64_t query_bound, const uint32_t* bound_dev, const std::function<void()>& after_upfront,
+            int* extra_rounds) {
     if (query_bound < 1) query_bound = 1;
     ctx->pm.zbuf_clean = false;
     int blocks = 0;
+    bool fresh = false;
     auto enqueue = [&](int first, int last) {
         blocks = enqueue_icp_iterations(ctx, query_bound, bound_dev, first, last);
-        if (first == 0) g_trace.lap(0);
+        fresh = false;
+        if (first == 0) {
+            g_trace.lap(0);
+            if (after_upfront) {
+                after_upfront();
+                g_trace.lap(2);
+            }
+        }
     };
     auto read_done = [&](int* done) {
-        int flags[3];
-        PLS_CUDA(cudaMemcpyAsync(flags, &fr->iters, sizeof(flags), cudaMemcpyDeviceToHost, st));
-        PLS_CUDA(cudaStreamSynchronize(st));
-        done[0] = flags[2];
+        fetch_result(ctx);
+        fresh = true;
+        done[0] = frame_result_host(ctx)->done;
     };
-    g_trace.extra_rounds += icp_rounds(&ctx, 1, enqueue, read_done);
+    *extra_rounds = icp_rounds(&ctx, 1, enqueue, read_done);
+    g_trace.extra_rounds += *extra_rounds;
+    if (*extra_rounds > 0 && after_upfront) {
+        after_upfront();
+        fresh = false;
+    }
+    if (!fresh) fetch_result(ctx);
     return blocks;
-}
-
-void enqueue_result_copy(pls_context* ctx, cudaStream_t st) {
-    PLS_CUDA(cudaMemcpyAsync(ctx->pinned.p, ctx->scalars.p, kScalarOffset + SC_NUM * sizeof(uint32_t), cudaMemcpyDeviceToHost,
-                             st));
-}
-
-void fetch_result(pls_context* ctx) {
-    enqueue_result_copy(ctx, ctx->stream);
-    PLS_CUDA(cudaStreamSynchronize(ctx->stream));
 }
 
 void credit_icp_profile(pls_context* ctx, const FrameResult* h, int blocks) {
@@ -458,6 +542,7 @@
     int64_t pts_bound = 0;
     int64_t query_bound = 0;
     const uint32_t* n_dev = nullptr;
+    int64_t map_points = 0;
 };
 
 struct FrameOut {
@@ -619,21 +704,29 @@
 
     flush_map_update(ctx);
     map_stream_wait(ctx);
+    in.map_points = ctx->kd.count;
     frame_begin(ctx, init_pose, nullptr, queries_are_rows);
     return true;
 }
 
-void frame_epilogue(pls_context* ctx, const FrameIn& in, const FrameOut& out, bool trace) {
+void frame_epilogue(pls_context* ctx, const FrameIn& in, const FrameOut& out, bool trace, const KdUpdateWords* upd) {
     FrameResult* h = frame_result_host(ctx);
     ctx->last_icp_iters = h->iters;
     raise_status(ctx, h->status);
 
-    const bool insert = keyframe_decision(ctx, h->T);
-    ctx->upd_pending = true;
-    ctx->upd_insert = insert;
-    memcpy(ctx->upd_T, h->T, sizeof(ctx->upd_T));
-    ctx->upd_slot = ctx->frame_slot;
-    ctx->upd_count = (long long)h->counts[2];
+    bool insert;
+    if (upd) {
+        insert = upd->insert != 0;
+        memcpy(ctx->delta_since_update, upd->delta, sizeof(ctx->delta_since_update));
+        kdmap_settle_device_update(ctx, *upd, ctx->cfg.local_map_size);
+    } else {
+        insert = keyframe_decision(ctx, h->T);
+        ctx->upd_pending = true;
+        ctx->upd_insert = insert;
+        memcpy(ctx->upd_T, h->T, sizeof(ctx->upd_T));
+        ctx->upd_slot = ctx->frame_slot;
+        ctx->upd_count = (long long)h->counts[2];
+    }
     if (trace) g_trace.lap(2);
     ctx->frame_index += 1;
     if (out.pose) memcpy(out.pose, h->T, 16 * sizeof(float));
@@ -643,7 +736,7 @@
         out.info[0] = (double)h->iters;
         out.info[1] = h->iters > 0 ? (double)h->losses[h->iters - 1] : 0.0;
         out.info[2] = (double)h->counts[1];
-        out.info[3] = (double)ctx->kd.count;
+        out.info[3] = (double)in.map_points;
         out.info[4] = (double)h->counts[0];
         out.info[5] = (double)(in.pts_bound - (int64_t)h->counts[2]);
         out.info[6] = (double)h->status;
@@ -654,14 +747,75 @@
     out.put_samples();
 }
 
+struct KdMirror {
+    int cur;
+    int64_t count, indexed;
+    bool valid, bbox_clean;
+    uint32_t gen, prev_gen;
+    const void* sorted;
+    explicit KdMirror(const pls_context* ctx)
+        : cur(ctx->kd.cur), count(ctx->kd.count), indexed(ctx->kd.indexed), valid(ctx->kd.valid),
+          bbox_clean(ctx->kd.bbox_clean), gen(ctx->kd.gen), prev_gen(ctx->kd.prev_gen), sorted(ctx->kd.sorted.p) {}
+    void restore(pls_context* ctx) const {
+        KdMap& kd = ctx->kd;
+        kd.cur = cur;
+        kd.count = count;
+        kd.indexed = indexed;
+        kd.valid = valid;
+        kd.bbox_clean = bbox_clean;
+        kd.gen = gen;
+        kd.prev_gen = prev_gen;
+        if (kd.sorted.p != sorted) std::swap(kd.sorted, kd.sorted_prev);
+    }
+};
+
+void enqueue_device_map_update(pls_context* ctx, const FrameIn& in) {
+    KdMap& kd = ctx->kd;
+    const int64_t bound = kdmap_device_update_bound(ctx, in.pts_bound);
+    const int64_t evict =
+        (int64_t)kd.frame_counts.size() + 1 > ctx->cfg.local_map_size ? kd.frame_counts.front() : 0;
+    Pose16 delta;
+    memcpy(delta.m, ctx->delta_since_update, sizeof(delta.m));
+    map_stream_wait(ctx);
+    kd_update_decision_kernel<<<1, 1, 0, ctx->stream>>>(frame_result_dev(ctx), kd_update_words_dev(ctx), delta,
+                                                         ctx->cfg.threshold_trans, ctx->cfg.threshold_rot,
+                                                         ctx->cfg.max_num_alignments, (uint32_t)kd.count, (uint32_t)evict,
+                                                         (uint32_t)bound, in.n_dev ? scalar_u32(ctx, SC_GS_OVERFLOW) : nullptr, ctx->gs_seq);
+    PLS_CHECK_LAUNCH();
+    if (!ctx->ev_icp_done) PLS_CUDA(cudaEventCreateWithFlags(&ctx->ev_icp_done, cudaEventDisableTiming));
+    PLS_CUDA(cudaEventRecord(ctx->ev_icp_done, ctx->stream_main));
+    PLS_CUDA(cudaStreamWaitEvent(ctx->stream_map, ctx->ev_icp_done, 0));
+    map_stream_begin(ctx);
+    try {
+        kdmap_update_on_device(ctx, ctx->frame_pts_buf[ctx->frame_slot].as<float4>(), bound, kd_update_words_dev(ctx));
+    } catch (...) {
+        map_stream_end(ctx);
+        throw;
+    }
+    map_stream_end(ctx);
+}
+
 bool process_frame_device(pls_context* ctx, const void* data_void, int layout, int64_t n, const uint32_t* n_dev,
                           const float* init_pose, FrameOut out) {
-    g_trace.start();
+    g_trace.frame_start();
     FrameIn in;
     if (!frame_input(ctx, data_void, layout, n, n_dev, init_pose, in, out)) return true;
-    int icp_blocks = run_icp(ctx, in.query_bound, in.n_dev);
-    fetch_result(ctx);
+    const bool device_update = ctx->cfg.local_map_type == PLS_MAP_KDTREE && comm_size(ctx) == 1 &&
+                               kdmap_device_update_bound(ctx, in.pts_bound) > 0;
+    const KdMirror before(ctx);
+    std::optional<KdMirror> after;
+    std::function<void()> update;
+    if (device_update)
+        update = [&] {
+            enqueue_device_map_update(ctx, in);
+            after.emplace(ctx);
+            before.restore(ctx);
+        };
+    int extra_rounds = 0;
+    int icp_blocks = run_icp(ctx, in.query_bound, in.n_dev, update, &extra_rounds);
     g_trace.lap(1);
+    const KdUpdateWords* upd = device_update && kd_update_words_host(ctx)->gate ? kd_update_words_host(ctx) : nullptr;
+    if (upd) after->restore(ctx);
     if (in.n_dev) {
         bool overflowed = false;
         const int64_t rows = grid_sample_host_count(ctx, &overflowed);
@@ -673,7 +827,7 @@
     }
     ctx->icp_result = true;
     credit_icp_profile(ctx, frame_result_host(ctx), icp_blocks);
-    frame_epilogue(ctx, in, out, true);
+    frame_epilogue(ctx, in, out, true, upd);
     g_trace.lap(3);
     g_trace.end_frame();
     return true;
@@ -813,8 +967,8 @@
         T0_dev = ctx->tmp[6].as<float>();
     }
     frame_begin(ctx, nullptr, T0_dev, false);
-    const int icp_blocks = run_icp(ctx, n, nullptr);
-    fetch_result(ctx);
+    int extra_rounds = 0;
+    const int icp_blocks = run_icp(ctx, n, nullptr, nullptr, &extra_rounds);
     ctx->icp_result = true;
     FrameResult* h = frame_result_host(ctx);
     credit_icp_profile(ctx, h, icp_blocks);
@@ -918,7 +1072,9 @@
 int pls_process_frame_grid_sample(pls_context* ctx, const float* raw_points, int64_t n, double voxel, int layout,
                                   const float* init_pose, float* out_pose, float* out_params, int* out_has_pose,
                                   double* out_info) {
+    g_trace.begin_call();
     PLS_API_BEGIN(ctx)
+    g_trace.lap(4);
     PLS_REQUIRE(raw_points && n > 0 && voxel > 0.0, "pls_process_frame_grid_sample: bad arguments");
     if (const char* why = frame_refusal(ctx, layout, n, voxel)) throw pls::Error{PLS_E_INVALID, why};
     const void* d = to_device(ctx, raw_points, (size_t)n * 3 * sizeof(float), ctx->stage_in[0]);
@@ -1093,7 +1249,7 @@
             const int i = icp_seq[j];
             cur = i;
             try {
-                frame_epilogue(icp[j], in[i], outputs(i), false);
+                frame_epilogue(icp[j], in[i], outputs(i), false, nullptr);
             } catch (const pls::Error& e) {
                 if (e.code != PLS_E_SINGULAR) throw;
                 icp[j]->err = e.msg;
diff --git a/pylidar_slam_b200/csrc/primitives.cu b/pylidar_slam_b200/csrc/primitives.cu
--- a/pylidar_slam_b200/csrc/primitives.cu
+++ b/pylidar_slam_b200/csrc/primitives.cu
@@ -26,10 +26,11 @@
 __global__ void __launch_bounds__(256) sort_hist_kernel(const uint64_t* __restrict__ keys, int64_t n,
                                                         int num_passes, uint32_t* __restrict__ hist,
                                                         uint32_t* __restrict__ done_counter, uint32_t* __restrict__ status,
-                                                        int64_t status_words) {
+                                                        int64_t status_words, const uint32_t* __restrict__ n_dev) {
     __shared__ uint32_t sh[8 * RADIX];
     __shared__ int s_last;
     pls_grid_dependency_wait();
+    if (n_dev) n = *n_dev;
     for (int64_t i = (int64_t)blockIdx.x * blockDim.x + threadIdx.x; i < status_words; i += (int64_t)gridDim.x * blockDim.x)
         status[i] = 0u;
     for (int i = threadIdx.x; i < num_passes * RADIX; i += blockDim.x) sh[i] = 0;
@@ -67,7 +68,7 @@
 __global__ void __launch_bounds__(SORT_THREADS)
 sort_pass_kernel(const uint64_t* __restrict__ kin, const uint32_t* __restrict__ vin, uint64_t* __restrict__ kout,
                  uint32_t* __restrict__ vout, int64_t n, int shift, const uint32_t* __restrict__ base,
-                 uint32_t* status, uint32_t* tile_counter) {
+                 uint32_t* status, uint32_t* tile_counter, const uint32_t* __restrict__ n_dev) {
     __shared__ uint32_t warp_hist[SORT_WARPS][RADIX];
     __shared__ uint32_t tile_offset[RADIX];
     __shared__ uint32_t s_tile;
@@ -81,6 +82,10 @@
     for (int i = tid; i < SORT_WARPS * RADIX; i += SORT_THREADS) (&warp_hist[0][0])[i] = 0;
     __syncthreads();
     const uint32_t tile = s_tile;
+    if (n_dev) {
+        n = *n_dev;
+        if ((int64_t)tile * SORT_TILE >= n) return;
+    }
     const int64_t seg = (int64_t)tile * SORT_TILE + (int64_t)warp * (32 * SORT_ITEMS);
     const uint32_t lt_mask = (1u << lane) - 1u;
 
@@ -259,7 +264,7 @@
 }
 
 void radix_sort_pairs(pls_context* ctx, uint64_t* keys, uint32_t* vals, int64_t n, int num_passes,
-                      uint64_t** keys_out, uint32_t** vals_out, int64_t cap_n) {
+                      uint64_t** keys_out, uint32_t** vals_out, int64_t cap_n, const uint32_t* n_dev) {
     PLS_REQUIRE(num_passes >= 1 && num_passes <= 8, "radix_sort_pairs: 1..8 passes");
     PLS_REQUIRE(n < (1ll << 30), "radix_sort_pairs: n must be < 2^30");
     SortScratch& s = ctx->sort;
@@ -282,7 +287,7 @@
     int hist_blocks = (int)((n + 256 * 4 - 1) / (256 * 4));
     if (hist_blocks > kNumSMs) hist_blocks = kNumSMs;
     launch_dependent(sort_hist_kernel, hist_blocks, 256, st, keys, n, num_passes, s.hist.as<uint32_t>(),
-                     s.hist.as<uint32_t>() + 8 * RADIX, s.status.as<uint32_t>(), (int64_t)status_words);
+                     s.hist.as<uint32_t>() + 8 * RADIX, s.status.as<uint32_t>(), (int64_t)status_words, n_dev);
     uint64_t* kin = keys;
     uint32_t* vin = vals;
     uint64_t* kout = s.keys_alt.as<uint64_t>();
@@ -290,7 +295,8 @@
     uint32_t* counters = s.status.as<uint32_t>() + (size_t)num_passes * tiles * RADIX;
     for (int p = 0; p < num_passes; ++p) {
         launch_dependent(sort_pass_kernel, (unsigned)tiles, SORT_THREADS, st, kin, vin, kout, vout, n, 8 * p,
-                         s.hist.as<uint32_t>() + p * RADIX, s.status.as<uint32_t>() + (size_t)p * tiles * RADIX, counters + p);
+                         s.hist.as<uint32_t>() + p * RADIX, s.status.as<uint32_t>() + (size_t)p * tiles * RADIX, counters + p,
+                         n_dev);
         uint64_t* tk = kin; kin = kout; kout = tk;
         uint32_t* tv = vin; vin = vout; vout = tv;
     }
```

After: 2157 (median of 6 runs). +7.5%, better.
